# chengzhag/PanFusion

Hardware: AMD Instinct MI355X
Metric: DDIM denoise steps/sec, 512x1024 pano + 20x512^2 views (higher is better)
Workload: dtype fp16; 1 GPU; cfg2: 512x1024 pano + 20x512^2 views, CFG pair, SD-2-base UNet shapes; views=20, cfg_pair=True, hip_graphs=True, parallelism=single

## Files before the change

### include/panfusion_hip.h

```cpp
#ifndef PANFUSION_HIP_H
#define PANFUSION_HIP_H

#include <stddef.h>
#include <stdint.h>

#ifdef __cplusplus
extern "C" {
#endif

typedef enum { PF_OK = 0, PF_ERR_ARG = 1, PF_ERR_LAUNCH = 2, PF_ERR_UNSUPPORTED = 3 } pf_status;
typedef enum { PF_BF16 = 0, PF_F16 = 1, PF_F32 = 2, PF_U8 = 3 } pf_dtype;

int pf_version(void);
const char* pf_last_error_string(void);


pf_status pf_e2p_grid(const double* host_fov, const double* host_theta, const double* host_phi,
                      int ncam, int eh, int ew, int h, int w,
                      float* map_x, float* map_y, float* lonlat, void* stream);

pf_status pf_p2e_grid(const double* host_fov, const double* host_theta, const double* host_phi,
                      int ncam, int ph, int pw, int h, int w,
                      float* map_u, float* map_v, uint8_t* mask, void* stream);

// ... 63 lines not shown
pf_status pf_crop_width(const void* x, int dtype, int n, int h, int w, int C, int crop, void* y, void* stream);

pf_status pf_pad_width_rows(const void* x, int elem_bytes, long rows, int w, int pad, void* y, void* stream);
pf_status pf_roll_width_rows(const void* x, int elem_bytes, long rows, int w, int shift, void* y, void* stream);

pf_status pf_nchw_to_nhwc(const void* x, int src_dtype, int n, int C, int h, int w, int dst_dtype, void* y, void* stream);
pf_status pf_nhwc_to_nchw(const void* x, int src_dtype, int n, int C, int h, int w, int dst_dtype, void* y, void* stream);

pf_status pf_add(const void* a, int dtype_a, const void* b, int dtype_b, long n, void* y, void* stream);

pf_status pf_embed_tokens(const int64_t* ids, int B, int L, int Lp, int C, long vocab, const float* tok,
                          const float* pos, int out_dtype, void* out, void* stream);

pf_status pf_softmax_rows(const float* scores, long rows, int n, long scores_ld, float scale, int out_dtype,
                          void* probs, long probs_ld, void* stream);

pf_status pf_tensor_to_image(const float* x, int n, int C, int h, int w, uint8_t* y, void* stream);

pf_status pf_cfg_ddim_step(const float* x, const float* eps_uncond, const float* eps_cond,
                           float guidance, float sqrt_a_t, float sqrt_1m_a_t, float sqrt_a_prev,
                           float sqrt_1m_a_prev, long rows, int W, int roll, float* out, void* stream);

pf_status pf_cfg_ddim_step_pair(const float* x, const float* eps_uncond, const float* eps_cond,
                                float guidance, float sqrt_a_t, float sqrt_1m_a_t, float sqrt_a_prev,
                                float sqrt_1m_a_prev, long rows, int W, int roll, float* out, float* out2,
                                int64_t* tstep, int n_tstep, int64_t t_next, void* stream);

pf_status pf_cfg_dpmpp_step_pair(const float* x, const float* eps_uncond, const float* eps_cond,
                                 float guidance, float sqrt_a_t, float sqrt_1m_a_t, float sqrt_a_prev,
                                 float sqrt_1m_a_prev, long rows, int W, int roll, float* out, float* out2,
                                 int64_t* tstep, int n_tstep, int64_t t_next, const float* x0_prev, float k,
                                 float* x0_out, void* stream);

pf_status pf_cfg_inpaint_step_pair(const float* x, const float* eps_uncond, const float* eps_cond,
                                   float guidance, float sqrt_a_t, float sqrt_1m_a_t, float sqrt_a_prev,
                                   float sqrt_1m_a_prev, long rows, int W, int roll, float* out, float* out2,
                                   int64_t* tstep, int n_tstep, int64_t t_next, const float* x0_prev, float k,
                                   float* x0_out, const float* known, const float* noise, const float* mask,
                                   float ka, float kb, int known_roll, void* stream);

pf_status pf_noised_start_pair(const float* z, const float* noise, float ka, float kb, long rows, int W, int roll,
                               float* out, float* out2, int64_t* tstep, int n_tstep, int64_t t0, void* stream);

pf_status pf_upsampled_start_pair(const float* z, const float* noise, float ka, float kb, long planes, int h_src, int w_src,
                                  int H, int W, int mode, int wrap, int roll, float* out, float* out2, int64_t* tstep,
                                  int n_tstep, int64_t t0, void* stream);

typedef struct {
    const void* a0;
    const void* a1;
    int c0, c1;
    int a0_ld, a1_ld;
    int n_img, h_in, w_in;
    int h_out, w_out;
    int ksize;
    int stride;
    int pad;
    int upsample;
    const void* w;
    int n_out;
    const float* bias;
    const float* rowvec;
    int rowvec_ld;
    const void* residual;
    int res_ld;
    int res_dtype;
    void* out;
    int out_ld;
    int out_dtype;
    int dtype;
    int batch;
    long a_bstride, w_bstride, out_bstride, res_bstride;
    int epilogue;
    void* workspace;
    size_t workspace_bytes;
    float* gn_partial;
    int wrap_pad;
    int crop;
    int* tickets;
    int n_tickets;
    int split3;
    int subpixel;
    int gn_rows;
} pf_conv_desc;

enum { PF_EPILOGUE_NONE = 0, PF_EPILOGUE_GEGLU = 1, PF_EPILOGUE_SPLIT = 2 };

size_t pf_conv_gemm_workspace_size(const pf_conv_desc* desc);
int pf_conv_gemm_gn_rows(const pf_conv_desc* desc);
int pf_conv_gemm_kernel_id(const pf_conv_desc* desc);
typedef struct {
    int kernel;
    int mrep, nrep;
    int block_rows;
    int waves;
    int ring_slots;
    int splits;
    int kb_per_split;
    int m_split;
    int tail_splits, tail_kb;
    int gn_rows;
    int n_tickets;
    size_t workspace_bytes;
} pf_conv_plan;
pf_status pf_conv_gemm_plan(const pf_conv_desc* desc, int want_moments, pf_conv_plan* out);
pf_status pf_debug_gemm_profile(void* device_buffer, long capacity_blocks);
pf_status pf_conv_gemm(const pf_conv_desc* desc, void* stream);

typedef struct {
    const void* a; int a_ld;
    const void* w;
    const float* bias;
    const float* residual; int res_ld;
    void* out; int out_ld;
    void* out_vt; int vt_ld; int rows_per_batch; long vt_bs;
    const float* ln_gamma; const float* ln_beta; float ln_eps; void* ln_out; int ln_ld;
    int M, N, K;
    int dtype; int mode;
} pf_linear_ws_desc;
enum { PF_LWS_16 = 0, PF_LWS_F32 = 1, PF_LWS_GEGLU = 2, PF_LWS_QKV = 3, PF_LWS_F32_LN = 4, PF_LWS_VT = 5 };
int pf_linear_ws_supported(long M, int N, int K, int mode);
pf_status pf_linear_ws(const pf_linear_ws_desc* desc, void* stream);

pf_status pf_conv_in(const float* x, int n, int cin, int h, int w, const float* wgt, const float* bias,
                     int cout, int wrap, int out_dtype, void* y, void* stream);
pf_status pf_conv_out(const void* x, int dtype, int n, int cin, int h, int w, const float* wgt,
                      const float* bias, int cout, int wrap, float* y, void* stream);
pf_status pf_conv_out_gn(const float* x, int n, int cin, int h, int w, const float* scale, const float* shift, int act,
                         const float* wgt_t, const float* bias, int cout, int wrap, float* y, void* stream);

typedef struct {
    const void* q; const void* k; const void* vt; void* out;
    int dtype;
    int B, H, D;
    int nq, nk;
    int q_ld, k_ld, vt_ld, o_ld;
    long q_bs, k_bs, vt_bs, o_bs;
    float scale;
    const float* bias; long bias_ld;
    const uint8_t* flags; int flags_ld;
    float* lse;
    void* workspace; size_t workspace_bytes;
} pf_attn_desc;

pf_status pf_attention(const pf_attn_desc* desc, void* stream);
size_t pf_attention_workspace_size(const pf_attn_desc* desc);


pf_status pf_attention_delta(const void* out, const void* dout, int dtype, int B, int H, int D, long nq,
                             int ld, long bs, float* delta, void* stream);

typedef struct {
    const void* q; const void* k; const void* v; const void* dout;
    const void* qt; const void* kt; const void* dot;
    void* dq; void* dk; void* dv;
    int dtype;
    int B, H, D;
    int nq, nk;
    int q_ld, k_ld, v_ld, do_ld;
    int qt_ld, kt_ld, dot_ld;
    int dq_ld, dk_ld, dv_ld;
    long q_bs, k_bs, v_bs, do_bs, qt_bs, kt_bs, dot_bs, dq_bs, dk_bs, dv_bs;
    float scale;
    const float* bias; long bias_ld;
    const uint8_t* flags; int flags_ld;
    const float* lse; const float* delta;
// ... 58 lines not shown
```

### panfusion_amd/_lib.py

```python
import ctypes as C
import os

_HERE = os.path.dirname(os.path.abspath(__file__))
LIB_PATH = os.environ.get("PF_HIP_LIB") or os.path.join(_HERE, "libpanfusion_hip.so")

PF_OK = 0
PF_BF16, PF_F16, PF_F32, PF_U8 = 0, 1, 2, 3

c_void_p, c_int, c_long, c_float, c_size_t = C.c_void_p, C.c_int, C.c_long, C.c_float, C.c_size_t
c_dp = C.POINTER(C.c_double)


class ConvDesc(C.Structure):
    _fields_ = [
        ("a0", c_void_p), ("a1", c_void_p), ("c0", c_int), ("c1", c_int),
        ("a0_ld", c_int), ("a1_ld", c_int),
        ("n_img", c_int), ("h_in", c_int), ("w_in", c_int), ("h_out", c_int), ("w_out", c_int),
        ("ksize", c_int), ("stride", c_int), ("pad", c_int), ("upsample", c_int),
        ("w", c_void_p), ("n_out", c_int),
        ("bias", c_void_p), ("rowvec", c_void_p), ("rowvec_ld", c_int),
        ("residual", c_void_p), ("res_ld", c_int), ("res_dtype", c_int),
        ("out", c_void_p), ("out_ld", c_int), ("out_dtype", c_int), ("dtype", c_int),
        ("batch", c_int),
        ("a_bstride", c_long), ("w_bstride", c_long), ("out_bstride", c_long), ("res_bstride", c_long),
        ("epilogue", c_int), ("workspace", c_void_p), ("workspace_bytes", c_size_t),
        ("gn_partial", c_void_p), ("wrap_pad", c_int), ("crop", c_int),
        ("tickets", c_void_p), ("n_tickets", c_int), ("split3", c_int), ("subpixel", c_int), ("gn_rows", c_int),
    ]


class ConvPlan(C.Structure):
    _fields_ = [
        ("kernel", c_int), ("mrep", c_int), ("nrep", c_int), ("block_rows", c_int), ("waves", c_int), ("ring_slots", c_int),
        ("splits", c_int), ("kb_per_split", c_int), ("m_split", c_int), ("tail_splits", c_int), ("tail_kb", c_int),
        ("gn_rows", c_int), ("n_tickets", c_int), ("workspace_bytes", c_size_t),
    ]


class AttnDesc(C.Structure):
    _fields_ = [
        ("q", c_void_p), ("k", c_void_p), ("vt", c_void_p), ("out", c_void_p),
        ("dtype", c_int), ("B", c_int), ("H", c_int), ("D", c_int), ("nq", c_int), ("nk", c_int),
        ("q_ld", c_int), ("k_ld", c_int), ("vt_ld", c_int), ("o_ld", c_int),
        ("q_bs", c_long), ("k_bs", c_long), ("vt_bs", c_long), ("o_bs", c_long),
        ("scale", c_float),
        ("bias", c_void_p), ("bias_ld", c_long), ("flags", c_void_p), ("flags_ld", c_int),
        ("lse", c_void_p),
        ("workspace", c_void_p), ("workspace_bytes", c_size_t),
    ]


class LinearWsDesc(C.Structure):
    _fields_ = [
        ("a", c_void_p), ("a_ld", c_int), ("w", c_void_p), ("bias", c_void_p),
        ("residual", c_void_p), ("res_ld", c_int), ("out", c_void_p), ("out_ld", c_int),
        ("out_vt", c_void_p), ("vt_ld", c_int), ("rows_per_batch", c_int), ("vt_bs", c_long),
        ("ln_gamma", c_void_p), ("ln_beta", c_void_p), ("ln_eps", c_float), ("ln_out", c_void_p), ("ln_ld", c_int),
        ("M", c_int), ("N", c_int), ("K", c_int), ("dtype", c_int), ("mode", c_int),
    ]


class AttnBwdDesc(C.Structure):
    _fields_ = [
        ("q", c_void_p), ("k", c_void_p), ("v", c_void_p), ("dout", c_void_p),
        ("qt", c_void_p), ("kt", c_void_p), ("dot", c_void_p),
        ("dq", c_void_p), ("dk", c_void_p), ("dv", c_void_p),
        ("dtype", c_int), ("B", c_int), ("H", c_int), ("D", c_int), ("nq", c_int), ("nk", c_int),
        ("q_ld", c_int), ("k_ld", c_int), ("v_ld", c_int), ("do_ld", c_int),
        ("qt_ld", c_int), ("kt_ld", c_int), ("dot_ld", c_int),
        ("dq_ld", c_int), ("dk_ld", c_int), ("dv_ld", c_int),
        ("q_bs", c_long), ("k_bs", c_long), ("v_bs", c_long), ("do_bs", c_long), ("qt_bs", c_long), ("kt_bs", c_long),
        ("dot_bs", c_long), ("dq_bs", c_long), ("dk_bs", c_long), ("dv_bs", c_long),
        ("scale", c_float),
        ("bias", c_void_p), ("bias_ld", c_long), ("flags", c_void_p), ("flags_ld", c_int),
        ("lse", c_void_p), ("delta", c_void_p),
        ("workspace", c_void_p), ("workspace_bytes", c_size_t),
    ]


SIGNATURES = {
    "pf_version": (c_int, []),
    "pf_last_error_string": (C.c_char_p, []),
    "pf_e2p_grid": (c_int, [c_dp, c_dp, c_dp, c_int, c_int, c_int, c_int, c_int,
                            c_void_p, c_void_p, c_void_p, c_void_p]),
    "pf_p2e_grid": (c_int, [c_dp, c_dp, c_dp, c_int, c_int, c_int, c_int, c_int,
                            c_void_p, c_void_p, c_void_p, c_void_p]),
    "pf_py360_e2p": (c_int, [c_void_p, c_int, c_int, c_int, c_int, c_dp, c_dp, c_dp, c_dp, c_dp, c_int, c_int, c_int, c_int,
                             c_void_p, c_void_p]),
    "pf_nearest_indices": (c_int, [c_void_p, c_void_p, c_long, c_int, c_int, c_void_p, c_void_p]),
    "pf_remap": (c_int, [c_void_p, c_int, c_int, c_int, c_int, c_int, c_void_p, c_void_p, c_void_p,
                         c_int, c_int, c_int, c_int, c_void_p, c_void_p]),
    "pf_equi_coords": (c_int, [c_int, c_int, c_void_p, c_void_p]),
    "pf_spherical_pe": (c_int, [c_void_p, c_long, c_void_p, c_int, c_void_p, c_void_p]),
    "pf_epa_tables_workspace_size": (c_size_t, [c_int, c_int, c_int, c_int, c_int]),
    "pf_epa_tables_build": (c_int, [c_dp, c_dp, c_dp, c_int, c_int, c_int, c_int, c_int,
                                    c_void_p, c_void_p, c_void_p, c_void_p, c_void_p, c_size_t, c_void_p]),
    "pf_groupnorm_workspace_size": (c_size_t, [c_int, c_int, c_int]),
    "pf_groupnorm_stats": (c_int, [c_void_p, c_int, c_void_p, c_int, c_int, c_int, c_int, c_int, c_float,
                                   c_void_p, c_void_p, c_void_p, c_void_p, c_void_p, c_size_t, c_void_p]),
    "pf_groupnorm_stats_wrap": (c_int, [c_void_p, c_int, c_void_p, c_int, c_int, c_int, c_int, c_int, c_int, c_int, c_float,
                                        c_void_p, c_void_p, c_void_p, c_void_p, c_void_p, c_size_t, c_void_p]),
    "pf_scale_shift_act": (c_int, [c_void_p, c_int, c_void_p, c_int, c_int, c_int, c_int,
                                   c_void_p, c_void_p, c_int, c_int, c_int, c_void_p, c_void_p]),
    "pf_layernorm": (c_int, [c_void_p, c_void_p, c_long, c_int, c_long, c_int, c_void_p, c_void_p,
                             c_float, c_int, c_void_p, c_void_p]),
    "pf_axpby": (c_int, [c_void_p, c_void_p, c_float, c_float, c_long, c_void_p, c_void_p]),
    "pf_vae_sample": (c_int, [c_void_p, c_void_p, c_int, c_int, c_long, c_float, c_void_p, c_void_p]),
    "pf_geglu": (c_int, [c_void_p, c_int, c_long, c_int, c_void_p, c_void_p]),
    "pf_timestep_features": (c_int, [c_void_p, c_int, c_int, c_int, c_void_p, c_void_p]),
    "pf_timestep_features_strided": (c_int, [c_void_p, c_long, c_int, c_int, c_int, c_void_p, c_void_p]),
# ... 123 lines not shown
```

### panfusion_amd/csrc/pf_common.h

```cpp
#pragma once
#include <hip/hip_runtime.h>
#include <stdint.h>
#include <stdio.h>
#include <stdarg.h>
#include "../../include/panfusion_hip.h"

namespace pf {

void set_error(const char* fmt, ...);

#define PF_REQUIRE(cond, ...)                         \
    do {                                              \
        if (!(cond)) {                                \
            pf::set_error(__VA_ARGS__);               \
            return PF_ERR_ARG;                        \
        }                                             \
    } while (0)

#define PF_CHECK_LAUNCH(name)                                                        \
    do {                                                                             \
        hipError_t e__ = hipGetLastError();                                          \
        if (e__ != hipSuccess) {                                                     \
            pf::set_error("%s: launch failed: %s", name, hipGetErrorString(e__));    \
            return PF_ERR_LAUNCH;                                                    \
        }                                                                            \
    } while (0)

static inline bool aligned16(const void* p) { return (reinterpret_cast<uintptr_t>(p) & 15) == 0; }
static inline hipStream_t as_stream(void* s) { return reinterpret_cast<hipStream_t>(s); }
static inline long cdiv(long a, long b) { return (a + b - 1) / b; }

struct Bf16 { static constexpr int id = PF_BF16; };
struct F16  { static constexpr int id = PF_F16; };

typedef __attribute__((ext_vector_type(8))) unsigned short u16x8;
typedef __attribute__((ext_vector_type(4))) unsigned short u16x4;
typedef __attribute__((ext_vector_type(4))) float f32x4;
typedef __attribute__((ext_vector_type(16))) float f32x16;

template <typename T> __device__ __forceinline__ float to_f32(unsigned short v);
template <> __device__ __forceinline__ float to_f32<Bf16>(unsigned short v) {
    return __uint_as_float(static_cast<unsigned>(v) << 16);
}
template <> __device__ __forceinline__ float to_f32<F16>(unsigned short v) {
    _Float16 h;
    __builtin_memcpy(&h, &v, 2);
    return static_cast<float>(h);
}

template <typename T> __device__ __forceinline__ unsigned short from_f32(float f);
template <> __device__ __forceinline__ unsigned short from_f32<Bf16>(float f) {
    __bf16 b = static_cast<__bf16>(f);
    unsigned short v;
    __builtin_memcpy(&v, &b, 2);
    return v;
}
template <> __device__ __forceinline__ unsigned short from_f32<F16>(float f) {
    _Float16 h = static_cast<_Float16>(f);
    unsigned short v;
    __builtin_memcpy(&v, &h, 2);
    return v;
}

template <typename T> __device__ __forceinline__ void unpack8(const u16x8& v, float (&f)[8]) {
#pragma unroll
    for (int i = 0; i < 8; ++i) f[i] = to_f32<T>(v[i]);
}
template <typename T> __device__ __forceinline__ u16x8 pack8(const float (&f)[8]) {
    u16x8 v;
#pragma unroll
    for (int i = 0; i < 8; ++i) v[i] = from_f32<T>(f[i]);
    return v;
}

__host__ __device__ __forceinline__ int pair_off(int c) { return ((c >> 5) << 6) | (c & 31); }

__device__ __forceinline__ float silu_f(float x) { return x / (1.0f + __expf(-x)); }

template <typename S> __device__ __forceinline__ float ld_any(const void* p, long i);
struct AnyF32 {}; struct AnyBf16 {}; struct AnyF16 {};
template <> __device__ __forceinline__ float ld_any<AnyF32>(const void* p, long i) { return static_cast<const float*>(p)[i]; }
template <> __device__ __forceinline__ float ld_any<AnyBf16>(const void* p, long i) { return to_f32<Bf16>(static_cast<const unsigned short*>(p)[i]); }
template <> __device__ __forceinline__ float ld_any<AnyF16>(const void* p, long i) { return to_f32<F16>(static_cast<const unsigned short*>(p)[i]); }
template <typename S> __device__ __forceinline__ void st_any(void* p, long i, float v);
template <> __device__ __forceinline__ void st_any<AnyF32>(void* p, long i, float v) { static_cast<float*>(p)[i] = v; }
template <> __device__ __forceinline__ void st_any<AnyBf16>(void* p, long i, float v) { static_cast<unsigned short*>(p)[i] = from_f32<Bf16>(v); }
template <> __device__ __forceinline__ void st_any<AnyF16>(void* p, long i, float v) { static_cast<unsigned short*>(p)[i] = from_f32<F16>(v); }

template <typename T> struct Mfma32;
template <> struct Mfma32<Bf16> {
    typedef __attribute__((ext_vector_type(8))) __bf16 frag;
    static __device__ __forceinline__ f32x16 run(frag a, frag b, f32x16 c) {
        return __builtin_amdgcn_mfma_f32_32x32x16_bf16(a, b, c, 0, 0, 0);
    }
};
template <> struct Mfma32<F16> {
    typedef __attribute__((ext_vector_type(8))) _Float16 frag;
    static __device__ __forceinline__ f32x16 run(frag a, frag b, f32x16 c) {
        return __builtin_amdgcn_mfma_f32_32x32x16_f16(a, b, c, 0, 0, 0);
    }
};

__device__ __forceinline__ float geglu_value(float v, float g) {
    const float ax = fabsf(g);
    const float t = __builtin_amdgcn_rcpf(fmaf(ax, 0.23164189f, 1.0f));
    float y = fmaf(t, 0.5307027145f, -0.7265760135f);
    y = fmaf(y, t, 0.7107068705f);
    y = fmaf(y, t, -0.142248368f);
    y = fmaf(y, t, 0.127414796f);
    y *= t;
    const float h = y * __builtin_amdgcn_exp2f(-0.72134752044448170368f * (g * g));
    return v * fmaf(-ax, h, fmaxf(g, 0.0f));
}

#define PF_DISPATCH_16(dtype, name, ...)                                         \
    do {                                                                         \
        if ((dtype) == PF_BF16) { using T = pf::Bf16; __VA_ARGS__; }             \
        else if ((dtype) == PF_F16) { using T = pf::F16; __VA_ARGS__; }          \
        else { pf::set_error("%s: dtype must be PF_BF16 or PF_F16", name); return PF_ERR_ARG; } \
    } while (0)

}
```

### panfusion_amd/csrc/pf_elementwise.hip

```cpp
#include "pf_common.h"
#include <stdlib.h>
#include <math.h>
#include <algorithm>

namespace pf {

__device__ __forceinline__ float wave_sum(float v) {
#pragma unroll
    for (int o = 32; o > 0; o >>= 1) v += __shfl_xor(v, o);
    return v;
}

struct F32In {};
template <typename TI> struct In8 {
    typedef unsigned short elem;
    static __device__ __forceinline__ void load(const elem* ptr, float (&f)[8]) {
        unpack8<TI>(*reinterpret_cast<const u16x8*>(ptr), f);
    }
};
template <> struct In8<F32In> {
    typedef float elem;
    static __device__ __forceinline__ void load(const elem* ptr, float (&f)[8]) {
        const float4 a = reinterpret_cast<const float4*>(ptr)[0], b = reinterpret_cast<const float4*>(ptr)[1];
        f[0] = a.x; f[1] = a.y; f[2] = a.z; f[3] = a.w; f[4] = b.x; f[5] = b.y; f[6] = b.z; f[7] = b.w;
// ... 195 lines not shown
            const int pr = pbeg + pl;
            const bool first = pr < P0;
            const int pp = first ? pr : pr - P0, Ps = first ? P0 : P1, ppi = first ? ppi0 : ppi1;
            const float* base = (first ? part0 : part1) + static_cast<long>(img) * ppi * 2 * Ps + pp;
            int k = slice;
            for (; k + 3 * slices < ppi; k += 4 * slices) {
                float a[4], b[4];
#pragma unroll
                for (int u = 0; u < 4; ++u) {
                    a[u] = base[static_cast<long>(k + u * slices) * 2 * Ps];
                    b[u] = base[static_cast<long>(k + u * slices) * 2 * Ps + Ps];
                }
#pragma unroll
                for (int u = 0; u < 4; ++u) { s += a[u]; q += b[u]; }
            }
            for (; k < ppi; k += slices) {
                s += base[static_cast<long>(k) * 2 * Ps];
                q += base[static_cast<long>(k) * 2 * Ps + Ps];
            }
        }
        if (slices > 1) {
            red_s[t] = s;
            red_q[t] = q;
            __syncthreads();
            if (t < npairs) {
                double ss = 0.0, qq = 0.0;
                for (int sl = 0; sl < slices; ++sl) { ss += red_s[sl * npairs + t]; qq += red_q[sl * npairs + t]; }
                chs[t] = ss;
                chq[t] = qq;
            }
        } else if (pl < npairs) {
            chs[pl] = s;
            chq[pl] = q;
        }
    }
    __syncthreads();
    if (t < gpb && blockIdx.y * gpb + t < groups) {
        double s = 0.0, q = 0.0;
        for (int j = 0; j < ppg; ++j) { s += chs[t * ppg + j]; q += chq[t * ppg + j]; }
        const double cnt = static_cast<double>(hw) * cpg;
        const double mean = s / cnt;
        double var = q / cnt - mean * mean;
        if (var < 0.0) var = 0.0;
        g_mean[t] = static_cast<float>(mean);
        g_rstd[t] = static_cast<float>(1.0 / sqrt(var + static_cast<double>(eps)));
    }
    __syncthreads();
    const int cbeg = blockIdx.y * gpb * cpg, cend = min(C, cbeg + gpb * cpg);
    for (int c = cbeg + t; c < cend; c += 256) {
        const int gg = (c - cbeg) / cpg;
        const float sc = g_rstd[gg] * gamma[c];
        scale[static_cast<long>(img) * C + c] = sc;
        shift[static_cast<long>(img) * C + c] = beta[c] - g_mean[gg] * sc;
    }
}

template <typename TI, typename T, int OUT>
__global__ __launch_bounds__(256) void k_scale_shift_act(const typename In8<TI>::elem* __restrict__ x0, int c0,
                                  const typename In8<TI>::elem* __restrict__ x1, int c1, int hw,
                                  const float* __restrict__ scale, const float* __restrict__ shift,
                                  int act, void* __restrict__ yv, unsigned short* __restrict__ raw_pair) {
    typedef typename In8<TI>::elem elem;
    const unsigned C = c0 + c1, OCT = C / 8, per_img = static_cast<unsigned>(hw) * OCT;
    const unsigned img = blockIdx.y;
    const unsigned j0 = (blockIdx.x * 256u + threadIdx.x) * 2u;
    if (j0 >= per_img) return;
    float v[2][8];
    unsigned cc[2];
    long pix[2];
#pragma unroll
    for (int u = 0; u < 2; ++u) {
        const unsigned j = min(j0 + u, per_img - 1);
        const unsigned p = j / OCT, c = (j - p * OCT) * 8;
        cc[u] = c;
        pix[u] = static_cast<long>(img) * hw + p;
        const elem* src = (c < static_cast<unsigned>(c0)) ? x0 + pix[u] * c0 + c : x1 + pix[u] * c1 + (c - c0);
        In8<TI>::load(src, v[u]);
    }
#pragma unroll
    for (int u = 0; u < 2; ++u) {
        if (j0 + u >= per_img) break;
        if (raw_pair) {
            unsigned short* y = raw_pair + pix[u] * (2 * C) + pair_off(cc[u]);
            const u16x8 hi = pack8<T>(v[u]);
            float lo[8];
#pragma unroll
            for (int j = 0; j < 8; ++j) lo[j] = v[u][j] - to_f32<T>(hi[j]);
            *reinterpret_cast<u16x8*>(y) = hi;
            *reinterpret_cast<u16x8*>(y + 32) = pack8<T>(lo);
        }
        float f[8];
        if (scale) {
            const float4* sc = reinterpret_cast<const float4*>(scale + static_cast<long>(img) * C + cc[u]);
            const float4* sh = reinterpret_cast<const float4*>(shift + static_cast<long>(img) * C + cc[u]);
            float4 s0 = sc[0], s1 = sc[1], h0 = sh[0], h1 = sh[1];
            const float sv[8] = {s0.x, s0.y, s0.z, s0.w, s1.x, s1.y, s1.z, s1.w};
            const float hv[8] = {h0.x, h0.y, h0.z, h0.w, h1.x, h1.y, h1.z, h1.w};
#pragma unroll
            for (int j = 0; j < 8; ++j) f[j] = v[u][j] * sv[j] + hv[j];
        } else {
#pragma unroll
            for (int j = 0; j < 8; ++j) f[j] = v[u][j];
        }
        if (act) {
#pragma unroll
            for (int j = 0; j < 8; ++j) f[j] = f[j] * __builtin_amdgcn_rcpf(1.0f + __expf(-f[j]));
        }
        if (OUT == 0) {
            *reinterpret_cast<u16x8*>(static_cast<unsigned short*>(yv) + pix[u] * C + cc[u]) = pack8<T>(f);
        } else if (OUT == 1) {
            unsigned short* y = static_cast<unsigned short*>(yv) + pix[u] * (2 * C) + pair_off(cc[u]);
            const u16x8 hi = pack8<T>(f);
            float lo[8];
#pragma unroll
            for (int j = 0; j < 8; ++j) lo[j] = f[j] - to_f32<T>(hi[j]);
            *reinterpret_cast<u16x8*>(y) = hi;
            *reinterpret_cast<u16x8*>(y + 32) = pack8<T>(lo);
        } else {
            store8_f32(static_cast<float*>(yv) + pix[u] * C + cc[u], f);
        }
    }
}

template <typename TI, typename T, int ROWS>
__global__ __launch_bounds__(256) void k_layernorm(const typename In8<TI>::elem* __restrict__ x, const float* __restrict__ pe,
                            long pe_rows, long rows, int C, const float* __restrict__ gamma,
                            const float* __restrict__ beta, float eps, unsigned short* __restrict__ y) {
    const int lane = threadIdx.x & 63;
    const long row0 = (blockIdx.x * static_cast<long>(blockDim.x >> 6) + (threadIdx.x >> 6)) * ROWS;
    if (row0 >= rows) return;
    const int OCT = C / 8;
    constexpr int KMAX = ROWS == 1 ? 4 : 1;
    float raw[ROWS][KMAX][8];
#pragma unroll
    for (int r = 0; r < ROWS; ++r)
#pragma unroll
        for (int k = 0; k < KMAX; ++k) {
            const int oct = lane + 64 * k;
#pragma unroll
            for (int j = 0; j < 8; ++j) raw[r][k][j] = 0.f;
            if (oct < OCT && row0 + r < rows) In8<TI>::load(x + (row0 + r) * C + oct * 8, raw[r][k]);
        }
#pragma unroll
    for (int r = 0; r < ROWS; ++r) {
        const long row = row0 + r;
        if (row >= rows) break;
        float (&v)[KMAX][8] = raw[r];
        float s = 0.f;
#pragma unroll
        for (int k = 0; k < KMAX; ++k) {
            const int oct = lane + 64 * k;
            if (oct < OCT) {
                if (pe) {
                    const float4* pp = reinterpret_cast<const float4*>(pe + (row % pe_rows) * C + oct * 8);
                    float4 a = pp[0], b = pp[1];
                    v[k][0] += a.x; v[k][1] += a.y; v[k][2] += a.z; v[k][3] += a.w;
                    v[k][4] += b.x; v[k][5] += b.y; v[k][6] += b.z; v[k][7] += b.w;
                }
#pragma unroll
                for (int j = 0; j < 8; ++j) s += v[k][j];
            }
        }
        const float mean = wave_sum(s) / static_cast<float>(C);
        float q = 0.f;
#pragma unroll
        for (int k = 0; k < KMAX; ++k) {
            const int oct = lane + 64 * k;
            if (oct < OCT) {
#pragma unroll
                for (int j = 0; j < 8; ++j) { float d = v[k][j] - mean; q += d * d; }
            }
        }
        const float rstd = 1.0f / sqrtf(wave_sum(q) / static_cast<float>(C) + eps);
#pragma unroll
        for (int k = 0; k < KMAX; ++k) {
            const int oct = lane + 64 * k;
            if (oct < OCT) {
                const float4* gp = reinterpret_cast<const float4*>(gamma + oct * 8);
                const float4* bp = reinterpret_cast<const float4*>(beta + oct * 8);
                float4 g0 = gp[0], g1 = gp[1], b0 = bp[0], b1 = bp[1];
                const float gv[8] = {g0.x, g0.y, g0.z, g0.w, g1.x, g1.y, g1.z, g1.w};
                const float bv[8] = {b0.x, b0.y, b0.z, b0.w, b1.x, b1.y, b1.z, b1.w};
                float f[8];
#pragma unroll
                for (int j = 0; j < 8; ++j) f[j] = (v[k][j] - mean) * rstd * gv[j] + bv[j];
                *reinterpret_cast<u16x8*>(y + row * C + oct * 8) = pack8<T>(f);
            }
        }
    }
}

template <typename T>
__global__ void k_geglu(const unsigned short* __restrict__ in, long total_oct, int inner,
                        unsigned short* __restrict__ out) {
    long i = blockIdx.x * static_cast<long>(blockDim.x) + threadIdx.x;
    if (i >= total_oct) return;
    const int OCT = inner / 8;
    const long row = i / OCT;
    const int c = (i % OCT) * 8;
    u16x8 a = *reinterpret_cast<const u16x8*>(in + row * 2 * inner + c);
// ... 1203 lines not shown
```

### panfusion_amd/csrc/pf_gemm.hip

```cpp
#include "pf_common.h"
#include "pf_gemm_params.h"
#include <stdlib.h>
#include <algorithm>
#include <atomic>
#include <type_traits>

namespace pf {


template <typename T> struct Mfma;
template <> struct Mfma<Bf16> {
    typedef __attribute__((ext_vector_type(8))) __bf16 frag;
    static __device__ __forceinline__ f32x4 run(frag a, frag b, f32x4 c) {
        return __builtin_amdgcn_mfma_f32_16x16x32_bf16(a, b, c, 0, 0, 0);
    }
    static __device__ __forceinline__ void acc_agpr(frag a, frag b, f32x4& c) {
        asm volatile("v_mfma_f32_16x16x32_bf16 %0, %1, %2, %0" : "+a"(c) : "v"(a), "v"(b));
    }
};
template <> struct Mfma<F16> {
    typedef __attribute__((ext_vector_type(8))) _Float16 frag;
    static __device__ __forceinline__ f32x4 run(frag a, frag b, f32x4 c) {
        return __builtin_amdgcn_mfma_f32_16x16x32_f16(a, b, c, 0, 0, 0);
    }
// ... 336 lines not shown
template <typename T, int MREP, int NREP, int NT, int BM, int BN, int HALVES = 1, bool STATS = false, typename F = NoOp>
__device__ __forceinline__ void epilogue_tile(const GemmParams& p, long bz, f32x4 (&acc)[MREP][NREP],
                                              unsigned short* smem16, int m0, int n0, int row_base, int col_base,
                                              int lane, int t, F after_ring = F()) {
    if constexpr (STATS) {
        if (!(p.out_f32 && p.residual)) gn_moments_phase<T, MREP, NREP>(p, bz, acc, m0, n0, row_base, col_base, lane);
        __builtin_amdgcn_sched_barrier(0);
    }
    __syncthreads();
    stamp(p, 4);
    after_ring();
    stamp(p, 5);
    if constexpr (STATS) {
        if (p.out_f32 && p.residual) {
            epilogue_f32_stats<T, MREP, NREP, true>(p, bz, acc, m0, n0, row_base, col_base, lane);
            return;
        }
    }
    const int n_store = p.geglu ? p.N >> 1 : p.N;
    if (p.split_out && !p.rowvec && (p.N & 3) == 0 && (p.out_ld & 3) == 0 && p.N >= 4) {
        if (!p.residual) { epilogue_f32<T, MREP, NREP, false, true>(p, bz, acc, m0, n0, row_base, col_base, lane); return; }
        if (p.res_f32 && (p.res_ld & 3) == 0) { epilogue_f32<T, MREP, NREP, true, true>(p, bz, acc, m0, n0, row_base, col_base, lane); return; }
    }
    if (p.out_f32 && !p.geglu && !p.rowvec && (p.N & 3) == 0 && (p.out_ld & 3) == 0 && p.N >= 4) {
        if (!p.residual) { epilogue_f32<T, MREP, NREP, false>(p, bz, acc, m0, n0, row_base, col_base, lane); return; }
        if (p.res_f32 && (p.res_ld & 3) == 0) { epilogue_f32<T, MREP, NREP, true>(p, bz, acc, m0, n0, row_base, col_base, lane); return; }
    }
    const bool staged = !p.out_f32 && !p.res_f32 && !p.split_out && (p.out_ld & 7) == 0 && (n_store & 7) == 0 && (p.N & 3) == 0;
    if (staged && !(p.rowvec && p.residual) && !(p.geglu && (p.rowvec || p.residual))) {
        if (p.geglu) epilogue_fast<T, MREP, NREP, NT, BM, BN, 1, 3>(p, bz, acc, smem16, m0, n0, row_base, col_base, lane, t);
        else if (p.rowvec && p.rows_per_img < BM) goto generic;
        else if (p.rowvec) epilogue_fast<T, MREP, NREP, NT, BM, BN, HALVES, 1>(p, bz, acc, smem16, m0, n0, row_base, col_base, lane, t);
        else if (p.residual) epilogue_fast<T, MREP, NREP, NT, BM, BN, HALVES, 2>(p, bz, acc, smem16, m0, n0, row_base, col_base, lane, t);
        else epilogue_fast<T, MREP, NREP, NT, BM, BN, HALVES, 0>(p, bz, acc, smem16, m0, n0, row_base, col_base, lane, t);
        return;
    }
generic:
    const int cq = 4 * (lane >> 4), rl = lane & 15;
#pragma unroll
    for (int i = 0; i < MREP; ++i) {
        const int m = m0 + row_base + i * 16 + rl;
#pragma unroll
        for (int j = 0; j < NREP; ++j) {
            const int n4 = n0 + col_base + j * 16 + cq;
            float v[4] = {acc[i][j][0], acc[i][j][1], acc[i][j][2], acc[i][j][3]};
            if (m < p.M && n4 < p.N) epilogue_store<T>(p, bz, m, n4, v);
        }
    }
}


template <typename T, int BM, int BN, int NT>
__device__ __forceinline__ void splitk_finish(const GemmParams& p, long bz, int tile_lin, int m0, int n0, int* flag, int t) {
    asm volatile("s_waitcnt vmcnt(0)" ::: "memory");
    __syncthreads();
    int* ticket = p.tickets + (bz * p.mtiles * p.ntiles + tile_lin);
    if (t == 0) {
        const int drawn = __hip_atomic_fetch_add(ticket, 1, __ATOMIC_RELAXED, __HIP_MEMORY_SCOPE_AGENT);
        *flag = drawn == p.splits - 1 ? 1 : 0;
    }
    __syncthreads();
    const bool last = *flag != 0;
    __syncthreads();
    if (!last) return;
    if (t == 0) __builtin_amdgcn_fence(__ATOMIC_ACQUIRE, "agent");
    __syncthreads();
    constexpr int QPR = BN / 4;
    const int Ms = p.M - p.m_begin;
    const long slab = static_cast<long>(p.batch) * Ms * p.N;
    for (int q = t; q < BM * QPR; q += NT) {
        const int r = q / QPR, m = m0 + r, n4 = n0 + (q - r * QPR) * 4;
        if (m >= p.M || n4 >= p.N) continue;
        const float* src = p.partial + (bz * Ms + (m - p.m_begin)) * p.N + n4;
        float v[4] = {0.f, 0.f, 0.f, 0.f};
        for (int s = 0; s < p.splits; ++s) {
            const float4 x = *reinterpret_cast<const float4*>(src + s * slab);
            v[0] += x.x; v[1] += x.y; v[2] += x.z; v[3] += x.w;
        }
        epilogue_store<T>(p, bz, m, n4, v);
    }
    if (t == 0) __hip_atomic_store(ticket, 0, __ATOMIC_RELAXED, __HIP_MEMORY_SCOPE_AGENT);
}

template <typename T, int MREP, int NREP, bool STATS = false, bool S3 = false, int STAGES = 2>
__global__ __launch_bounds__(256, STAGES > 2 ? 1 : 2) void k_conv_gemm(const GemmParams p) {
    constexpr int BM = 32 * MREP, BN = 32 * NREP;
    extern __shared__ __attribute__((aligned(16))) unsigned short smem[];
    unsigned short* As = smem;
    unsigned short* Bs = smem + STAGES * BM * 64;

    const int ntile_total = p.mtiles * p.ntiles;
    int tid_lin = blockIdx.x;
    {
        const int q = ntile_total / 8, r = ntile_total % 8;
        const int xcd = tid_lin % 8, idx = tid_lin / 8;
        tid_lin = (xcd < r ? xcd * (q + 1) : r * (q + 1) + (xcd - r) * q) + idx;
    }
    const int tile_n = tid_lin % p.ntiles, tile_m = tid_lin / p.ntiles;
    const int m0 = p.m_begin + tile_m * BM, n0 = tile_n * BN;
    const long bz = blockIdx.z;
    const unsigned short* a0 = p.a0 + bz * p.a_bs;
    const unsigned short* a1 = p.a1 ? p.a1 + bz * p.a_bs : nullptr;
    const unsigned short* wg = p.w + bz * p.w_bs;

    const int t = threadIdx.x, lane = t & 63;
    const int wave = __builtin_amdgcn_readfirstlane(t >> 6);
    const int wm = wave >> 1, wn = wave & 1;
    const int chunk = t & 7, lrow = t >> 3;
    const int lchunk8 = (chunk ^ ((lrow >> 1) & 7)) * 8;

    const int pad_y = p.subpix ? 1 - (static_cast<int>(bz) >> 1) : p.pad, pad_x = p.subpix ? 1 - (static_cast<int>(bz) & 1) : p.pad;
    int a_img[MREP], a_y[MREP], a_x[MREP];
#pragma unroll
    for (int i = 0; i < MREP; ++i) {
        const int m = m0 + i * 32 + lrow;
        if (m < p.M) {
            const int img = m / p.rows_per_img, rem = m - img * p.rows_per_img;
            const int yo = rem / p.w_out;
            a_img[i] = img;
            a_y[i] = yo * p.stride - pad_y;
            a_x[i] = (rem - yo * p.w_out + p.crop) * p.stride - pad_x;
        } else {
            a_img[i] = 0; a_y[i] = -(1 << 20); a_x[i] = 0;
        }
        if (p.fastseg) seg_pack(a_img[i], a_y[i], a_x[i], p.h_in, p.w_in);
    }
    constexpr unsigned OOB = 0x80000000u;
    auto uniform_ptr = [](const unsigned short* ptr) {
        const unsigned long long v = reinterpret_cast<unsigned long long>(ptr);
        const unsigned lo = __builtin_amdgcn_readfirstlane(static_cast<unsigned>(v));
        const unsigned hi = __builtin_amdgcn_readfirstlane(static_cast<unsigned>(v >> 32));
        return reinterpret_cast<unsigned short*>(static_cast<unsigned long long>(lo) | (static_cast<unsigned long long>(hi) << 32));
    };
    const __amdgpu_buffer_rsrc_t rs_w = __builtin_amdgcn_make_buffer_rsrc(uniform_ptr(wg), 0, __builtin_amdgcn_readfirstlane(p.w_bytes), 0x00020000);
    unsigned w_off[NREP];
#pragma unroll
    for (int j = 0; j < NREP; ++j) {
        const int n = n0 + j * 32 + lrow;
        w_off[j] = n < p.N ? static_cast<unsigned>(n * p.K + lchunk8) * 2u : OOB;
    }
    const int Ctot = p.c0 + p.c1;
    const int Hl = p.h_in << p.up, Wl = (p.w_in + 2 * p.wrap) << p.up;

    const int nkb = p.K / 64;
    const int kb0 = blockIdx.y * p.kb_per_split;
    const int kb1 = min(nkb, kb0 + p.kb_per_split);
    int kg = kb0 * 64;
    int tap = kg / Ctot, cc = kg - tap * Ctot;
    unsigned a_off[MREP];
    bool seg1 = false;
    auto set_segment = [&]() {
        const int ky = p.ksize == 3 ? tap / 3 : p.ksize == 2 ? tap >> 1 : 0, kx = p.ksize == 3 ? tap - 3 * ky : p.ksize == 2 ? tap & 1 : 0;
        seg1 = __builtin_amdgcn_readfirstlane(cc >= p.c0 ? 1 : 0) != 0;
        const int ld = seg1 ? p.a1_ld : p.a0_ld;
        if (p.fastseg) {
            const unsigned sel = (1u << ky) | (16u << kx);
            const int tap_pix = ky * p.w_in + kx;
#pragma unroll
            for (int i = 0; i < MREP; ++i) {
                const unsigned off = ((static_cast<unsigned>(a_img[i]) + static_cast<unsigned>(tap_pix)) * static_cast<unsigned>(ld) + static_cast<unsigned>(lchunk8)) * 2u;
                a_off[i] = (static_cast<unsigned>(a_y[i]) & sel) == sel ? off : OOB;
            }
            return;
        }
#pragma unroll
        for (int i = 0; i < MREP; ++i) {
            const int yi = a_y[i] + ky, xi = a_x[i] + kx;
            const bool ok = yi >= 0 && yi < Hl && xi >= 0 && xi < Wl;
            int sx = (xi >> p.up) - p.wrap;
            sx += sx < 0 ? p.w_in : 0;
            sx -= sx >= p.w_in ? p.w_in : 0;
            const int pix = (a_img[i] * p.h_in + (yi >> p.up)) * p.w_in + sx;
            a_off[i] = ok ? static_cast<unsigned>(pix * ld + lchunk8) * 2u : OOB;
        }
    };
    set_segment();

    auto lds_dma = [&](const __amdgpu_buffer_rsrc_t& r, unsigned short* dst, unsigned voff, int soff) {
        __builtin_amdgcn_raw_ptr_buffer_load_lds(r, (__attribute__((address_space(3))) void*)dst, 16, voff, soff, 0, 0);
    };
    auto dma_stage = [&](int buf) {
        const int soff_a = __builtin_amdgcn_readfirstlane((seg1 ? cc - p.c0 : cc) * 2);
        const int soff_w = __builtin_amdgcn_readfirstlane(kg * 2);
        const __amdgpu_buffer_rsrc_t rs_a = __builtin_amdgcn_make_buffer_rsrc(
            uniform_ptr(seg1 ? a1 : a0), 0, __builtin_amdgcn_readfirstlane(seg1 ? p.a1_bytes : p.a0_bytes), 0x00020000);
#pragma unroll
        for (int i = 0; i < MREP; ++i) {
            unsigned short* dst = As + buf * BM * 64 + (i * 32 + wave * 8) * 64;
            lds_dma(rs_a, dst, a_off[i], soff_a);
        }
#pragma unroll
        for (int j = 0; j < NREP; ++j) {
            unsigned short* dst = Bs + buf * BN * 64 + (j * 32 + wave * 8) * 64;
            lds_dma(rs_w, dst, w_off[j], soff_w);
        }
        kg += 64;
        cc += 64;
        if (cc == Ctot) { cc = 0; ++tap; set_segment(); }
        else if (cc == p.c0) set_segment();
    };

    f32x4 acc[MREP][NREP];
#pragma unroll
    for (int i = 0; i < MREP; ++i)
#pragma unroll
        for (int j = 0; j < NREP; ++j) acc[i][j] = f32x4{0.f, 0.f, 0.f, 0.f};

    typedef typename Mfma<T>::frag frag;
    const int frow = lane & 15, fchunk = lane >> 4;
    auto compute = [&](int buf) {
        if constexpr (S3) {
            frag af[2][MREP], bf[2][NREP];
#pragma unroll
            for (int slab = 0; slab < 2; ++slab) {
#pragma unroll
                for (int i = 0; i < MREP; ++i)
                    af[slab][i] = __builtin_bit_cast(frag, *reinterpret_cast<const u16x8*>(As + buf * BM * 64 + lds_off(wm * 16 * MREP + i * 16 + frow, slab * 4 + fchunk)));
#pragma unroll
                for (int j = 0; j < NREP; ++j)
                    bf[slab][j] = __builtin_bit_cast(frag, *reinterpret_cast<const u16x8*>(Bs + buf * BN * 64 + lds_off(wn * 16 * NREP + j * 16 + frow, slab * 4 + fchunk)));
            }
#pragma unroll
            for (int i = 0; i < MREP; ++i)
#pragma unroll
                for (int j = 0; j < NREP; ++j) {
                    acc[i][j] = Mfma<T>::run(bf[0][j], af[0][i], acc[i][j]);
                    acc[i][j] = Mfma<T>::run(bf[0][j], af[1][i], acc[i][j]);
                    acc[i][j] = Mfma<T>::run(bf[1][j], af[0][i], acc[i][j]);
                }
            return;
        }
#pragma unroll
        for (int slab = 0; slab < 2; ++slab) {
            frag af[MREP], bf[NREP];
#pragma unroll
            for (int i = 0; i < MREP; ++i) {
                const int brow = wm * 16 * MREP + i * 16 + frow;
                u16x8 v = *reinterpret_cast<const u16x8*>(As + buf * BM * 64 + lds_off(brow, slab * 4 + fchunk));
                af[i] = __builtin_bit_cast(frag, v);
            }
#pragma unroll
            for (int j = 0; j < NREP; ++j) {
                const int brow = wn * 16 * NREP + j * 16 + frow;
                u16x8 v = *reinterpret_cast<const u16x8*>(Bs + buf * BN * 64 + lds_off(brow, slab * 4 + fchunk));
                bf[j] = __builtin_bit_cast(frag, v);
            }
#pragma unroll
            for (int i = 0; i < MREP; ++i)
#pragma unroll
                for (int j = 0; j < NREP; ++j) acc[i][j] = Mfma<T>::run(bf[j], af[i], acc[i][j]);
        }
    };

    stamp(p, 0);
    if constexpr (STAGES == 2) {
        dma_stage(0);
        asm volatile("s_waitcnt vmcnt(0)" ::: "memory");
        __syncthreads();
        stamp(p, 1);
        for (int kb = kb0, it = 0; kb < kb1; ++kb, ++it) {
            if (kb + 1 < kb1) dma_stage((it + 1) & 1);
            compute(it & 1);
            asm volatile("s_waitcnt vmcnt(0)" ::: "memory");
            __syncthreads();
        }
    } else {
        constexpr int L = MREP + NREP, KEEP = (STAGES - 2) * L;
        const int n_it = kb1 - kb0;
#pragma unroll
        for (int s = 0; s < STAGES - 1; ++s)
            if (s < n_it) dma_stage(s);
        if (n_it >= STAGES - 1) asm volatile("s_waitcnt vmcnt(%0)" :: "n"(KEEP) : "memory");
        else asm volatile("s_waitcnt vmcnt(0)" ::: "memory");
        __syncthreads();
        stamp(p, 1);
        int slot = 0, fill = STAGES - 1;
        for (int it = 0; it < n_it; ++it) {
            const bool more = it + STAGES - 1 < n_it;
            if (more) dma_stage(fill);
            compute(slot);
            if (more) asm volatile("s_waitcnt vmcnt(%0)" :: "n"(KEEP) : "memory");
            else asm volatile("s_waitcnt vmcnt(0)" ::: "memory");
            __syncthreads();
            slot = slot == STAGES - 1 ? 0 : slot + 1;
            fill = fill == STAGES - 1 ? 0 : fill + 1;
        }
    }
    stamp(p, 2);

    if (p.splits > 1) {
#pragma unroll
        for (int i = 0; i < MREP; ++i) {
            const int m = m0 + wm * 16 * MREP + i * 16 + (lane & 15);
            if (m >= p.M) continue;
#pragma unroll
            for (int j = 0; j < NREP; ++j) {
                const int n4 = n0 + wn * 16 * NREP + j * 16 + 4 * (lane >> 4);
                if (n4 >= p.N) continue;
                slab_store(p, ((static_cast<long>(blockIdx.y) * p.batch + bz) * (p.M - p.m_begin) + (m - p.m_begin)) * p.N + n4, acc[i][j]);
            }
        }
        if (p.tickets) splitk_finish<T, BM, BN, 256>(p, bz, tid_lin, m0, n0, reinterpret_cast<int*>(smem), t);
        return;
    }
    epilogue_tile<T, MREP, NREP, 256, BM, BN, 1, STATS>(p, bz, acc, smem, m0, n0, wm * 16 * MREP, wn * 16 * NREP, lane, t);
    stamp(p, 3);
}

template <typename T, int NREP, int NW, bool STATS = false, bool S3 = false, int BM_ = 256>
__global__ __launch_bounds__(64 * NW, BM_ == 128 ? 2 : 1) void k_conv_gemm8(const GemmParams p) {
    constexpr int NT = 64 * NW, WMG = NW / 2, BM = BM_, BN = 32 * NREP, MREP = BM / (16 * WMG), STAGES = BM_ == 128 ? 2 : 3;
    constexpr bool ONEWAVE = NW == 4 && BM_ == 256;
    static_assert(BM_ == 256 || (BM_ == 128 && NW == 4), "tile shapes: 256 rows (8 or 4 waves) or 128 rows (4 waves, two blocks per CU)");
    constexpr int RPP = NT / 8;
    constexpr int STAGE = (BM + BN) * 64;
    constexpr int BFULL = BN / RPP;
    constexpr bool BHALF = (BN % RPP) != 0;
    extern __shared__ __attribute__((aligned(16))) unsigned short smem[];

    const int ntile_total = p.mtiles * p.ntiles;
    const long bz = blockIdx.z;
    const unsigned short* a0 = p.a0 + bz * p.a_bs;
    const unsigned short* a1 = p.a1 ? p.a1 + bz * p.a_bs : nullptr;
    const unsigned short* wg = p.w + bz * p.w_bs;
    int m0 = 0, n0 = 0;
    const int pad_y = p.subpix ? 1 - (static_cast<int>(bz) >> 1) : p.pad, pad_x = p.subpix ? 1 - (static_cast<int>(bz) & 1) : p.pad;

    const int t = threadIdx.x, lane = t & 63;
    const int wave = __builtin_amdgcn_readfirstlane(t >> 6);
    const int wm = wave >> 1, wn = wave & 1;
    const int chunk = t & 7, lrow = t >> 3;
    const int lchunk8 = (chunk ^ ((lrow >> 1) & 7)) * 8;
    const int hrow = wave * 4 + (lane >> 3);
    const int hchunk8 = (chunk ^ ((hrow >> 1) & 7)) * 8;

    constexpr int APASS = BM / RPP;
    int a_img[APASS], a_y[APASS], a_x[APASS];
    constexpr unsigned OOB = 0x80000000u;
    auto uniform_ptr = [](const unsigned short* ptr) __attribute__((always_inline)) {
        const unsigned long long v = reinterpret_cast<unsigned long long>(ptr);
        const unsigned lo = __builtin_amdgcn_readfirstlane(static_cast<unsigned>(v));
        const unsigned hi = __builtin_amdgcn_readfirstlane(static_cast<unsigned>(v >> 32));
        return reinterpret_cast<unsigned short*>(static_cast<unsigned long long>(lo) | (static_cast<unsigned long long>(hi) << 32));
    };
    const __amdgpu_buffer_rsrc_t rs_w = __builtin_amdgcn_make_buffer_rsrc(uniform_ptr(wg), 0, __builtin_amdgcn_readfirstlane(p.w_bytes), 0x00020000);
    unsigned w_off[BFULL + 1];
#ifdef PF_GEMM_BDIRECT
    unsigned wb_off[NREP];
    int kw = 0;
#endif
    const int Ctot = p.c0 + p.c1;
    const int Hl = p.h_in << p.up, Wl = (p.w_in + 2 * p.wrap) << p.up;

    const int nkb = p.K / 64;
    const int kb0 = blockIdx.y * p.kb_per_split;
    const int kb1 = min(nkb, kb0 + p.kb_per_split);
    const int n_it = kb1 - kb0;
    int kg = 0, tap = 0, cc = 0;
    unsigned a_off[APASS];
    bool seg1 = false;
    auto set_segment = [&]() __attribute__((always_inline)) {
        const int ky = p.ksize == 3 ? tap / 3 : p.ksize == 2 ? tap >> 1 : 0, kx = p.ksize == 3 ? tap - 3 * ky : p.ksize == 2 ? tap & 1 : 0;
        seg1 = __builtin_amdgcn_readfirstlane(cc >= p.c0 ? 1 : 0) != 0;
        const int ld = seg1 ? p.a1_ld : p.a0_ld;
        if (p.fastseg) {
            const unsigned sel = (1u << ky) | (16u << kx);
            const int tap_pix = ky * p.w_in + kx;
#pragma unroll
            for (int i = 0; i < APASS; ++i) {
                const unsigned off = ((static_cast<unsigned>(a_img[i]) + static_cast<unsigned>(tap_pix)) * static_cast<unsigned>(ld) + static_cast<unsigned>(lchunk8)) * 2u;
                a_off[i] = (static_cast<unsigned>(a_y[i]) & sel) == sel ? off : OOB;
            }
            return;
        }
#pragma unroll
        for (int i = 0; i < APASS; ++i) {
            const int yi = a_y[i] + ky, xi = a_x[i] + kx;
            const bool ok = yi >= 0 && yi < Hl && xi >= 0 && xi < Wl;
            int sx = (xi >> p.up) - p.wrap;
            sx += sx < 0 ? p.w_in : 0;
            sx -= sx >= p.w_in ? p.w_in : 0;
            const int pix = (a_img[i] * p.h_in + (yi >> p.up)) * p.w_in + sx;
            a_off[i] = ok ? static_cast<unsigned>(pix * ld + lchunk8) * 2u : OOB;
        }
    };
    auto set_tile = [&](int tile) __attribute__((always_inline)) {
        int tid_lin = tile;
        {
            const int q = ntile_total >> 3, r = ntile_total & 7;
            const int xcd = tid_lin & 7, idx = tid_lin >> 3;
            tid_lin = (xcd < r ? xcd * (q + 1) : r * (q + 1) + (xcd - r) * q) + idx;
        }
        const int tile_m = static_cast<unsigned>(tid_lin) / static_cast<unsigned>(p.ntiles), tile_n = tid_lin - tile_m * p.ntiles;
        m0 = p.m_begin + tile_m * BM;
        n0 = tile_n * BN;
        {
            const unsigned m = static_cast<unsigned>(m0 + lrow);
            int img = static_cast<int>(m / static_cast<unsigned>(p.rows_per_img));
            const unsigned rem = m - static_cast<unsigned>(img) * static_cast<unsigned>(p.rows_per_img);
            int yo = static_cast<int>(rem / static_cast<unsigned>(p.w_out));
            int xo = static_cast<int>(rem) - yo * p.w_out;
#pragma unroll
            for (int i = 0; i < APASS; ++i) {
                const bool ok = m0 + i * RPP + lrow < p.M;
                a_img[i] = ok ? img : 0;
                a_y[i] = ok ? yo * p.stride - pad_y : -(1 << 20);
                a_x[i] = (xo + p.crop) * p.stride - pad_x;
                if (p.fastseg) seg_pack(a_img[i], a_y[i], a_x[i], p.h_in, p.w_in);
                xo += p.adv_x;
                if (xo >= p.w_out) { xo -= p.w_out; ++yo; }
                yo += p.adv_y;
                if (yo >= p.h_out) { yo -= p.h_out; ++img; }
                img += p.adv_img;
            }
        }
#pragma unroll
        for (int j = 0; j < BFULL; ++j) {
            const int n = n0 + j * RPP + lrow;
            w_off[j] = n < p.N ? static_cast<unsigned>(n * p.K + lchunk8) * 2u : OOB;
        }
        {
            const int n = n0 + BFULL * RPP + hrow;
            w_off[BFULL] = (BHALF && n < p.N) ? static_cast<unsigned>(n * p.K + hchunk8) * 2u : OOB;
        }
        kg = kb0 * 64;
        tap = kg / Ctot;
        cc = kg - tap * Ctot;
        set_segment();
#ifdef PF_GEMM_BDIRECT
        kw = kb0 * 64;
#pragma unroll
        for (int j = 0; j < NREP; ++j) {
            const int n = n0 + (wave & 1) * 16 * NREP + j * 16 + (lane & 15);
            wb_off[j] = n < p.N ? static_cast<unsigned>(n * p.K + (lane >> 4) * 8) * 2u : OOB;
        }
#endif
    };

    constexpr int NPIECE = APASS + BFULL + (BHALF ? 1 : 0);
    int st_soff_a = 0, st_soff_w = 0;
    auto stage_begin = [&]() __attribute__((always_inline)) {
        st_soff_a = __builtin_amdgcn_readfirstlane((seg1 ? cc - p.c0 : cc) * 2);
        st_soff_w = __builtin_amdgcn_readfirstlane(kg * 2);
        return __builtin_amdgcn_make_buffer_rsrc(uniform_ptr(seg1 ? a1 : a0), 0,
                                                 __builtin_amdgcn_readfirstlane(seg1 ? p.a1_bytes : p.a0_bytes), 0x00020000);
    };
    auto stage_end = [&]() __attribute__((always_inline)) {
        kg += 64;
        cc += 64;
        if (cc == Ctot) { cc = 0; ++tap; set_segment(); }
        else if (cc == p.c0) set_segment();
    };
    auto lds_dma = [&](const __amdgpu_buffer_rsrc_t& r, unsigned short* dst, unsigned voff, int soff) __attribute__((always_inline)) {
        __builtin_amdgcn_raw_ptr_buffer_load_lds(r, (__attribute__((address_space(3))) void*)dst, 16, voff, soff, 0, 0);
    };
    auto dma_piece = [&](const __amdgpu_buffer_rsrc_t& rs_a, int slot, int k) __attribute__((always_inline)) {
        unsigned short* As = smem + slot * STAGE;
        unsigned short* Bs = As + BM * 64;
        if (k < APASS) {
            unsigned short* dst = As + (k * RPP + wave * 8) * 64;
            lds_dma(rs_a, dst, a_off[k], st_soff_a);
#ifdef PF_GEMM_BDIRECT
        } else if (true) {
#endif
        } else if (k < APASS + BFULL) {
            const int j = k - APASS;
            lds_dma(rs_w, Bs + (j * RPP + wave * 8) * 64, w_off[j], st_soff_w);
        } else if (BHALF) {
            if (lane < 32) lds_dma(rs_w, Bs + (BFULL * RPP + wave * 4) * 64, w_off[BFULL], st_soff_w);
        }
    };
    auto dma_stage = [&](int slot) __attribute__((always_inline)) {
        const __amdgpu_buffer_rsrc_t rs_a = stage_begin();
#pragma unroll
        for (int k = 0; k < NPIECE; ++k) dma_piece(rs_a, slot, k);
        stage_end();
    };

    f32x4 acc[MREP][NREP];

    typedef typename Mfma<T>::frag frag;
    const int frow = lane & 15, fchunk = lane >> 4;
    frag fa0[MREP], fb0[NREP], fa1[MREP], fb1[NREP];
#ifdef PF_ABL_DUMMY_B
#pragma unroll
    for (int j = 0; j < NREP; ++j) {
        u16x8 z = {1, 2, 3, 4, 5, 6, 7, static_cast<unsigned short>(lane)};
        asm volatile("" : "+v"(z));
        fb0[j] = __builtin_bit_cast(frag, z);
        fb1[j] = __builtin_bit_cast(frag, z);
    }
#endif
    auto load_frags_a = [&](int slot, int slab, frag (&fa)[MREP]) __attribute__((always_inline)) {
        const unsigned short* As = smem + slot * STAGE;
#pragma unroll
        for (int i = 0; i < MREP; ++i)
            fa[i] = __builtin_bit_cast(frag, *reinterpret_cast<const u16x8*>(As + lds_off(wm * 16 * MREP + i * 16 + frow, slab * 4 + fchunk)));
    };
    auto load_frags_b = [&](int slot, int slab, frag (&fb)[NREP], int kadd) __attribute__((always_inline)) {
#ifdef PF_GEMM_BDIRECT
        typedef __attribute__((ext_vector_type(4))) unsigned int u32x4;
        const int soff = __builtin_amdgcn_readfirstlane((kw + kadd + slab * 32) * 2);
#pragma unroll
        for (int j = 0; j < NREP; ++j) {
            const u32x4 v = __builtin_amdgcn_raw_buffer_load_b128(rs_w, wb_off[j], soff, 0);
            fb[j] = __builtin_bit_cast(frag, v);
        }
        return;
#endif
        const unsigned short* Bs = smem + slot * STAGE + BM * 64;
#ifdef PF_ABL_DUMMY_B
#pragma unroll
        for (int j = 0; j < NREP; ++j) {
            u16x8 v = *reinterpret_cast<const u16x8*>(Bs + lds_off(wn * 16 * NREP + j * 16 + frow, slab * 4 + fchunk));
            asm volatile("" :: "v"(v));
        }
        (void)fb;
#else
#pragma unroll
        for (int j = 0; j < NREP; ++j)
            fb[j] = __builtin_bit_cast(frag, *reinterpret_cast<const u16x8*>(Bs + lds_off(wn * 16 * NREP + j * 16 + frow, slab * 4 + fchunk)));
#endif
    };
    auto load_frags = [&](int slot, int slab, frag (&fa)[MREP], frag (&fb)[NREP], int kadd) __attribute__((always_inline)) {
        load_frags_a(slot, slab, fa);
#ifndef PF_ABL_NOLDS_B
        load_frags_b(slot, slab, fb, kadd);
#endif
    };

    auto issue_prologue = [&]() __attribute__((always_inline)) {
        dma_stage(0);
        if (n_it > 1) dma_stage(1);
    };
    const std::true_type YES;
    const std::false_type NO;
    int cur = 0, nx1 = 1, nx2 = 2;
#ifdef PF_GEMM_TIMELINE
    int tl_tile = 0, tl_step = 0;
#endif
    auto step_l = [&](auto more_tag, auto dma_tag, auto wait_tag, auto flead_tag) __attribute__((always_inline)) {
        constexpr bool MORE = decltype(more_tag)::value, DMA = decltype(dma_tag)::value;
        constexpr int WAIT = decltype(wait_tag)::value;
        constexpr int NM = MREP * NREP, LEAD0 = NM - 1 - 2 * (NPIECE - 1), LEAD = LEAD0 < 4 ? LEAD0 : 4, FLEAD = decltype(flead_tag)::value;
#pragma unroll
        for (int idx = 0; idx < NM; ++idx) {
            const int fi = S3 ? idx % MREP : idx / NREP, fj = S3 ? idx / MREP : idx % NREP;
            if constexpr (ONEWAVE) Mfma<T>::acc_agpr(fb0[fj], fa0[fi], acc[fi][fj]);
            else acc[fi][fj] = Mfma<T>::run(fb0[fj], fa0[fi], acc[fi][fj]);
#ifdef PF_GEMM_FLEAD2
            if (idx == FLEAD - 1) { __builtin_amdgcn_sched_barrier(0); load_frags_a(cur, 1, fa1); __builtin_amdgcn_sched_barrier(0); }
            if (idx == PF_GEMM_FLEAD2 - 1) { __builtin_amdgcn_sched_barrier(0); load_frags_b(cur, 1, fb1, 0); __builtin_amdgcn_sched_barrier(0); }
#else
            if (idx == FLEAD - 1) {
                __builtin_amdgcn_sched_barrier(0);
#ifndef PF_ABL_NOLDS
                load_frags(cur, 1, fa1, fb1, 0);
#endif
                __builtin_amdgcn_sched_barrier(0);
            }
#endif
        }
        if constexpr (S3) __builtin_amdgcn_sched_barrier(0);
        if constexpr (MORE) {
#ifdef PF_GEMM_BDIRECT
            if constexpr (true) asm volatile("s_waitcnt vmcnt(0) lgkmcnt(0)" ::: "memory");
#else
            if constexpr (WAIT == 0) asm volatile("s_waitcnt vmcnt(0) lgkmcnt(0)" ::: "memory");
#endif
            else if constexpr (WAIT == 6) asm volatile("s_waitcnt vmcnt(6) lgkmcnt(0)" ::: "memory");
            else if constexpr (WAIT == 7) asm volatile("s_waitcnt vmcnt(7) lgkmcnt(0)" ::: "memory");
            else if constexpr (WAIT == 8) asm volatile("s_waitcnt vmcnt(8) lgkmcnt(0)" ::: "memory");
            else if constexpr (WAIT == 9) asm volatile("s_waitcnt vmcnt(9) lgkmcnt(0)" ::: "memory");
            else if constexpr (WAIT == 12) asm volatile("s_waitcnt vmcnt(12) lgkmcnt(0)" ::: "memory");
            else if constexpr (WAIT == 13) asm volatile("s_waitcnt vmcnt(13) lgkmcnt(0)" ::: "memory");
            else static_assert(WAIT == 0, "add the immediate");
#ifndef PF_ABL_NOBARRIER
            __builtin_amdgcn_s_barrier();
#endif
            asm volatile("" ::: "memory");
        }
        __amdgpu_buffer_rsrc_t rs_a = rs_w;
        if constexpr (DMA) rs_a = stage_begin();
        if constexpr (S3) {
#pragma unroll
            for (int idx = 0; idx < NM; ++idx) {
                acc[idx / NREP][idx % NREP] = Mfma<T>::run(fb1[idx % NREP], fa0[idx / NREP], acc[idx / NREP][idx % NREP]);
                if constexpr (DMA) {
                    const int k = idx - LEAD;
                    if (k >= 0 && (k & 1) == 0 && (k >> 1) < NPIECE) {
                        __builtin_amdgcn_sched_barrier(0);
                        dma_piece(rs_a, cur, k >> 1);
                        __builtin_amdgcn_sched_barrier(0);
                    }
                }
            }
            if (MORE) { __builtin_amdgcn_sched_barrier(0); load_frags_a(nx1, 0, fa0); __builtin_amdgcn_sched_barrier(0); }
#pragma unroll
            for (int j = 0; j < NREP; ++j) {
#pragma unroll
                for (int i = 0; i < MREP; ++i) acc[i][j] = Mfma<T>::run(fb0[j], fa1[i], acc[i][j]);
                if (MORE) {
                    __builtin_amdgcn_sched_barrier(0);
                    const unsigned short* Bn = smem + nx1 * STAGE + BM * 64;
                    fb0[j] = __builtin_bit_cast(frag, *reinterpret_cast<const u16x8*>(Bn + lds_off(wn * 16 * NREP + j * 16 + frow, fchunk)));
                    __builtin_amdgcn_sched_barrier(0);
                }
            }
        } else {
#pragma unroll
        for (int idx = 0; idx < NM; ++idx) {
            if constexpr (ONEWAVE) Mfma<T>::acc_agpr(fb1[idx % NREP], fa1[idx / NREP], acc[idx / NREP][idx % NREP]);
            else acc[idx / NREP][idx % NREP] = Mfma<T>::run(fb1[idx % NREP], fa1[idx / NREP], acc[idx / NREP][idx % NREP]);
#ifdef PF_GEMM_FLEAD2
            if (MORE && idx == FLEAD - 1) { __builtin_amdgcn_sched_barrier(0); load_frags_a(nx1, 0, fa0); __builtin_amdgcn_sched_barrier(0); }
            if (MORE && idx == PF_GEMM_FLEAD2 - 1) { __builtin_amdgcn_sched_barrier(0); load_frags_b(nx1, 0, fb0, 64); __builtin_amdgcn_sched_barrier(0); }
#else
            if (MORE && idx == FLEAD - 1) {
                __builtin_amdgcn_sched_barrier(0);
#ifndef PF_ABL_NOLDS
                load_frags(nx1, 0, fa0, fb0, 64);
#endif
                __builtin_amdgcn_sched_barrier(0);
            }
#endif
            if constexpr (DMA) {
                const int k = idx - LEAD;
                if (k >= 0 && (k & 1) == 0 && (k >> 1) < NPIECE) {
                    __builtin_amdgcn_sched_barrier(0);
#ifndef PF_ABL_NODMA
#ifdef PF_ABL_NODMA_B
                    if ((k >> 1) < APASS)
#endif
                    dma_piece(rs_a, cur, k >> 1);
#endif
                    __builtin_amdgcn_sched_barrier(0);
                }
            }
        }
        }
        static_assert(LEAD >= 0 && LEAD + 2 * (NPIECE - 1) < NM, "DMA pieces must fit behind the MFMAs of the second half");
        if constexpr (DMA) stage_end();
        cur = cur == STAGES - 1 ? 0 : cur + 1;
        nx1 = nx1 == STAGES - 1 ? 0 : nx1 + 1;
        nx2 = nx2 == STAGES - 1 ? 0 : nx2 + 1;
#ifdef PF_GEMM_BDIRECT
        kw += 64;
#endif
#ifdef PF_GEMM_TIMELINE
        PF_TL(p, tl_tile == 1 && tl_step < 8, 15 + tl_step);
        ++tl_step;
#endif
    };
#ifndef PF_GEMM_FLEAD
#define PF_GEMM_FLEAD 4
#endif
    auto step = [&](auto more_tag, auto dma_tag, auto wait_tag) __attribute__((always_inline)) { step_l(more_tag, dma_tag, wait_tag, std::integral_constant<int, PF_GEMM_FLEAD>()); };

    stamp(p, 0);
#ifdef PF_GEMM_SETPRIO
    if (NW == 8 && wave >= 4) __builtin_amdgcn_s_setprio(PF_GEMM_SETPRIO);
#endif
    int tile = blockIdx.x;
    set_tile(tile);
    issue_prologue();
    bool first = true;
    for (;;) {
        PF_TL(p, tl_tile == 1, 12);
#pragma unroll
        for (int i = 0; i < MREP; ++i)
#pragma unroll
            for (int j = 0; j < NREP; ++j) acc[i][j] = f32x4{0.f, 0.f, 0.f, 0.f};
        if (first && n_it > 1) {
#ifdef PF_GEMM_BDIRECT
            if constexpr (true) asm volatile("s_waitcnt vmcnt(0)" ::: "memory");
#else
            if constexpr (NPIECE == 7) asm volatile("s_waitcnt vmcnt(7)" ::: "memory");
#endif
            else if constexpr (NPIECE == 6) asm volatile("s_waitcnt vmcnt(6)" ::: "memory");
            else if constexpr (NPIECE == 8) asm volatile("s_waitcnt vmcnt(8)" ::: "memory");
            else if constexpr (NPIECE == 9) asm volatile("s_waitcnt vmcnt(9)" ::: "memory");
            else if constexpr (NPIECE == 13) asm volatile("s_waitcnt vmcnt(13)" ::: "memory");
            else if constexpr (NPIECE == 12) asm volatile("s_waitcnt vmcnt(12)" ::: "memory");
            else asm volatile("s_waitcnt vmcnt(0)" ::: "memory");
        } else {
            asm volatile("s_waitcnt vmcnt(0)" ::: "memory");
        }
        __builtin_amdgcn_s_barrier();
        asm volatile("" ::: "memory");
        if (first) stamp(p, 1);
        first = false;
        PF_TL(p, tl_tile == 1, 13);
        if constexpr (STAGES == 3) { if (n_it > 2) dma_stage(2); }
        load_frags(0, 0, fa0, fb0, 0);
        cur = 0; nx1 = 1; nx2 = 2 % STAGES;
        PF_TL(p, tl_tile == 1, 14);
        const std::integral_constant<int, NPIECE> W1;
        const std::integral_constant<int, 0> W0;
        if constexpr (STAGES == 3) {
            for (int it = 0; it + 3 < n_it; ++it) step(YES, YES, W1);
            if (n_it >= 3) step(YES, NO, W1);
            if (n_it >= 2) step(YES, NO, W0);
            step(NO, NO, W0);
        } else {
            for (int it = 0; it + 2 < n_it; ++it) step(YES, YES, W0);
            if (n_it >= 2) step(YES, NO, W0);
            step(NO, NO, W0);
        }
        if constexpr (ONEWAVE) asm volatile("s_nop 15\n\ts_nop 15" ::: "memory");
        stamp(p, 2);

        const int em0 = m0, en0 = n0;
        const int next = tile + static_cast<int>(gridDim.x);
        const bool has_next = next < ntile_total;
        if (p.splits > 1) {
#pragma unroll
            for (int i = 0; i < MREP; ++i) {
                const int m = em0 + wm * 16 * MREP + i * 16 + (lane & 15);
                if (m >= p.M) continue;
#pragma unroll
                for (int j = 0; j < NREP; ++j) {
                    const int n4 = en0 + wn * 16 * NREP + j * 16 + 4 * (lane >> 4);
                    if (n4 >= p.N) continue;
                    slab_store(p, ((static_cast<long>(blockIdx.y) * p.batch + bz) * (p.M - p.m_begin) + (m - p.m_begin)) * p.N + n4, acc[i][j]);
                }
            }
            if (p.tickets) splitk_finish<T, BM, BN, NT>(p, bz, tile, em0, en0, reinterpret_cast<int*>(smem + (STAGES - 1) * STAGE), t);
            if (!has_next) break;
            __syncthreads();
            set_tile(next);
            issue_prologue();
        } else {
            int e_lane = lane, e_t = t;
            asm volatile("" : "+v"(e_lane), "+v"(e_t));
            if constexpr (STAGES == 3) {
                epilogue_tile<T, MREP, NREP, NT, BM, BN, 2, STATS>(p, bz, acc, smem + 2 * STAGE, em0, en0, wm * 16 * MREP, wn * 16 * NREP,
                                                            e_lane, e_t, [&]() __attribute__((always_inline)) { if (has_next) { set_tile(next); issue_prologue(); } });
            } else {
                epilogue_tile<T, MREP, NREP, NT, BM, BN, 1, STATS>(p, bz, acc, smem, em0, en0, wm * 16 * MREP, wn * 16 * NREP, e_lane, e_t);
                if (has_next) {
                    __syncthreads();
                    set_tile(next);
                    issue_prologue();
                }
            }
            PF_TL(p, tl_tile == 1, 23);
            if (!has_next) break;
        }
        tile = next;
#ifdef PF_GEMM_TIMELINE
        ++tl_tile; tl_step = 0;
#endif
    }
    stamp(p, 3);
}

template <typename T>
__global__ __launch_bounds__(256) void k_splitk_reduce(const GemmParams p) {
    const long quads = static_cast<long>(p.N / 4);
    const int Ms = p.M - p.m_begin;
    const long total = static_cast<long>(p.batch) * Ms * quads;
    const long i = blockIdx.x * 256L + threadIdx.x;
    if (i >= total) return;
    const int n4 = static_cast<int>(i % quads) * 4;
    const long bm = i / quads;
    const int ml = static_cast<int>(bm % Ms), m = p.m_begin + ml;
    const long bz = bm / Ms;
    const long slab = static_cast<long>(p.batch) * Ms * p.N;
    const float* src = p.partial + (bz * Ms + ml) * p.N + n4;
    float v[4] = {0.f, 0.f, 0.f, 0.f};
    for (int s = 0; s < p.splits; ++s) {
        const float4 x = *reinterpret_cast<const float4*>(src + s * slab);
        v[0] += x.x; v[1] += x.y; v[2] += x.z; v[3] += x.w;
    }
    epilogue_store<T>(p, bz, m, n4, v);
}

struct ProfState { unsigned long long* buf; long blocks; };
static std::atomic<const ProfState*> g_prof_state{nullptr};
static inline ProfState prof_snapshot() {
    const ProfState* s = g_prof_state.load(std::memory_order_acquire);
    return s ? *s : ProfState{nullptr, 0};
}

pf_status allow_dynamic_lds(const void* kernel, size_t bytes, std::atomic<unsigned long long>& done, const char* what) {
    int dev = 0;
    hipError_t e = hipGetDevice(&dev);
    const unsigned long long bit = dev >= 0 && dev < 64 ? 1ULL << dev : 0;
    if (e == hipSuccess && (done.load(std::memory_order_relaxed) & bit)) return PF_OK;
    if (e == hipSuccess) e = hipFuncSetAttribute(kernel, hipFuncAttributeMaxDynamicSharedMemorySize, static_cast<int>(bytes));
    if (e != hipSuccess) { set_error("%s: hipFuncSetAttribute failed: %s", what, hipGetErrorString(e)); return PF_ERR_LAUNCH; }
    done.fetch_or(bit, std::memory_order_relaxed);
    return PF_OK;
}


template <typename T, int MREP, int NREP, bool STATS, bool S3, int STAGES>
static pf_status launch_ring(const GemmParams& p, int batch, hipStream_t st) {
    constexpr int BM = 32 * MREP, BN = 32 * NREP;
    const size_t smem = static_cast<size_t>(STAGES) * (BM + BN) * 64 * sizeof(unsigned short);
    static std::atomic<unsigned long long> lds_set{0};
    const pf_status s = allow_dynamic_lds(reinterpret_cast<const void*>(k_conv_gemm<T, MREP, NREP, STATS, S3, STAGES>), smem, lds_set, "pf_conv_gemm");
    if (s != PF_OK) return s;
    hipLaunchKernelGGL((k_conv_gemm<T, MREP, NREP, STATS, S3, STAGES>), dim3(p.mtiles * p.ntiles, p.splits, batch), dim3(256), smem, st, p);
    PF_CHECK_LAUNCH("pf_conv_gemm");
    return PF_OK;
}

template <typename T, int MREP, int NREP, bool STATS = false, bool S3 = false>
static pf_status launch_s(const pf_conv_plan& g, const GemmParams& gp, int batch, hipStream_t st) {
    constexpr int BM = 32 * MREP, BN = 32 * NREP;
    GemmParams p = gp;
    p.mtiles = static_cast<int>(cdiv(p.M - p.m_begin, BM));
    p.ntiles = static_cast<int>(cdiv(p.N, BN));
    const ProfState ps = prof_snapshot();
    p.prof = (ps.buf && static_cast<long>(p.mtiles) * p.ntiles * p.splits * batch <= ps.blocks) ? ps.buf : nullptr;
    if constexpr (!STATS && !S3) {
        if (g.ring_slots == 4) return launch_ring<T, MREP, NREP, false, false, 4>(p, batch, st);
    }
    return launch_ring<T, MREP, NREP, STATS, S3, 2>(p, batch, st);
}

template <typename T, int MREP, int NREP>
static pf_status launch(const pf_conv_plan& g, const GemmParams& gp, int batch, hipStream_t st) {
    if (gp.s3) return gp.gn_partial ? launch_s<T, MREP, NREP, true, true>(g, gp, batch, st) : launch_s<T, MREP, NREP, false, true>(g, gp, batch, st);
    return gp.gn_partial ? launch_s<T, MREP, NREP, true>(g, gp, batch, st) : launch_s<T, MREP, NREP, false>(g, gp, batch, st);
}

template <typename T, int NREP, int NW, bool STATS = false, bool S3 = false, int BM = 256>
static pf_status launch8w_s(const GemmParams& gp, int batch, hipStream_t st) {
    constexpr int BN = 32 * NREP, STAGES = BM == 128 ? 2 : 3;
    GemmParams p = gp;
    p.mtiles = static_cast<int>(cdiv(p.M - p.m_begin, BM));
    p.ntiles = static_cast<int>(cdiv(p.N, BN));
    {
        const int rpp = 8 * NW, rem = rpp % p.rows_per_img;
        p.adv_img = rpp / p.rows_per_img;
        p.adv_y = rem / p.w_out;
        p.adv_x = rem % p.w_out;
    }
    const ProfState ps = prof_snapshot();
    p.prof = (ps.buf && static_cast<long>(p.mtiles) * p.ntiles * p.splits * batch <= ps.blocks) ? ps.buf : nullptr;
    const size_t smem = static_cast<size_t>(STAGES) * (BM + BN) * 64 * sizeof(unsigned short);
    static std::atomic<unsigned long long> lds_set{0};
    const pf_status s = allow_dynamic_lds(reinterpret_cast<const void*>(k_conv_gemm8<T, NREP, NW, STATS, S3, BM>), smem, lds_set, "pf_conv_gemm (8-wave)");
    if (s != PF_OK) return s;
    const int cap1 = gemm_tuning().big_persist;
    const int cap = BM == 128 ? 2 * cap1 : cap1;
    int grid = p.mtiles * p.ntiles;
    if (cap > 0) {
        int gx = std::max(1, cap / (p.splits * batch));
        if (gx >= 8) gx = gx / 8 * 8;
        grid = std::min(grid, gx);
    }
    hipLaunchKernelGGL((k_conv_gemm8<T, NREP, NW, STATS, S3, BM>), dim3(grid, p.splits, batch), dim3(64 * NW), smem, st, p);
    PF_CHECK_LAUNCH("pf_conv_gemm (8-wave)");
    return PF_OK;
}

template <typename T, int NREP, int NW, int BM = 256>
static pf_status launch8w(const GemmParams& gp, int batch, hipStream_t st) {
    if constexpr (NW == 8 || BM == 128) {
        if (gp.s3) return gp.gn_partial ? launch8w_s<T, NREP, NW, true, true, BM>(gp, batch, st) : launch8w_s<T, NREP, NW, false, true, BM>(gp, batch, st);
        if (gp.gn_partial) return launch8w_s<T, NREP, NW, true, false, BM>(gp, batch, st);
    }
    return launch8w_s<T, NREP, NW, false, false, BM>(gp, batch, st);
}

template <typename T, int NREP>
static pf_status launch8(const pf_conv_plan& g, const GemmParams& gp, int batch, hipStream_t st) {
    if (g.block_rows == 128) return launch8w<T, NREP, 4, 128>(gp, batch, st);
    if (g.waves == 4) return launch8w<T, NREP, 4>(gp, batch, st);
    return launch8w<T, NREP, 8>(gp, batch, st);
}

static pf_status launch_pass(const pf_conv_plan& g, GemmParams p, int dtype, int batch, hipStream_t st) {
    pf_status s = PF_OK;
    if (g.kernel == 2) {
        const ProfState ps = prof_snapshot();
        p.prof = (ps.buf && ps.blocks >= 256) ? ps.buf : nullptr;
        s = launch_gemm32(p, dtype, batch, st);
    } else if (g.kernel == 1) {
        PF_DISPATCH_16(dtype, "pf_conv_gemm", s = g.nrep == 5 ? launch8<T, 5>(g, p, batch, st) : launch8<T, 4>(g, p, batch, st));
    } else {
        PF_DISPATCH_16(dtype, "pf_conv_gemm",
            if (g.nrep == 5) s = g.mrep == 2 ? launch<T, 2, 5>(g, p, batch, st) : launch<T, 4, 5>(g, p, batch, st);
            else s = g.mrep == 2 ? launch<T, 2, 4>(g, p, batch, st) : launch<T, 4, 4>(g, p, batch, st));
    }
    if (s != PF_OK || p.splits == 1 || p.tickets) return s;
    const long total = static_cast<long>(batch) * (p.M - p.m_begin) * (p.N / 4);
    PF_DISPATCH_16(dtype, "pf_conv_gemm", hipLaunchKernelGGL((k_splitk_reduce<T>), dim3(cdiv(total, 256)), dim3(256), 0, st, p));
    PF_CHECK_LAUNCH("pf_conv_gemm (split-K reduce)");
    return PF_OK;
}

}

using namespace pf;

extern "C" pf_status pf_conv_gemm(const pf_conv_desc* d, void* stream) {
    PF_REQUIRE(d, "pf_conv_gemm: null descriptor");
    PF_REQUIRE(d->a0 && d->w && d->out, "pf_conv_gemm: null pointer");
    PF_REQUIRE(d->dtype == PF_BF16 || d->dtype == PF_F16, "pf_conv_gemm: dtype must be PF_BF16 or PF_F16");
    PF_REQUIRE(d->out_dtype == d->dtype || d->out_dtype == PF_F32, "pf_conv_gemm: out_dtype must equal dtype or be PF_F32");
    PF_REQUIRE(!d->residual || d->res_dtype == d->dtype || d->res_dtype == PF_F32, "pf_conv_gemm: res_dtype must equal dtype or be PF_F32");
    const int c1 = d->a1 ? d->c1 : 0;
    PF_REQUIRE(d->c0 > 0 && d->c0 % 64 == 0 && c1 % 64 == 0, "pf_conv_gemm: channel counts (%d,%d) must be multiples of 64", d->c0, c1);
    PF_REQUIRE(d->ksize == 1 || d->ksize == 3, "pf_conv_gemm: ksize must be 1 or 3");
    PF_REQUIRE(d->stride == 1 || d->stride == 2, "pf_conv_gemm: stride must be 1 or 2");
    PF_REQUIRE(d->pad == 0 || d->pad == 1, "pf_conv_gemm: pad must be 0 or 1");
    PF_REQUIRE(d->upsample == 0 || d->upsample == 1, "pf_conv_gemm: upsample must be 0 or 1");
    PF_REQUIRE(d->n_img > 0 && d->h_in > 0 && d->w_in > 0 && d->h_out > 0 && d->w_out > 0, "pf_conv_gemm: bad spatial sizes");
    PF_REQUIRE(d->n_out > 0 && (d->n_out % 4 == 0 || (!d->bias && !d->rowvec && !d->residual && d->out_ld >= (d->n_out + 3) / 4 * 4)),
               "pf_conv_gemm: n_out=%d must be a multiple of 4 (or no epilogue operands and a padded out_ld)", d->n_out);
    PF_REQUIRE(d->a0_ld >= d->c0 && d->a0_ld % 8 == 0, "pf_conv_gemm: a0_ld must be >= c0 and a multiple of 8");
    PF_REQUIRE(!d->a1 || (d->a1_ld >= c1 && d->a1_ld % 8 == 0), "pf_conv_gemm: a1_ld must be >= c1 and a multiple of 8");
    PF_REQUIRE(d->epilogue == PF_EPILOGUE_GEGLU || (d->out_ld >= d->n_out && d->out_ld % 4 == 0), "pf_conv_gemm: out_ld must be >= n_out and a multiple of 4");
    PF_REQUIRE(!d->residual || (d->res_ld >= d->n_out && d->res_ld % 4 == 0), "pf_conv_gemm: res_ld must be >= n_out and a multiple of 4");
    PF_REQUIRE(!d->rowvec || (d->rowvec_ld >= d->n_out && d->rowvec_ld % 4 == 0), "pf_conv_gemm: rowvec_ld must be >= n_out and a multiple of 4");
    PF_REQUIRE(aligned16(d->a0) && aligned16(d->w) && aligned16(d->out) && (!d->a1 || aligned16(d->a1)) &&
               (!d->bias || aligned16(d->bias)) && (!d->rowvec || aligned16(d->rowvec)) &&
               (!d->residual || aligned16(d->residual)), "pf_conv_gemm: pointers must be 16-byte aligned");
    PF_REQUIRE(d->batch >= 1, "pf_conv_gemm: batch must be >= 1");
    PF_REQUIRE(d->epilogue == PF_EPILOGUE_NONE || d->epilogue == PF_EPILOGUE_GEGLU || d->epilogue == PF_EPILOGUE_SPLIT,
               "pf_conv_gemm: unknown epilogue %d", d->epilogue);
    if (d->epilogue == PF_EPILOGUE_SPLIT)
        PF_REQUIRE(d->n_out % 32 == 0 && d->out_dtype == d->dtype && d->out_ld >= 2 * d->n_out && !d->rowvec,
                   "pf_conv_gemm: SPLIT epilogue needs n_out %% 32 == 0 (hi / lo interleave per 32 columns), a 16-bit output with out_ld >= 2 n_out, no row vector");
    if (d->split3)
        PF_REQUIRE(!d->a1 && d->c0 % 64 == 0, "pf_conv_gemm: a split-precision walk (split3) takes ONE source of 2 x channels = c0 (hi / lo interleaved per 32)");
    if (d->epilogue == PF_EPILOGUE_GEGLU)
        PF_REQUIRE(d->n_out % 4 == 0 && d->out_dtype == d->dtype && !d->residual && d->out_ld >= d->n_out / 2 && d->out_ld % 2 == 0,
                   "pf_conv_gemm: GEGLU epilogue needs n_out %% 4 == 0, 16-bit output, no residual, out_ld >= n_out/2");
    PF_REQUIRE(d->wrap_pad >= 0 && d->wrap_pad <= 2 && d->crop >= 0 && d->crop <= 2 && d->wrap_pad <= d->w_in,
               "pf_conv_gemm: wrap_pad and crop must be in 0..2");
    {
        const int hl = d->h_in << d->upsample, wl = (d->w_in + 2 * d->wrap_pad) << d->upsample;
        const int ho = (hl + 2 * d->pad - d->ksize) / d->stride + 1, wo = (wl + 2 * d->pad - d->ksize) / d->stride + 1 - 2 * d->crop;
        const int ho1 = (hl + 2 * d->pad + 1 - d->ksize) / d->stride + 1, wo1 = (wl + 2 * d->pad + 1 - d->ksize) / d->stride + 1 - 2 * d->crop;
        PF_REQUIRE((d->h_out == ho && d->w_out == wo) || (d->h_out == ho1 && d->w_out == wo1),
                   "pf_conv_gemm: output size (%d,%d) does not match (%d,%d) [or (%d,%d) with a trailing zero row / column]",
                   d->h_out, d->w_out, ho, wo, ho1, wo1);
    }
    if (d->subpixel)
        PF_REQUIRE(d->ksize == 3 && d->upsample == 1 && d->stride == 1 && d->pad == 1 && d->batch == 1 && !d->residual && !d->rowvec &&
                   d->epilogue == PF_EPILOGUE_NONE && d->h_out % 2 == 0 && d->w_out % 2 == 0 && d->crop % 2 == 0 && d->wrap_pad <= 1,
                   "pf_conv_gemm: subpixel serves nearest x2 + 3x3 stride-1 pad-1 convolutions (bias only; weights packed [4][n_out][2][2][c0 + c1])");
    const int batch = d->subpixel ? 4 : d->batch;
    GemmParams p;
    params_from_desc(d, p);
    const pf_conv_plan g = plan_conv_gemm(p, batch, d->workspace != nullptr, d->gn_partial != nullptr);
    if (d->gn_partial) {
        PF_REQUIRE(g.gn_rows > 0, "pf_conv_gemm: gn_partial given but this problem cannot emit GroupNorm moments (ask pf_conv_gemm_gn_rows first)");
        PF_REQUIRE(aligned16(d->gn_partial), "pf_conv_gemm: gn_partial must be 16-byte aligned");
        PF_REQUIRE(d->gn_rows == g.gn_rows, "pf_conv_gemm: gn_partial is sized for runs of gn_rows = %d rows, but this launch's plan writes runs of %d rows (ask pf_conv_gemm_plan again)",
                   d->gn_rows, g.gn_rows);
        p.gn_partial = d->gn_partial;
        p.gn_rows = g.gn_rows;
    }
    {
        const long npix = static_cast<long>(d->n_img) * d->h_in * d->w_in;
        const long a0b = ((npix - 1) * p.a0_ld + p.c0) * 2, a1b = p.a1 ? ((npix - 1) * p.a1_ld + p.c1) * 2 : 0;
        const long wb = static_cast<long>(p.N) * p.K * 2;
        PF_REQUIRE(a0b < (1L << 31) && a1b < (1L << 31) && wb < (1L << 31),
                   "pf_conv_gemm: each operand must be smaller than 2 GiB (32-bit buffer offsets)");
        p.a0_bytes = static_cast<unsigned>(a0b); p.a1_bytes = static_cast<unsigned>(a1b); p.w_bytes = static_cast<unsigned>(wb);
    }
    p.partial = static_cast<float*>(d->workspace);
    if (d->tickets && g.kernel != 2 && gemm_tuning().splitk_inkernel && d->workspace_bytes < (1ULL << 32)) {
        PF_REQUIRE(d->n_tickets >= g.n_tickets && (reinterpret_cast<uintptr_t>(d->tickets) & 3) == 0,
                   "pf_conv_gemm: %d arrival counters needed, %d given", g.n_tickets, d->n_tickets);
        p.tickets = d->tickets;
    }
    PF_REQUIRE(g.workspace_bytes == 0 || (d->workspace_bytes >= g.workspace_bytes && aligned16(d->workspace)),
               "pf_conv_gemm: workspace of %zu bytes (16-byte aligned) needed, got %zu", g.workspace_bytes, d->workspace_bytes);
    hipStream_t st = as_stream(stream);
    p.splits = g.splits; p.kb_per_split = g.kb_per_split;
    if (g.m_split == 0) return launch_pass(g, p, d->dtype, batch, st);
    GemmParams p2 = p;
    p.M = g.m_split;
    p2.m_begin = g.m_split; p2.splits = g.tail_splits; p2.kb_per_split = g.tail_kb;
    const pf_status s1 = launch_pass(g, p, d->dtype, batch, st);
    return s1 != PF_OK ? s1 : launch_pass(g, p2, d->dtype, batch, st);
}

extern "C" pf_status pf_debug_gemm_profile(void* device_buffer, long capacity_blocks) {
    const ProfState* s = device_buffer ? new ProfState{static_cast<unsigned long long*>(device_buffer), capacity_blocks} : nullptr;
    g_prof_state.store(s, std::memory_order_release);
    return PF_OK;
}
```

### panfusion_amd/csrc/pf_gemm_params.h

```cpp
#pragma once
#include <atomic>
#include <cstdlib>

#include "pf_common.h"

namespace pf {

struct GemmParams {
    const unsigned short* a0; const unsigned short* a1;
    int c0, c1, a0_ld, a1_ld;
    int h_in, w_in, h_out, w_out;
    int ksize, stride, pad, up;
    int wrap, crop;
    const unsigned short* w;
    int M, N, K;
    int m_begin;
    int rows_per_img;
    const float* bias; const float* rowvec; int rowvec_ld;
    const void* residual; int res_ld; int res_f32;
    void* out; int out_ld; int out_f32; int geglu;
    int split_out;
    long a_bs, w_bs, out_bs, res_bs;
    int mtiles, ntiles;
    int splits, kb_per_split;
    float* partial;
    int* tickets;
    int batch;
    unsigned a0_bytes, a1_bytes, w_bytes;
    int adv_img, adv_y, adv_x;
    unsigned long long* prof;
    int s3;
    float* gn_partial;
    int gn_rows;
    int fastseg;
    int subpix;
};

__device__ __forceinline__ void seg_pack(int& img_pix, int& y_msk, int x, int h_in, int w_in) {
    const int img = img_pix, y = y_msk;
    unsigned m = 0;
#pragma unroll
    for (int k = 0; k < 3; ++k) {
        m |= (static_cast<unsigned>(y + k) < static_cast<unsigned>(h_in) ? 1u : 0u) << k;
        m |= (static_cast<unsigned>(x + k) < static_cast<unsigned>(w_in) ? 16u : 0u) << k;
    }
    img_pix = static_cast<int>((static_cast<unsigned>(img) * static_cast<unsigned>(h_in) + static_cast<unsigned>(y)) * static_cast<unsigned>(w_in) + static_cast<unsigned>(x));
    y_msk = static_cast<int>(m);
}

__device__ __forceinline__ long out_row(const GemmParams& p, long bz, int m) {
    if (!p.subpix) return m;
    const int q = m / p.w_out, x = m - q * p.w_out;
    return (2L * q + (bz >> 1)) * (2 * p.w_out) + 2 * x + (bz & 1);
}
__device__ __forceinline__ long gn_part(const GemmParams& p, long bz, int m) {
    if (!p.subpix) return m / p.gn_rows;
    const int img = m / p.rows_per_img, rem = m - img * p.rows_per_img, ppi = p.rows_per_img / p.gn_rows;
    return (static_cast<long>(img) * 4 + bz) * ppi + rem / p.gn_rows;
}

#ifdef PF_GEMM_TIMELINE
#define PF_TL(p, cond, slot) do { if ((cond) && (p).prof && threadIdx.x == 0) { const long b_ = blockIdx.x + static_cast<long>(gridDim.x) * (blockIdx.y + static_cast<long>(gridDim.y) * blockIdx.z); (p).prof[b_ * 32 + (slot)] = __builtin_amdgcn_s_memtime(); } } while (0)
#else
#define PF_TL(p, cond, slot) do { } while (0)
#endif
__device__ __forceinline__ void stamp(const GemmParams& p, int slot) {
    if (p.prof && threadIdx.x == 0) {
        const long b = blockIdx.x + static_cast<long>(gridDim.x) * (blockIdx.y + static_cast<long>(gridDim.y) * blockIdx.z);
        p.prof[b * 32 + slot] = __builtin_amdgcn_s_memtime();
    }
}

template <typename T>
__device__ __forceinline__ void epilogue_store(const GemmParams& p, long bz, int m, int n4, float (&v)[4]) {
    if (p.bias) {
        const float4 b = *reinterpret_cast<const float4*>(p.bias + n4);
        v[0] += b.x; v[1] += b.y; v[2] += b.z; v[3] += b.w;
    }
    if (p.rowvec) {
        const int img = m / p.rows_per_img;
        const float4 b = *reinterpret_cast<const float4*>(p.rowvec + static_cast<long>(img) * p.rowvec_ld + n4);
        v[0] += b.x; v[1] += b.y; v[2] += b.z; v[3] += b.w;
    }
    if (p.residual && p.res_f32) {
        const float4 r = *reinterpret_cast<const float4*>(static_cast<const float*>(p.residual) + bz * p.res_bs + static_cast<long>(m) * p.res_ld + n4);
        v[0] += r.x; v[1] += r.y; v[2] += r.z; v[3] += r.w;
    } else if (p.residual) {
        const u16x4 r = *reinterpret_cast<const u16x4*>(static_cast<const unsigned short*>(p.residual) + bz * p.res_bs + static_cast<long>(m) * p.res_ld + n4);
#pragma unroll
        for (int e = 0; e < 4; ++e) v[e] += to_f32<T>(r[e]);
    }
    if (p.geglu) {
        unsigned short* o = static_cast<unsigned short*>(p.out) + bz * p.out_bs + out_row(p, bz, m) * p.out_ld + (n4 >> 1);
        typedef __attribute__((ext_vector_type(2))) unsigned short u16x2;
        u16x2 w2;
#pragma unroll
        for (int e = 0; e < 2; ++e) {
            const float g = v[2 * e + 1];
            w2[e] = from_f32<T>(geglu_value(v[2 * e], g));
        }
        *reinterpret_cast<u16x2*>(o) = w2;
    } else if (p.split_out) {
        unsigned short* o = static_cast<unsigned short*>(p.out) + bz * p.out_bs + out_row(p, bz, m) * p.out_ld + n4;
        u16x4 hi, lo;
#pragma unroll
        for (int e = 0; e < 4; ++e) {
            hi[e] = from_f32<T>(v[e]);
            lo[e] = from_f32<T>(v[e] - to_f32<T>(hi[e]));
        }
        *reinterpret_cast<u16x4*>(o + (pair_off(n4) - n4)) = hi;
        *reinterpret_cast<u16x4*>(o + (pair_off(n4) - n4) + 32) = lo;
    } else if (p.out_f32) {
        float* o = static_cast<float*>(p.out) + bz * p.out_bs + out_row(p, bz, m) * p.out_ld + n4;
        *reinterpret_cast<float4*>(o) = float4{v[0], v[1], v[2], v[3]};
    } else {
        unsigned short* o = static_cast<unsigned short*>(p.out) + bz * p.out_bs + out_row(p, bz, m) * p.out_ld + n4;
        u16x4 w4;
// ... 57 lines not shown
```

### panfusion_amd/csrc/pf_gemm_plan.hip

```cpp
#include "pf_gemm_params.h"

namespace pf {

const GemmTuning& gemm_tuning() {
    static const GemmTuning t;
    return t;
}

void params_from_desc(const pf_conv_desc* d, GemmParams& p) {
    const int c1 = d->a1 ? d->c1 : 0;
    const int Ctot = d->c0 + c1;
    p.a0 = static_cast<const unsigned short*>(d->a0);
    p.a1 = static_cast<const unsigned short*>(d->a1);
    p.c0 = d->c0; p.c1 = c1; p.a0_ld = d->a0_ld; p.a1_ld = d->a1 ? d->a1_ld : 0;
    p.h_in = d->h_in; p.w_in = d->w_in; p.h_out = d->h_out; p.w_out = d->w_out;
    p.ksize = d->ksize; p.stride = d->stride; p.pad = d->pad; p.up = d->upsample;
    p.wrap = d->wrap_pad; p.crop = d->crop;
    p.w = static_cast<const unsigned short*>(d->w);
    p.rows_per_img = d->h_out * d->w_out;
    p.M = d->n_img * p.rows_per_img; p.N = d->n_out; p.K = d->ksize * d->ksize * Ctot;
    p.bias = d->bias; p.rowvec = d->rowvec; p.rowvec_ld = d->rowvec_ld;
    p.residual = d->residual; p.res_ld = d->res_ld;
    p.res_f32 = d->residual != nullptr && d->res_dtype == PF_F32;
    p.out = d->out; p.out_ld = d->out_ld; p.out_f32 = d->out_dtype == PF_F32;
    p.geglu = d->epilogue == PF_EPILOGUE_GEGLU;
    p.split_out = d->epilogue == PF_EPILOGUE_SPLIT;
    p.a_bs = d->a_bstride; p.w_bs = d->w_bstride; p.out_bs = d->out_bstride; p.res_bs = d->res_bstride;
    p.mtiles = p.ntiles = 0;
    p.prof = nullptr;
    p.s3 = d->split3 != 0;
    p.batch = d->batch;
    p.gn_partial = nullptr; p.gn_rows = 0;
    p.m_begin = 0; p.splits = 1; p.kb_per_split = 0; p.partial = nullptr; p.tickets = nullptr;
    p.a0_bytes = p.a1_bytes = p.w_bytes = 0; p.adv_img = p.adv_y = p.adv_x = 0;
    p.subpix = 0;
    p.fastseg = (d->upsample == 0 || d->subpixel) && d->wrap_pad == 0 && GemmTuning::conv_fastseg() ? 1 : 0;
    if (d->subpixel) {
        p.subpix = 1; p.ksize = 2; p.up = 0; p.pad = 0;
        p.h_out = d->h_out / 2; p.w_out = d->w_out / 2;
        p.rows_per_img = p.h_out * p.w_out;
        p.M = d->n_img * p.rows_per_img; p.K = 4 * Ctot;
        p.crop = d->crop / 2;
        p.batch = 4; p.a_bs = 0; p.out_bs = 0; p.res_bs = 0; p.w_bs = static_cast<long>(p.N) * p.K;
    }
}


static pf_conv_plan plan_small(long M, int N, int K, int batch, bool allow_split, bool s3) {
    const GemmTuning& t = gemm_tuning();
    pf_conv_plan g{};
    g.kernel = 0;
    g.nrep = (N % 160 == 0) ? 5 : 4;
    const long ntiles = cdiv(N, 32 * g.nrep);
    const long tiles128 = cdiv(M, 128) * ntiles * batch;
    g.mrep = tiles128 < 512 ? 2 : 4;
    g.block_rows = 32 * g.mrep;
    const long tiles = cdiv(M, 32 * g.mrep) * ntiles * batch;
    const int nkb = K / 64;
    g.splits = 1;
    g.kb_per_split = nkb;
    if (t.deep_ring && !s3 && tiles <= 256) {
        long s = allow_split && N % 4 == 0 && nkb >= t.split_min_kb ? 256 / tiles : 1;
        if (s > nkb / 4) s = nkb / 4;
        if (s > 32) s = 32;
        if (s > 1) {
            g.kb_per_split = static_cast<int>(cdiv(nkb, s));
            g.splits = static_cast<int>(cdiv(nkb, g.kb_per_split));
        }
        return g;
    }
    if (allow_split && N % 4 == 0 && tiles <= 320 && nkb >= t.split_min_kb) {
        long s = (640 + tiles - 1) / tiles;
        if (s > nkb / 6) s = nkb / 6;
        if (s > 32) s = 32;
        if (s > 1) {
            g.kb_per_split = static_cast<int>(cdiv(nkb, s));
            g.splits = static_cast<int>(cdiv(nkb, g.kb_per_split));
        }
    }
    return g;
}

static pf_conv_plan plan_big(int nrep, int K) {
    pf_conv_plan g{};
    g.kernel = 1; g.mrep = 8; g.nrep = nrep; g.block_rows = 256; g.splits = 1; g.kb_per_split = K / 64;
    return g;
}

static pf_conv_plan plan_tiles(long M, int N, int K, int batch, bool allow_split, bool s3) {
    const GemmTuning& t = gemm_tuning();
    const int nrep = (N % 160 == 0) ? 5 : 4;
    const long tiles256 = cdiv(M, 256) * cdiv(N, 32 * nrep) * batch;
    const long rounds = cdiv(tiles256, 256);
    const bool filled = tiles256 * 100 >= rounds * 256 * t.big_fill_pct;
    pf_conv_plan tail = plan_big(nrep, K);
    bool tail_ok = false;
    if (t.big_min_tiles > 0 && t.tail_split && allow_split && batch == 1 && N % 4 == 0 && tiles256 > 256 && K >= t.big_min_k &&
        K / 64 >= t.tail_min_kb) {
        const long ntl = cdiv(N, 32 * nrep), mt = cdiv(M, 256);
        const long rows1 = (tiles256 / 256) * 256 / ntl;
        const long tiles2 = (mt - rows1) * ntl;
        long sp = tiles2 > 0 ? (256 + tiles2 / 2) / tiles2 : 1;
        if (sp > (K / 64) / 8) sp = (K / 64) / 8;
        if (rows1 > 0 && tiles2 > 0 && sp >= 2 && rows1 * ntl * 100 >= (tiles256 / 256) * 256 * 90) {
            tail.m_split = static_cast<int>(rows1 * 256);
            tail.tail_kb = static_cast<int>(cdiv(K / 64, sp));
            tail.tail_splits = static_cast<int>(cdiv(K / 64, tail.tail_kb));
            tail_ok = true;
        }
    }
    if (tail_ok && tiles256 * 100 < rounds * 256 * t.tail_first_pct) return tail;
    if (t.big_min_tiles > 0 && tiles256 >= t.big_min_tiles && filled && K >= t.big_min_k) return plan_big(nrep, K);
    if (tail_ok) return tail;
    const int nkb_all = K / 64;
    if (t.big_min_tiles > 0 && allow_split && N % 4 == 0 && tiles256 >= 32 && tiles256 <= 128 && nkb_all >= 32) {
        long sp = 256 / tiles256;
        if (sp > nkb_all / 16) sp = nkb_all / 16;
        if (sp >= 2) {
            pf_conv_plan g = plan_big(nrep, K);
            g.kb_per_split = static_cast<int>(cdiv(nkb_all, sp));
            g.splits = static_cast<int>(cdiv(nkb_all, g.kb_per_split));
            return g;
        }
    }
    return plan_small(M, N, K, batch, allow_split, s3);
}

static bool takes_128_row_blocks(const pf_conv_plan& g, long M, int N, int K, int batch) {
    const GemmTuning& t = gemm_tuning();
    if (g.kernel != 1 || g.m_split > 0 || t.bm128 == 0) return false;
    if (t.bm128 == 1) return true;
    const long tiles256 = cdiv(M, 256) * cdiv(N, 32 * g.nrep) * batch * g.splits;
    return t.bm128 == 2 && (K <= t.bm128_max_k || (t.bm128_one_round && tiles256 <= 256));
}

static int gn_rows16(const GemmParams& p, const pf_conv_plan& g, int batch) {
    if ((batch != 1 && !p.subpix) || g.splits > 1 || g.m_split > 0 || p.geglu || p.split_out) return 0;
    if (p.residual && GemmTuning::gn_epilogue_res() == 0) return 0;
    if (g.kernel == 1 && gemm_tuning().big_waves == 4) return 0;
    const int rows = g.kernel == 1 ? 64 : 16 * g.mrep;
    const int BM = g.kernel == 1 ? 256 : 32 * g.mrep;
    if (p.rows_per_img % rows != 0 || p.N % (32 * g.nrep) != 0) return 0;
    if (p.out_f32) {
        const bool ok = !p.rowvec && (p.out_ld & 3) == 0 && (!p.residual || (p.res_f32 && (p.res_ld & 3) == 0));
        return ok ? rows : 0;
    }
    const bool staged = !p.res_f32 && (p.out_ld & 7) == 0 && (p.N & 7) == 0 && !(p.rowvec && p.residual) &&
                        !(p.rowvec && p.rows_per_img < BM);
    return staged ? rows : 0;
}


static bool plan32(const GemmParams& p, int batch, bool allow_split, pf_conv_plan& g) {
    const GemmTuning& t = gemm_tuning();
    if (!GemmTuning::gemm32() || p.s3 || p.subpix || batch != 1 || p.N % 320 != 0 || p.K < t.gemm32_min_k || p.K % 64 != 0 || p.geglu)
        return false;
    if (p.ksize != 3 && !t.gemm32_k1) return false;
    const int nkb = p.K / 64;
    g = pf_conv_plan{};
    g.kernel = 2; g.mrep = 8; g.nrep = 10; g.block_rows = 256; g.splits = 1; g.kb_per_split = nkb;
    const long ntl = p.N / 320, mt = cdiv(p.M, 256), tiles = mt * ntl;
    const long full = tiles / 256 * 256, rest = tiles - full;
    if (rest == 0) return true;
    if (full == 0 || !allow_split || p.N % 4 != 0) return false;
    const long rows1 = full / ntl;
    long sp = (256 + rest / 2) / rest;
    if (sp > nkb / 8) sp = nkb / 8;
    if (sp < 2 || rest * sp > 256) return false;
    g.m_split = static_cast<int>(rows1 * 256);
    g.tail_kb = static_cast<int>(cdiv(nkb, sp));
    g.tail_splits = static_cast<int>(cdiv(nkb, g.tail_kb));
    return true;
}
static int gn_rows32(const GemmParams& p, const pf_conv_plan& g) {
    if (g.m_split > 0 || p.residual || p.split_out || p.geglu) return 0;
    if (p.rows_per_img % 64 != 0) return 0;
    const bool ok = p.out_f32 ? (p.out_ld & 3) == 0 : (p.out_ld & 7) == 0;
    return ok ? 64 : 0;
}


pf_conv_plan plan_conv_gemm(const GemmParams& p, int batch, bool allow_split, bool want_moments) {
    const GemmTuning& t = gemm_tuning();
    pf_conv_plan g{};
    if (plan32(p, batch, allow_split, g) && (!want_moments || gn_rows32(p, g) > 0)) {
        g.gn_rows = want_moments ? 64 : 0;
        g.waves = 8; g.ring_slots = 4;
    } else {
        g = plan_tiles(p.M, p.N, p.K, batch, allow_split, p.s3 != 0);
        g.gn_rows = want_moments ? gn_rows16(p, g, batch) : 0;
        if (g.kernel == 1) {
            if (takes_128_row_blocks(g, p.M, p.N, p.K, batch)) { g.block_rows = 128; g.waves = 4; g.ring_slots = 2; }
            else { g.waves = t.big_waves == 4 && !p.s3 ? 4 : 8; g.ring_slots = 3; }
        } else {
            const long blocks = cdiv(p.M, g.block_rows) * cdiv(p.N, 32 * g.nrep) * g.splits * batch;
            const int deep_max = t.deep_ring ? t.deep_ring_max_blocks : 0;
            g.waves = 4;
            g.ring_slots = g.gn_rows == 0 && !p.s3 && blocks <= deep_max && p.K / 64 / g.splits >= 3 ? 4 : 2;
        }
    }
    const long rows2 = p.M - g.m_split;
    if (g.m_split > 0) g.workspace_bytes = static_cast<size_t>(g.tail_splits) * rows2 * p.N * sizeof(float);
    else if (g.splits > 1) g.workspace_bytes = static_cast<size_t>(g.splits) * batch * p.M * p.N * sizeof(float);
    if (g.workspace_bytes && g.kernel != 2) g.n_tickets = static_cast<int>(cdiv(rows2, g.block_rows) * cdiv(p.N, 32 * g.nrep) * batch);
    return g;
}

}

using namespace pf;

extern "C" pf_status pf_conv_gemm_plan(const pf_conv_desc* d, int want_moments, pf_conv_plan* out) {
    PF_REQUIRE(d && out, "pf_conv_gemm_plan: null pointer");
    PF_REQUIRE(d->batch >= 1 && d->n_out >= 1 && d->n_img >= 1, "pf_conv_gemm_plan: batch, n_out and n_img must be >= 1");
    GemmParams p;
    params_from_desc(d, p);
    *out = plan_conv_gemm(p, d->subpixel ? 4 : d->batch, true, want_moments != 0);
    return PF_OK;
}

extern "C" int pf_conv_gemm_gn_rows(const pf_conv_desc* d) {
    pf_conv_plan g;
    return pf_conv_gemm_plan(d, 1, &g) == PF_OK ? g.gn_rows : 0;
}

extern "C" int pf_conv_gemm_kernel_id(const pf_conv_desc* d) {
    pf_conv_plan g;
    return pf_conv_gemm_plan(d, 0, &g) == PF_OK ? g.kernel : -1;
}

extern "C" size_t pf_conv_gemm_workspace_size(const pf_conv_desc* d) {
    pf_conv_plan g0, g1;
    if (pf_conv_gemm_plan(d, 0, &g0) != PF_OK || pf_conv_gemm_plan(d, 1, &g1) != PF_OK) return 0;
    if (d->residual && g1.gn_rows == 0) return g0.workspace_bytes;
    return g0.workspace_bytes > g1.workspace_bytes ? g0.workspace_bytes : g1.workspace_bytes;
}
```

### panfusion_amd/engine.py

```python
import os
from types import SimpleNamespace as NS

import torch

from . import ops


def default_precision(dtype):
    env = os.environ.get("PF_PRECISION")
    if env in ("mixed", "fast"):
        return env
    return "mixed" if dtype == torch.float16 else "fast"


RAW_PAIR_FUSED = os.environ.get("PF_RAW_PAIR", "1") != "0"
VIRTUAL_PAD = os.environ.get("PF_VIRTUAL_PAD", "1") != "0"
EXACT_UP0 = os.environ.get("PF_EXACT_UP0", "1") != "0"
SUBPIXEL_UP = os.environ.get("PF_SUBPIXEL_UP", "1") != "0"
FUSED_HEAD = os.environ.get("PF_FUSED_HEAD", "1") != "0"


def stream_dtype(dtype, precision):
    return torch.float32 if precision == "mixed" else dtype


def _f32(t, dev):
    return t.detach().to(device=dev, dtype=torch.float32).contiguous()


def _w16(t, dev, dtype):
    return t.detach().to(device=dev, dtype=torch.float32).to(dtype).contiguous()


def _processor_lora(attn, name):
    proc = getattr(attn, "processor", None)
    lora = getattr(proc, name, None) if proc is not None else None
    if lora is not None and not (hasattr(lora, "down") and hasattr(lora, "up")):
        raise TypeError("%s.%s has no down / up matrices" % (type(proc).__name__, name))
    return lora


def _conv3_weight(conv, dev, dtype):
    return _w16(conv.weight.detach().float().permute(0, 2, 3, 1).reshape(conv.weight.shape[0], -1), dev, dtype)


def _subpixel_weight(conv, dev, dtype):
    w = conv.weight.detach().float()
    groups = (((0,), (1, 2)), ((0, 1), (2,)))
    phases = []
    for a in range(2):
        for b in range(2):
            taps = [[sum(w[:, :, ky, kx] for ky in groups[a][r] for kx in groups[b][c]) for c in range(2)] for r in range(2)]
            phases.append(torch.stack([torch.stack(row, 1) for row in taps], 1))
    return _w16(torch.stack(phases).reshape(4 * w.shape[0], -1), dev, dtype)


def _split_weight(w, taps, dev, dtype):
    w = w.detach().to(device=dev, dtype=torch.float32).reshape(w.shape[0], taps, -1, 32)
    hi = w.to(dtype)
    lo = (w - hi.float()).to(dtype)
    return torch.stack([hi, lo], 3).reshape(w.shape[0], -1).contiguous()


def split_operand(x0, x1=None, scale=None, shift=None, act=0, dtype=None):
    c = x0.shape[-1]
    n_img = scale.shape[0] if scale is not None else 1
    hw = x0.numel() // (c * n_img)
    return ops.scale_shift_act(x0, x1, n_img, hw, scale, shift, act, out_dtype=dtype, split=True)


def exact_gemm(a_split, w3, n_out, **kw):
    C2 = a_split.shape[-1]
    k = kw.get("ksize", 1)
    return ops.conv_gemm(a_split, w3, n_out, c0=C2, a0_ld=C2, algo_k=k * k * (C2 // 2), split3=True, **kw)


def to16(x, dtype):
    if x.dtype == dtype:
        return x
    c = x.shape[-1]
    return ops.scale_shift_act(x, None, 1, x.numel() // c, None, None, 0, out_dtype=dtype).view(x.shape)


def _norm(n, dev):
    return NS(g=_f32(n.weight, dev), b=_f32(n.bias, dev), eps=float(n.eps),
              groups=getattr(n, "num_groups", None))


def _bias(m, dev):
    return None if m.bias is None else _f32(m.bias, dev)


def pack_resnet(res, dev, dtype, mixed=False):
    r = NS()
    r.dtype, r.stream = dtype, (torch.float32 if mixed else dtype)
    r.cin, r.cout = res.conv1.weight.shape[1], res.conv1.weight.shape[0]
    r.norm1, r.norm2 = _norm(res.norm1, dev), _norm(res.norm2, dev)
    r.w1, r.b1 = _conv3_weight(res.conv1, dev, dtype), _bias(res.conv1, dev)
    r.w2, r.b2 = _conv3_weight(res.conv2, dev, dtype), _bias(res.conv2, dev)
    sc = getattr(res, "conv_shortcut", None)
    r.ws3 = None
    if sc is not None:
        r.ws = _w16(sc.weight.detach().float().reshape(r.cout, r.cin), dev, dtype)
        r.bs = _bias(sc, dev)
        if mixed:
            r.ws3 = _split_weight(sc.weight.detach().float().reshape(r.cout, r.cin), 1, dev, dtype)
    else:
        r.ws = r.bs = None
    r.temb = getattr(res, "time_emb_proj", None)
    r.src = res
    return r


def pack_resnet_plain(res, dev, dtype, mixed=False):
    r = pack_resnet(res, dev, dtype, mixed)
    del r.temb
    return r


def run_resnet_plain(r, x):
    return run_resnet(r, x, None, None)


def _current_lora(attn, name, lin):
    own = getattr(lin, "lora_layer", None)
    proc = _processor_lora(attn, name + "_lora")
    if own is not None and proc is not None:
        raise ValueError("LoRA weights found both in <linear>.lora_layer and in the attention processor")
    return own if own is not None else proc


def _dev32(t, dev):
    t = t.detach()
    if t.dtype == torch.float32 and t.device == torch.device(dev) and t.is_contiguous():
        return t
    return t.to(device=dev, dtype=torch.float32).contiguous()


def pack_attention(attn, dev, dtype, self_attn):
    a = NS()
    a.heads, a.src, a.dtype, a.self_attn = attn.heads, attn, dtype, self_attn
    Cc, Dk = attn.to_q.weight.shape[0], attn.to_k.weight.shape[1]
    a.dim = Cc
    buf = lambda rows, cols: torch.empty(rows, cols, device=dev, dtype=dtype)
    if self_attn:
        a.wqkv = buf(3 * Cc, Cc)
        a.wqk, a.wv = a.wqkv[:2 * Cc], a.wqkv[2 * Cc:]
        dst = {"to_q": a.wqkv[:Cc], "to_k": a.wqkv[Cc:2 * Cc], "to_v": a.wv}
    else:
        a.wq, a.wkv = buf(Cc, Cc), buf(2 * Cc, Dk)
        a.wk, a.wv = a.wkv[:Cc], a.wkv[Cc:]
# ... 140 lines not shown
                      c=m.weight.shape[0])
    c.zero_down = [zc(m) for m in cn.controlnet_down_blocks]
    c.zero_mid = zc(cn.controlnet_mid_block)
    return c


def run_cond_embedding(c, cond):
    n, _, H, W = cond.shape
    dev = cond.device
    key = (n, H, W, str(dev))
    bufs = c.ce_bufs.get(key)
    if bufs is None:
        bufs = [torch.zeros(n, H, W, c.ce_c0, device=dev, dtype=c.dtype)]
        h, w = H, W
        for L in c.ce_layers:
            h, w = (h - 1) // L.stride + 1, (w - 1) // L.stride + 1
            bufs.append(torch.zeros(n, h, w, _pad64(L.cout), device=dev, dtype=c.dtype))
        c.ce_bufs[key] = bufs
    x = ops.conv_in(cond.float(), c.ce_w0, c.ce_b0, c.ce_c0, c.dtype, wrap=False, out=bufs[0])
    x = ops.silu(x, out=x)
    h, w = H, W
    for i, L in enumerate(c.ce_layers):
        out = bufs[i + 1]
        ops.conv_gemm(x, L.w, L.cout, n_img=n, h_in=h, w_in=w, ksize=3, stride=L.stride, pad=1, bias=L.b,
                      c0=L.cin_pad, out=out.view(-1, out.shape[-1]))
        if i + 1 < len(c.ce_layers):
            out = ops.silu(out, out=out)
        x, h, w = out, out.shape[1], out.shape[2]
    return x


def run_controlnet(c, latent, timestep, text, cond, make_branch=None, embed=None, rec=None):
    br = (make_branch or Branch)(c, latent, timestep, text, pano=False, pad=False)
    br.h = ops.add(br.h, (embed or run_cond_embedding)(c, cond))
    br.skips = [br.h]
    for blk in c.down:
        for j, r in enumerate(blk.resnets):
            br.resnet(r)
            if blk.attns is not None:
                br.attention(blk.attns[j])
            br.push()
        if blk.down is not None:
            br.downsample(blk.down)
            br.push()
    br.resnet(c.mid.resnets[0])
    for a, r in zip(c.mid.attns, c.mid.resnets[1:]):
        br.attention(a)
        br.resnet(r)

    def zero_conv(z, x):
        n, h, w, Cc = x.shape
        return ops.conv_gemm(to16(x, c.dtype), z.w, z.c, n_img=n, h_in=h, w_in=w, ksize=1, bias=z.b).view(n, h, w, z.c)

    if rec is not None:
        rec.br, rec.skips, rec.h_mid = br, list(br.skips), br.h
    return [zero_conv(z, s) for z, s in zip(c.zero_down, br.skips)], zero_conv(c.zero_mid, br.h)


def pack_epa(block, dev, dtype, mixed=False):
    tr = block.transformer
    e = NS()
    e.cdtype, e.stream = dtype, (torch.float32 if mixed else dtype)
    e.dim = tr.norm1.weight.shape[0]
    e.heads = e.dim // 32
    e.ln1, e.ln2 = _norm(tr.norm1, dev), _norm(tr.norm2, dev)
    a = tr.attn1
    e.wqkv = _w16(torch.cat([a.to_q.weight.detach().float(), a.to_k.weight.detach().float(), a.to_v.weight.detach().float()], 0), dev, dtype)
    e.wqk, e.wv = e.wqkv[:2 * e.dim], e.wqkv[2 * e.dim:]
    e.wo, e.bo = _w16(a.to_out.weight, dev, dtype), _bias(a.to_out, dev)
    e.w_ff1, e.b_ff1 = ops.interleave_geglu(_w16(tr.ff.net[0].proj.weight, dev, dtype), _bias(tr.ff.net[0].proj, dev))
    e.w_ff2, e.b_ff2 = _w16(tr.ff.net[2].weight, dev, dtype), _bias(tr.ff.net[2], dev)
    e.freq = _f32(block.pe.freq_bands, dev)
    return e


def run_resnet(r, x, skip, temb_all, groups_eps=None, wrap=0, save=None):
    n, h, w, _ = x.shape
    hw = h * w
    sc, sh = ops.groupnorm_scale_shift(x, skip, n, hw, r.norm1.groups, r.norm1.eps, r.norm1.g, r.norm1.b,
                                       wrap=(w, wrap) if wrap else None)
    if save is not None:
        save.sc1, save.sh1 = sc, sh
    pair = None
    if r.ws3 is not None and x.dtype == torch.float32 and RAW_PAIR_FUSED:
        y, pair = ops.scale_shift_act(x, skip, n, hw, sc, sh, 1, out_dtype=r.dtype, raw_pair=True)
    else:
        y = ops.scale_shift_act(x, skip, n, hw, sc, sh, 1, out_dtype=r.dtype)
    rowvec = temb_all[:, r.temb_off:] if temb_all is not None else None
    wp = w + 2 * wrap
    h1 = ops.conv_gemm(y, r.w1, r.cout, n_img=n, h_in=h, w_in=w, ksize=3, pad=1, bias=r.b1, rowvec=rowvec, gn_stats=True,
                       wrap_pad=wrap, out_dtype=torch.float32 if save is not None else None)
    h1 = ops.carry(h1.view(n, h * wp, r.cout), h1)
    sc, sh = ops.groupnorm_scale_shift(h1, None, n, h * wp, r.norm2.groups, r.norm2.eps, r.norm2.g, r.norm2.b)
    if save is not None:
        save.h1, save.sc2, save.sh2 = h1, sc, sh
    y2 = ops.scale_shift_act(h1, None, n, h * wp, sc, sh, 1, out_dtype=r.dtype)
    if r.ws3 is not None:
        if pair is None:
            pair = split_operand(x, skip, dtype=r.dtype)
        short = exact_gemm(pair, r.ws3, r.cout, w_in=n * hw, bias=r.bs, out_dtype=r.stream)
    elif r.ws is not None:
        short = ops.conv_gemm(x, r.ws, r.cout, a1=skip, n_img=n, h_in=h, w_in=w, ksize=1, bias=r.bs)
    else:
        short = x.view(n * hw, r.cout)
    out = ops.conv_gemm(y2, r.w2, r.cout, n_img=n, h_in=h, w_in=wp, ksize=3, pad=1, bias=r.b2, residual=short, gn_stats=True,
                        crop=wrap)
    return ops.carry(out.view(n, h, w, r.cout), out)


def text_kv(a, text):
    n, L = text.shape[:2]
    return ops.linear(text.reshape(n * L, -1), a.wk), ops.linear_t(text, a.wv)


def all_transformers(u):
    for blk in [*u.down, u.mid, *u.up]:
        for t in (blk.attns or []):
            yield t


def self_qkv(a, tokens, n, nk):
    fused = ops.linear_qkv(tokens, a.wqkv, n)
    if fused is not None:
        return fused
    qk = ops.linear(tokens, a.wqk)
    vt = ops.linear_vt(tokens, a.wv, n)
    if vt is None:
        vt = ops.linear_t(tokens.view(n, nk, -1), a.wv)
    return qk, vt


def _attend(a, q_src, kv_tokens, n, nq, nk, head_dim, *, self_attn, residual, kv=None, next_ln=None, split=None):
    Cq = a.dim
    vt = None
    if split is not None and self_attn and n == 1:
        from . import sharding
        o = sharding.split_pano_attention(split, a, q_src, nq)
        if next_ln is not None:
            return ops.linear_ln(o.view(n * nq, Cq), a.wo, a.bo, residual, next_ln.g, next_ln.b, next_ln.eps)
        return ops.linear(o.view(n * nq, Cq), a.wo, bias=a.bo, residual=residual)
    if self_attn:
        qk, vt = self_qkv(a, q_src, n, nk)
        q, k, ld = qk, qk[:, Cq:], 2 * Cq
    else:
        q, ld = ops.linear(q_src, a.wq), Cq
        k = kv[0] if kv is not None else ops.linear(kv_tokens, a.wk)
    if kv is not None:
        vt = kv[1]
    elif vt is None:
        vt = ops.linear_t(kv_tokens.view(n, nk, -1), a.wv)
    o = ops.attention(q, k, vt, n, a.heads, head_dim, nq, nk,
                      q_ld=ld, k_ld=(ld if self_attn else Cq), vt_ld=vt.shape[-1],
                      q_bs=nq * ld, k_bs=nk * (ld if self_attn else Cq), vt_bs=vt.shape[1] * vt.shape[2])
    if next_ln is not None:
        return ops.linear_ln(o.view(n * nq, Cq), a.wo, a.bo, residual, next_ln.g, next_ln.b, next_ln.eps)
    return ops.linear(o.view(n * nq, Cq), a.wo, bias=a.bo, residual=residual)


def run_transformer(t, x, text, kv=None, split=None):
    n, h, w, Cc = x.shape
    hw = h * w
    sc, sh = ops.groupnorm_scale_shift(x, None, n, hw, t.norm.groups, t.norm.eps, t.norm.g, t.norm.b)
    if t.w_in3 is not None:
        tok = exact_gemm(split_operand(x, None, sc, sh, 0, dtype=t.dtype), t.w_in3, Cc, w_in=n * hw, bias=t.b_in,
                         out_dtype=t.stream)
    else:
        y = ops.scale_shift_act(x, None, n, hw, sc, sh, 0)
        tok = ops.linear(y.view(n * hw, Cc), t.w_in, bias=t.b_in)
    dh = t.attn1.dim // t.attn1.heads
    ln = ops.layernorm(tok, t.ln1.g, t.ln1.b, t.ln1.eps, out_dtype=t.dtype)
    tok, ln = _attend(t.attn1, ln, ln, n, hw, hw, dh, self_attn=True, residual=tok, next_ln=t.ln2, split=split)
    if ln is None:
        ln = ops.layernorm(tok, t.ln2.g, t.ln2.b, t.ln2.eps, out_dtype=t.dtype)
    L = text.shape[1]
    tok, ln = _attend(t.attn2, ln, text.reshape(n * L, -1), n, hw, L, dh, self_attn=False, residual=tok, kv=kv, next_ln=t.ln3)
    if ln is None:
        ln = ops.layernorm(tok, t.ln3.g, t.ln3.b, t.ln3.eps, out_dtype=t.dtype)
    g = ops.linear(ln, t.w_ff1, bias=t.b_ff1, geglu=True)
    if t.w_out3 is not None and os.environ.get("PF_FF2_PAIR", "1") != "0":
        pair = ops.linear(g, t.w_ff2, bias=t.b_ff2, residual=tok, split_out=True)
        out = exact_gemm(pair, t.w_out3, Cc, w_in=n * hw, bias=t.b_out, residual=x.view(n * hw, Cc), gn_stats=True)
    elif t.w_out3 is not None:
        tok = ops.linear(g, t.w_ff2, bias=t.b_ff2, residual=tok)
        out = exact_gemm(split_operand(tok, dtype=t.dtype), t.w_out3, Cc, w_in=n * hw, bias=t.b_out, residual=x.view(n * hw, Cc),
                         gn_stats=True)
    else:
        tok = ops.linear(g, t.w_ff2, bias=t.b_ff2, residual=tok)
        out = ops.linear(tok, t.w_out, bias=t.b_out, residual=x.view(n * hw, Cc), gn_stats=True)
    return ops.carry(out.view(n, h, w, Cc), out)


class Branch:

    def __init__(self, u, latent, timestep, text, pano, pad):
        self.u, self.text, self.pad = u, text, (pano and pad)
        n = latent.shape[0]
        feats = ops.timestep_features(timestep, u.t_dim, u.dtype)
        e = ops.linear(feats, u.w_t1, bias=u.b_t1)
        e = ops.linear(ops.silu(e), u.w_t2, bias=u.b_t2)
        self.temb = ops.linear(ops.silu(e), u.w_temb, bias=u.b_temb, out_dtype=torch.float32)
        self.h = ops.conv_in(latent.float(), u.w_conv_in, u.b_conv_in, u.c0, u.stream, wrap=self.pad)
        self.skips = [self.h]
        self.text_kv = {}
        self.text_ready = None
        self.attn_split = None
        self.attn_help = None
        self.split_streams = None
        self.keep = None

    def precompute_text_kv(self):
        key = (self.text.data_ptr(), self.text._version, tuple(self.text.shape), self.text.dtype, str(self.text.device))
        cache = self.u.__dict__.setdefault("text_kv_cache", {})
        hit = cache.get(key)
        if hit is None:
            if len(cache) >= 4:
                victim = next((ck for ck, h in cache.items() if not h.get("pins")), None)
                if victim is not None:
                    cache.pop(victim)
            hit = {id(t): text_kv(t.attn2, self.text) for t in all_transformers(self.u)}
            hit["text"] = self.text
            cache[key] = hit
        self.text_kv = hit

    def _padded(self, t, p):
        return ops.pad_width(t, p) if (self.pad and t is not None) else t

    def resnet(self, r, skip=False, save=None):
        s = self.skips.pop() if skip else None
        if self.pad and VIRTUAL_PAD:
            self.h = run_resnet(r, self.h, s, self.temb, wrap=2, save=save)
        elif self.pad:
            out = run_resnet(r, self._padded(self.h, 2), self._padded(s, 2), self.temb, save=save)
            self.h = ops.crop_width(out, 2)
        else:
            self.h = run_resnet(r, self.h, s, self.temb, save=save)

    def attention(self, t):
        if self.text_ready is not None:
            torch.cuda.current_stream(self.h.device).wait_event(self.text_ready)
            self.text_ready = None
        split = None
        if self.attn_split is not None:
            from . import sharding
            if sharding.splits_pano_attention(self.attn_split, self.h.shape[1] * self.h.shape[2]) and self.h.shape[0] == 1:
                split = self.attn_split
        if split is not None and self.split_streams is not None:
            main, side = self.split_streams
            main.wait_stream(side)
# ... 255 lines not shown
```

### panfusion_amd/ops.py

```python
import ctypes as C
import os

import numpy as np
import torch

from . import _lib
from ._lib import PF_BF16, PF_F16, PF_F32, AttnBwdDesc, AttnDesc, ConvDesc, ConvPlan, LinearWsDesc, check

_DT = {torch.bfloat16: PF_BF16, torch.float16: PF_F16, torch.float32: PF_F32}

TRACE = None


class _PlanCache(__import__("threading").local):
    LIMIT = 4096

    def __init__(self):
        self.plans = {}


_PLANS = _PlanCache()
SPLITK_INKERNEL = os.environ.get("PF_SPLITK_INKERNEL") == "1"


# ... 381 lines not shown
    if x0_out is None:
        x0_out = torch.empty_like(x)
    assert x.is_contiguous() and out.is_contiguous() and x0_out.is_contiguous() and (out2 is None or out2.is_contiguous())
    assert x0_prev is None or (x0_prev.is_contiguous() and x0_prev.dtype == torch.float32 and x0_prev.numel() == x.numel())
    assert x0_out.dtype == torch.float32 and x0_out.numel() == x.numel()
    assert tstep is None or (tstep.dtype == torch.int64 and tstep.is_contiguous())
    sa, sb, sap, sbp = (float(c) for c in coef)
    check(_lib.lib().pf_cfg_dpmpp_step_pair(_p(x), _p(eps_uncond), _p(eps_cond), float(guidance), sa, sb, sap, sbp,
                                            rows, W, int(roll), _p(out), _p(out2) if out2 is not None else None,
                                            _p(tstep) if tstep is not None else None, tstep.numel() if tstep is not None else 0,
                                            int(t_next), _p(x0_prev) if x0_prev is not None else None, float(k), _p(x0_out),
                                            _stream()), "pf_cfg_dpmpp_step_pair")
    return out, x0_out


def cfg_inpaint_step_pair(x, eps_uncond, eps_cond, guidance, coef, roll=0, out=None, out2=None, tstep=None, t_next=0,
                          x0_prev=None, k=0.0, x0_out=None, *, known, noise, mask, ka, kb, known_roll=0):
    W = x.shape[-1]
    rows = x.numel() // W
    if out is None:
        out = torch.empty_like(x)
    assert x.is_contiguous() and out.is_contiguous() and (out2 is None or out2.is_contiguous())
    assert x0_out is None or (x0_out.is_contiguous() and x0_out.dtype == torch.float32 and x0_out.numel() == x.numel())
    assert x0_prev is None or (x0_prev.is_contiguous() and x0_prev.dtype == torch.float32 and x0_prev.numel() == x.numel())
    for t in (known, noise, mask):
        assert t is None or (t.is_contiguous() and t.dtype == torch.float32 and t.numel() == x.numel())
    assert tstep is None or (tstep.dtype == torch.int64 and tstep.is_contiguous())
    sa, sb, sap, sbp = (float(c) for c in coef)
    opt = lambda t: _p(t) if t is not None else None
    check(_lib.lib().pf_cfg_inpaint_step_pair(_p(x), _p(eps_uncond), _p(eps_cond), float(guidance), sa, sb, sap, sbp,
                                              rows, W, int(roll), _p(out), opt(out2), opt(tstep),
                                              tstep.numel() if tstep is not None else 0, int(t_next), opt(x0_prev), float(k),
                                              opt(x0_out), opt(known), opt(noise), opt(mask), float(ka), float(kb),
                                              int(known_roll), _stream()), "pf_cfg_inpaint_step_pair")
    return out, x0_out


def noised_start_pair(z, noise, ka, kb, roll=0, *, out, out2=None, tstep=None, t0=0):
    W = noise.shape[-1]
    rows = noise.numel() // W
    for t in (z, noise, out, out2):
        assert t is None or (t.is_contiguous() and t.dtype == torch.float32 and t.numel() == noise.numel())
    assert tstep is None or (tstep.dtype == torch.int64 and tstep.is_contiguous())
    opt = lambda t: _p(t) if t is not None else None
    check(_lib.lib().pf_noised_start_pair(opt(z), _p(noise), float(ka), float(kb), rows, W, int(roll), _p(out), opt(out2),
                                          opt(tstep), tstep.numel() if tstep is not None else 0, int(t0), _stream()),
          "pf_noised_start_pair")
    return out


RESIZE_MODES = {"nearest": 0, "bilinear": 1, "bicubic": 2}


def upsampled_start_pair(z, noise, ka, kb, roll=0, *, mode, wrap, out, out2=None, tstep=None, t0=0):
    if mode not in RESIZE_MODES:
        raise ValueError("resample mode must be one of %s, got %r" % (sorted(RESIZE_MODES), mode))
    (h, w), (H, W) = z.shape[-2:], out.shape[-2:]
    planes = z.numel() // (h * w)
    assert tuple(z.shape[:-2]) == tuple(out.shape[:-2]), (z.shape, out.shape)
    for t in (z, noise, out, out2):
        assert t is None or (t.is_contiguous() and t.dtype == torch.float32)
    for t in (noise, out2):
        assert t is None or t.numel() == out.numel()
    assert tstep is None or (tstep.dtype == torch.int64 and tstep.is_contiguous())
    opt = lambda t: _p(t) if t is not None else None
    check(_lib.lib().pf_upsampled_start_pair(_p(z), opt(noise), float(ka), float(kb), planes, h, w, H, W, RESIZE_MODES[mode],
                                             int(bool(wrap)), int(roll), _p(out), opt(out2), opt(tstep),
                                             tstep.numel() if tstep is not None else 0, int(t0), _stream()),
          "pf_upsampled_start_pair")
    return out


def resize_latent(x, size, mode="bicubic", wrap=False, out=None):
    if out is None:
        out = torch.empty(tuple(x.shape[:-2]) + tuple(size), device=x.device, dtype=torch.float32)
    assert tuple(out.shape[-2:]) == tuple(size)
    return upsampled_start_pair(x, None, 0.0, 0.0, 0, mode=mode, wrap=wrap, out=out)


def conv_gemm(a0, w, n_out, *, a1=None, n_img=1, h_in=1, w_in=None, ksize=1, stride=1, pad=0, upsample=0,
              bias=None, rowvec=None, residual=None, out=None, out_dtype=None, batch=1,
              a_bstride=0, w_bstride=0, out_bstride=0, res_bstride=0, a0_ld=None, a1_ld=None, c0=None, c1=None,
              out_ld=None, res_ld=None, geglu=False, algo_k=None, split_out=False, pad_hi=0, gn_stats=False,
              wrap_pad=0, crop=0, split3=False, plan_only=False, subpixel=False):
    c0 = c0 if c0 is not None else a0.shape[-1]
    c1 = (c1 if c1 is not None else a1.shape[-1]) if a1 is not None else 0
    if w_in is None:
        w_in = a0.numel() // (a0.shape[-1] * max(batch, 1)) if ksize == 1 else None
    hl, wl = h_in << upsample, (w_in + 2 * wrap_pad) << upsample
    h_out = (hl + 2 * pad + pad_hi - ksize) // stride + 1
    w_out = (wl + 2 * pad + pad_hi - ksize) // stride + 1 - 2 * crop
    M = n_img * h_out * w_out
    if out is not None:
        out_dtype = out.dtype
    if split_out:
        out_dtype = a0.dtype
    out_dtype = out_dtype or (residual.dtype if residual is not None else a0.dtype)
    n_store = n_out // 2 if geglu else (2 * n_out if split_out else n_out)
    if out is None:
        out = torch.empty((batch, M, n_store) if batch > 1 else (M, n_store), device=a0.device, dtype=out_dtype)
    a0_ld = a0_ld if a0_ld is not None else _ld(a0)
    a1_ld = (a1_ld if a1_ld is not None else _ld(a1)) if a1 is not None else 0
    rowvec_ld = _ld(rowvec) if rowvec is not None else 0
    res_ld = (res_ld if res_ld is not None else _ld(residual)) if residual is not None else 0
    res_dtype = dt(residual) if residual is not None else dt(a0)
    out_ld = out_ld if out_ld is not None else _ld(out)
    epilogue = 1 if geglu else (2 if split_out else 0)
    pkey = (c0, c1, a0_ld, a1_ld, n_img, h_in, w_in, h_out, w_out, ksize, stride, pad, upsample, n_out, batch, epilogue, wrap_pad,
            crop, dt(a0), dt(out_dtype), residual is not None, res_dtype, res_ld, rowvec is not None, rowvec_ld, bias is not None,
            out_ld, a_bstride, w_bstride, out_bstride, res_bstride, bool(split3), bool(subpixel))
    plans = _PLANS.plans
    plan = plans.get(pkey)
    if plan is None:
        d = _conv_desc(pkey)
        d.a0, d.a1, d.w, d.bias, d.rowvec, d.residual, d.out = _p(a0), _p(a1), _p(w), _p(bias), _p(rowvec), _p(residual), _p(out)
        if len(plans) >= _PLANS.LIMIT:
            plans.pop(next(iter(plans)))
        plan = plans[pkey] = [d, _conv_plan(d, 0), None]
    d = plan[0]
    if plan_only:
        return plan[1].kernel
    d.a0, d.a1, d.w, d.bias, d.rowvec, d.residual, d.out = _p(a0), _p(a1), _p(w), _p(bias), _p(rowvec), _p(residual), _p(out)
    d.gn_partial, d.gn_rows, d.tickets, d.n_tickets = None, 0, None, 0
    g, gn = plan[1], None
    if gn_stats and GN_FROM_EPILOGUE and batch == 1:
        if plan[2] is None:
            plan[2] = _conv_plan(d, 1)
        if plan[2].gn_rows > 0:
            g = plan[2]
            gn = (torch.empty(M // g.gn_rows, 2, n_out // 2, device=a0.device, dtype=torch.float32), g.gn_rows)
            d.gn_partial, d.gn_rows = _p(gn[0]), g.gn_rows
    nbytes = g.workspace_bytes
    ws = torch.empty(nbytes, device=a0.device, dtype=torch.uint8) if nbytes else None
    d.workspace, d.workspace_bytes = _p(ws), nbytes
    if nbytes and SPLITK_INKERNEL:
        d.tickets, d.n_tickets = _ticket_slice(a0.device), _TICKET_SLICE
    if TRACE is None:
        check(_lib.lib().pf_conv_gemm(C.byref(d), _stream()), "pf_conv_gemm")
    else:
        _traced("k_conv_gemm", 2.0 * M * n_out * (algo_k or ksize * ksize * (c0 + c1)) * batch,
                lambda: check(_lib.lib().pf_conv_gemm(C.byref(d), _stream()), "pf_conv_gemm"),
                "M%d N%d K%d k%d s%d u%d b%d%s" % (M, n_out, ksize * ksize * (c0 + c1), ksize, stride, upsample, batch, " g32" if plan[1].kernel == 2 else " subpixel" if subpixel else ""))
    if gn is not None:
        out._pf_gn = gn
    elif hasattr(out, "_pf_gn"):
        del out._pf_gn
    return out


def _conv_desc(pkey):
    d = ConvDesc()
    (d.c0, d.c1, d.a0_ld, d.a1_ld, d.n_img, d.h_in, d.w_in, d.h_out, d.w_out, d.ksize, d.stride, d.pad, d.upsample, d.n_out, d.batch,
     d.epilogue, d.wrap_pad, d.crop, d.dtype, d.out_dtype, _, d.res_dtype, d.res_ld, _, d.rowvec_ld, _, d.out_ld,
     d.a_bstride, d.w_bstride, d.out_bstride, d.res_bstride, d.split3, d.subpixel) = pkey
    return d


def _conv_plan(d, want_moments):
    g = ConvPlan()
    check(_lib.lib().pf_conv_gemm_plan(C.byref(d), want_moments, C.byref(g)), "pf_conv_gemm_plan")
    return g


def gemm_workspace_bytes(a0, w, n_out, *, a1=None, n_img=1, h_in=1, w_in=None, ksize=1, stride=1, pad=0,
                         upsample=0, batch=1, wrap_pad=0, crop=0, subpixel=False, **_):
    c0, c1 = a0.shape[-1], (a1.shape[-1] if a1 is not None else 0)
    if w_in is None:
        w_in = a0.numel() // (a0.shape[-1] * max(batch, 1))
    h_out = ((h_in << upsample) + 2 * pad - ksize) // stride + 1
    w_out = (((w_in + 2 * wrap_pad) << upsample) + 2 * pad - ksize) // stride + 1 - 2 * crop
    d = _conv_desc((c0, c1, c0, c1, n_img, h_in, w_in, h_out, w_out, ksize, stride, pad, upsample, n_out, batch, 0, wrap_pad, crop,
                    dt(a0), dt(a0), False, dt(a0), 0, False, 0, False, n_out, 0, 0, 0, 0, False, bool(subpixel)))
    d.a1 = _p(a1)
    return max(_conv_plan(d, 0).workspace_bytes, _conv_plan(d, 1).workspace_bytes)


LWS_16, LWS_F32, LWS_GEGLU, LWS_QKV, LWS_F32_LN, LWS_VT = 0, 1, 2, 3, 4, 5
LINEAR_WS = os.environ.get("PF_LINEAR_WS", "1") != "0"
LINEAR_WS_K640 = os.environ.get("PF_LINEAR_WS_K640", "1") != "0"
LINEAR_WS_K1280 = os.environ.get("PF_LINEAR_WS_K1280", "1") != "0"
LINEAR_VT = os.environ.get("PF_LINEAR_VT", "1") != "0"
LINEAR_WS_MIN_ROWS = int(os.environ.get("PF_LINEAR_WS_MIN_ROWS", "8192"))


def linear_ws_ok(rows, N, K, mode, x=None):
    if not LINEAR_WS or rows < LINEAR_WS_MIN_ROWS:
        return False
    if K == 640:
        if not LINEAR_WS_K640 or not ((N % 256 == 0 and mode in (LWS_16, LWS_GEGLU)) or (N % 128 == 0 and mode in (LWS_16, LWS_VT))):
            return False
    elif K == 1280:
        if not LINEAR_WS_K1280 or N % 128 or mode not in (LWS_16, LWS_GEGLU, LWS_VT):
            return False
    elif K != 320 or N % 320:
        return False
    elif N == 320 and rows < 4 * LINEAR_WS_MIN_ROWS:
        return False
    if x is not None and (x.dtype not in (torch.float16, torch.bfloat16) or x.stride(-1) != 1 or x.stride(-2) % 8):
        return False
    return bool(_lib.lib().pf_linear_ws_supported(rows, N, K, mode))


def linear_ws(x, w, mode, bias=None, residual=None, out=None, out_vt=None, rows_per_batch=0, ln=None):
    rows, K = x.shape
    N = w.shape[0]
    d = LinearWsDesc()
    ln_out = None
    if mode == LWS_F32_LN:
        ln_out = torch.empty(rows, N, device=x.device, dtype=x.dtype)
        d.ln_gamma, d.ln_beta, d.ln_eps, d.ln_out, d.ln_ld = _p(ln[0]), _p(ln[1]), float(ln[2]), _p(ln_out), N
    if mode == LWS_QKV:
        nb = rows // rows_per_batch
        if out is None:
            out = torch.empty(rows, 640, device=x.device, dtype=x.dtype)
        if out_vt is None:
            out_vt = torch.empty(nb, 320, rows_per_batch, device=x.device, dtype=x.dtype)
        d.out_vt, d.vt_ld, d.rows_per_batch, d.vt_bs = _p(out_vt), out_vt.stride(1), rows_per_batch, out_vt.stride(0)
    elif mode == LWS_VT:
        nb = rows // rows_per_batch
        if out_vt is None:
            out_vt = torch.empty(nb, N, rows_per_batch, device=x.device, dtype=x.dtype)
        d.out_vt, d.vt_ld, d.rows_per_batch, d.vt_bs = _p(out_vt), out_vt.stride(1), rows_per_batch, out_vt.stride(0)
    elif out is None:
        out = torch.empty(rows, N // 2 if mode == LWS_GEGLU else N, device=x.device,
                          dtype=torch.float32 if mode in (LWS_F32, LWS_F32_LN) else x.dtype)
    d.a, d.a_ld, d.w, d.bias = _p(x), _ld(x), _p(w), _p(bias)
    d.residual, d.res_ld = _p(residual), (_ld(residual) if residual is not None else 0)
    for buf in (out, out_vt):
        if buf is not None:
            _written(buf)
    d.out, d.out_ld = _p(out), (_ld(out) if out is not None else 0)
    d.M, d.N, d.K, d.dtype, d.mode = rows, N, K, dt(x), mode
    if TRACE is None:
        check(_lib.lib().pf_linear_ws(C.byref(d), _stream()), "pf_linear_ws")
    else:
        _traced("k_linear_ws", 2.0 * rows * N * K, lambda: check(_lib.lib().pf_linear_ws(C.byref(d), _stream()), "pf_linear_ws"),
                "M%d N%d K%d mode%d" % (rows, N, K, mode))
    return (out, out_vt) if mode == LWS_QKV else (out, ln_out) if mode == LWS_F32_LN else out_vt if mode == LWS_VT else out


def linear_vt(x, w, n_batch):
    rows, K = x.shape
    nk = rows // n_batch
    if not LINEAR_VT:
        return None
    if nk * n_batch != rows or nk % (16 if K == 1280 else 32 if K == 640 else 64) or not w.is_contiguous() or not linear_ws_ok(rows, w.shape[0], K, LWS_VT, x):
        return None
    return linear_ws(x, w, LWS_VT, rows_per_batch=nk)


def linear_ln(x, w, bias, residual, gamma, beta, eps):
    rows, K = x.shape
    if (w.shape[0] == 320 and x.dim() == 2 and w.is_contiguous() and residual is not None and residual.dtype == torch.float32
            and linear_ws_ok(rows, 320, K, LWS_F32_LN, x) and os.environ.get("PF_LINEAR_LN", "1") != "0"):
        return linear_ws(x, w, LWS_F32_LN, bias=bias, residual=residual, ln=(gamma, beta, eps))
# ... 299 lines not shown
```

### panfusion_amd/train_engine.py

```python
import torch

from . import engine, ops, training

import os

NS = engine.NS
F32 = torch.float32
EXACT = os.environ.get("PF_TRAIN_EXACT", "1") != "0"
KEEP = os.environ.get("PF_TRAIN_KEEP", "1") != "0"
TWO_STREAMS = os.environ.get("PF_TRAIN_STREAMS", "1") != "0"


def flip_conv3_weight(w, dtype):
    w = w.detach().float()
    return w.flip(2, 3).permute(1, 2, 3, 0).reshape(w.shape[1], -1).to(dtype).contiguous()


def conv_out_dgrad_weight(w):
    return w.detach().float().flip(2, 3).permute(2, 3, 0, 1).contiguous()


def _t16(w, dev, dtype):
    return w.detach().to(device=dev, dtype=F32).t().to(dtype).contiguous()

# ... 450 lines not shown
        g_n, b_n = gn_param_grads(t.norm, x, None, n, hw, sc, sh, 0, dy.view(n, hw, Cc))
        put(src.norm.weight, g_n)
        put(src.norm.bias, b_n)
    dx, _ = ops.groupnorm_bwd(x, None, n, hw, t.norm.groups, t.norm.eps, t.norm.g, sc, sh, 0, dy.view(n, hw, Cc), dres=d.view(n, hw, Cc))
    return _unscale(dx, state).view(n, h, w, Cc)


class ScaledSink:

    def __init__(self, sink, state):
        self.sink, self.state = sink, state


def downsample_backward(d, dout, pano_pad, dev_dtype, wsink=None, x=None):
    tw = getattr(d, "train", None)
    cin = d.src.weight.shape[1]
    if tw is None:
        wflip = d.src.weight.detach().float().flip(2, 3).permute(1, 2, 3, 0).reshape(cin, -1)
        tw = d.train = NS(w=wflip.to(device=dout.device, dtype=dev_dtype).contiguous(), w3=None)
        if EXACT:
            tw.w3 = engine._split_weight(wflip, 9, dout.device, dev_dtype)
    g, state = _normalise(dout)
    if pano_pad:
        g = ops.crop_width_bwd(g, 1)
    if wsink is not None:
        assert not pano_pad and x is not None
        put = _scaled(wsink, state)
        put(d.src.weight, conv3_wgrad(engine.to16(g, dev_dtype), engine.to16(x, dev_dtype), stride=2))
        put(d.src.bias, ops.colsum(g.view(-1, g.shape[-1])))
    if tw.w3 is not None:
        n, ho, wo, cout = g.shape
        z = ops.zero_insert2(engine.split_operand(g, dtype=dev_dtype).view(n, ho, wo, 2 * cout))
        dx = engine.exact_gemm(z, tw.w3, cin, n_img=n, h_in=2 * ho, w_in=2 * wo, ksize=3, pad=1, out_dtype=F32).view(n, 2 * ho, 2 * wo, cin)
    else:
        dx = conv3_dgrad(g, tw.w, cin, "s2", dev_dtype)
    if pano_pad:
        dx = ops.pad_width_bwd(dx, 2)
    return _unscale(dx, state)


def upsample_backward(up, dout, pano_pad, dev_dtype):
    tw = getattr(up, "train", None)
    if tw is None:
        tw = up.train = NS(w=flip_conv3_weight(up.src.weight, dev_dtype))
    g, state = _normalise(dout)
    if pano_pad:
        g = ops.crop_width_bwd(g, 2)
    dx = conv3_dgrad(g, tw.w.to(dout.device), up.src.weight.shape[1], "up", dev_dtype)
    if pano_pad:
        dx = ops.pad_width_bwd(dx, 1)
    return _unscale(dx, state)


def head_backward(u, hin, d_eps, pano_pad):
    n, h, w, Cc = hin.shape
    tw = getattr(u, "train_head", None)
    if tw is None:
        tw = u.train_head = NS(w=conv_out_dgrad_weight(u.src_conv_out.weight).to(hin.device))
    g, state = _normalise(d_eps.float().contiguous())
    sc, sh = ops.groupnorm_scale_shift(hin, None, n, h * w, u.norm_out.groups, u.norm_out.eps, u.norm_out.g, u.norm_out.b)
    dy = conv_out_dgrad(g, tw.w, Cc, bool(pano_pad))
    dx, _ = ops.groupnorm_bwd(hin, None, n, h * w, u.norm_out.groups, u.norm_out.eps, u.norm_out.g, sc, sh, 1, dy.view(n, h * w, Cc))
    return _unscale(dx, state).view(n, h, w, Cc)


class TrainBranch(engine.Branch):

    def __init__(self, tape, *args, **kw):
        super().__init__(*args, **kw)
        self.tape = tape

    def resnet(self, r, skip=False):
        x, s = self.h, (self.skips[-1] if skip else None)
        saved = NS() if KEEP else None
        super().resnet(r, skip, save=saved)
        self.tape.append(("resnet", self, r, x, s, saved))

    def attention(self, t):
        x = self.h
        rec = None
        if KEEP:
            self.h, rec = transformer_forward_keep(t, x, self.text)
        else:
            super().attention(t)
        self.tape.append(("attention", self, t, x, rec))

    def push(self):
        super().push()
        self.tape.append(("push", self))

    def downsample(self, d):
        x = self.h
        super().downsample(d)
        self.tape.append(("down", self, d, x))

    def upsample(self, up):
        super().upsample(up)
        self.tape.append(("up", self, up))

    def head(self):
        x = self.h
        out = super().head()
        self.tape.append(("head", self, x))
        return out


class ParamGrads:

    def __init__(self):
        self.grads = {}

    def __call__(self, param, grad, scale=1.0):
        g = grad.reshape(param.shape).to(F32)
        if scale != 1.0:
            g = g * scale
        key = id(param)
        if key in self.grads:
            self.grads[key] = (param, ops.add(self.grads[key][1].contiguous(), g.contiguous()))
        else:
            self.grads[key] = (param, g)

    def get(self, param):
        hit = self.grads.get(id(param))
        return None if hit is None else hit[1].to(device=param.device, dtype=param.dtype)


def _trains(refs):
    return any(r is not None and (r.up.requires_grad or r.down.requires_grad) for r in refs)


def _first_trainable_entry(tape):
    for i, entry in enumerate(tape):
        kind = entry[0]
        if kind in ("cn_skips", "cn_mid"):
            return i
        if kind == "fuse" and any(p_.requires_grad for p_ in training.train_params(entry[3])):
            return i
        if kind == "attention":
            tw = transformer_train(entry[2], entry[3].device)
            groups = (tw.attn1.lora_qkv, tw.attn1.lora_out, tw.attn2.lora_q, tw.attn2.lora_kv, tw.attn2.lora_out)
            if any(_trains(g.refs) for g in groups):
                return i
    return None


def backward(tape, d_eps, sink, dh=None, dskips=None, wsink=None, dtemb=None, side=None):
    import contextlib
    dh = {} if dh is None else dh
    dskips = {} if dskips is None else dskips
    main = torch.cuda.current_stream() if side is not None else None
    crossing = []
    if side is not None:
        side.wait_stream(main)

    def stream_of(br):
        return torch.cuda.stream(side) if (side is not None and getattr(br, "on_side", False)) else contextlib.nullcontext()
    first = 0 if wsink is not None else _first_trainable_entry(tape)
    if first is None:
        return dh, dskips
    for index in range(len(tape) - 1, first - 1, -1):
        entry = tape[index]
        kind, br = entry[0], entry[1]
        if kind == "cn_mid":
            entry[2].d_mid = dh[br]
            continue
        if kind == "cn_skips":
            with stream_of(br):
# ... 218 lines not shown
```

Measured before the change: 16.74 steps/s.

## Fuse fp32 source split and GroupNorm affine into conv GEMM A staging

Adds an fp32-source mode (A32) to the conv GEMM kernels. In this mode the kernel loads fp32 activations directly, optionally applies the per-image GroupNorm scale/shift, and splits each value into hi/lo half-precision parts while writing to LDS. This replaces the separate split_operand pass that materialized the hi/lo pair buffer before the exact (split3) GEMMs in resnet shortcuts and transformer proj_in. It saves a full read/write of the activation but moves register-staged loads and conversion math into the GEMM pipeline, which can cost occupancy or pipelining, and some plan shapes are excluded.

New measurement: 16.97 steps/s (median of 6 runs). +1.4%, better.

```diff
diff --git a/include/panfusion_hip.h b/include/panfusion_hip.h
--- a/include/panfusion_hip.h
+++ b/include/panfusion_hip.h
@@ -169,6 +169,9 @@
     int split3;
     int subpixel;
     int gn_rows;
+    int a_src_dtype;
+    const float* a_scale;
+    const float* a_shift;
 } pf_conv_desc;
 
 enum { PF_EPILOGUE_NONE = 0, PF_EPILOGUE_GEGLU = 1, PF_EPILOGUE_SPLIT = 2 };
diff --git a/panfusion_amd/_lib.py b/panfusion_amd/_lib.py
--- a/panfusion_amd/_lib.py
+++ b/panfusion_amd/_lib.py
@@ -26,6 +26,7 @@
         ("epilogue", c_int), ("workspace", c_void_p), ("workspace_bytes", c_size_t),
         ("gn_partial", c_void_p), ("wrap_pad", c_int), ("crop", c_int),
         ("tickets", c_void_p), ("n_tickets", c_int), ("split3", c_int), ("subpixel", c_int), ("gn_rows", c_int),
+        ("a_src_dtype", c_int), ("a_scale", c_void_p), ("a_shift", c_void_p),
     ]
 
 
diff --git a/panfusion_amd/csrc/pf_common.h b/panfusion_amd/csrc/pf_common.h
--- a/panfusion_amd/csrc/pf_common.h
+++ b/panfusion_amd/csrc/pf_common.h
@@ -75,6 +75,19 @@
 
 __host__ __device__ __forceinline__ int pair_off(int c) { return ((c >> 5) << 6) | (c & 31); }
 
+__device__ __forceinline__ float affine_f(float v, float scale, float shift) {
+    float r = __builtin_fmaf(v, scale, shift);
+    asm("" : "+v"(r));
+    return r;
+}
+template <typename T> __device__ __forceinline__ void split8(const float (&f)[8], u16x8& hi, u16x8& lo) {
+    hi = pack8<T>(f);
+    float r[8];
+#pragma unroll
+    for (int j = 0; j < 8; ++j) r[j] = f[j] - to_f32<T>(hi[j]);
+    lo = pack8<T>(r);
+}
+
 __device__ __forceinline__ float silu_f(float x) { return x / (1.0f + __expf(-x)); }
 
 template <typename S> __device__ __forceinline__ float ld_any(const void* p, long i);
diff --git a/panfusion_amd/csrc/pf_elementwise.hip b/panfusion_amd/csrc/pf_elementwise.hip
--- a/panfusion_amd/csrc/pf_elementwise.hip
+++ b/panfusion_amd/csrc/pf_elementwise.hip
@@ -301,12 +301,10 @@
         if (j0 + u >= per_img) break;
         if (raw_pair) {
             unsigned short* y = raw_pair + pix[u] * (2 * C) + pair_off(cc[u]);
-            const u16x8 hi = pack8<T>(v[u]);
-            float lo[8];
-#pragma unroll
-            for (int j = 0; j < 8; ++j) lo[j] = v[u][j] - to_f32<T>(hi[j]);
+            u16x8 hi, lo;
+            split8<T>(v[u], hi, lo);
             *reinterpret_cast<u16x8*>(y) = hi;
-            *reinterpret_cast<u16x8*>(y + 32) = pack8<T>(lo);
+            *reinterpret_cast<u16x8*>(y + 32) = lo;
         }
         float f[8];
         if (scale) {
@@ -316,7 +314,7 @@
             const float sv[8] = {s0.x, s0.y, s0.z, s0.w, s1.x, s1.y, s1.z, s1.w};
             const float hv[8] = {h0.x, h0.y, h0.z, h0.w, h1.x, h1.y, h1.z, h1.w};
 #pragma unroll
-            for (int j = 0; j < 8; ++j) f[j] = v[u][j] * sv[j] + hv[j];
+            for (int j = 0; j < 8; ++j) f[j] = affine_f(v[u][j], sv[j], hv[j]);
         } else {
 #pragma unroll
             for (int j = 0; j < 8; ++j) f[j] = v[u][j];
@@ -329,12 +327,10 @@
             *reinterpret_cast<u16x8*>(static_cast<unsigned short*>(yv) + pix[u] * C + cc[u]) = pack8<T>(f);
         } else if (OUT == 1) {
             unsigned short* y = static_cast<unsigned short*>(yv) + pix[u] * (2 * C) + pair_off(cc[u]);
-            const u16x8 hi = pack8<T>(f);
-            float lo[8];
-#pragma unroll
-            for (int j = 0; j < 8; ++j) lo[j] = f[j] - to_f32<T>(hi[j]);
+            u16x8 hi, lo;
+            split8<T>(f, hi, lo);
             *reinterpret_cast<u16x8*>(y) = hi;
-            *reinterpret_cast<u16x8*>(y + 32) = pack8<T>(lo);
+            *reinterpret_cast<u16x8*>(y + 32) = lo;
         } else {
             store8_f32(static_cast<float*>(yv) + pix[u] * C + cc[u], f);
         }
diff --git a/panfusion_amd/csrc/pf_gemm.hip b/panfusion_amd/csrc/pf_gemm.hip
--- a/panfusion_amd/csrc/pf_gemm.hip
+++ b/panfusion_amd/csrc/pf_gemm.hip
@@ -442,9 +442,10 @@
     if (t == 0) __hip_atomic_store(ticket, 0, __ATOMIC_RELAXED, __HIP_MEMORY_SCOPE_AGENT);
 }
 
-template <typename T, int MREP, int NREP, bool STATS = false, bool S3 = false, int STAGES = 2>
+template <typename T, int MREP, int NREP, bool STATS = false, bool S3 = false, int STAGES = 2, bool A32 = false>
 __global__ __launch_bounds__(256, STAGES > 2 ? 1 : 2) void k_conv_gemm(const GemmParams p) {
     constexpr int BM = 32 * MREP, BN = 32 * NREP;
+    static_assert(!A32 || (S3 && STAGES == 2 && MREP % 2 == 0), "fp32-source staging: split-precision walk, two slots");
     extern __shared__ __attribute__((aligned(16))) unsigned short smem[];
     unsigned short* As = smem;
     unsigned short* Bs = smem + STAGES * BM * 64;
@@ -513,6 +514,7 @@
         const int ky = p.ksize == 3 ? tap / 3 : p.ksize == 2 ? tap >> 1 : 0, kx = p.ksize == 3 ? tap - 3 * ky : p.ksize == 2 ? tap & 1 : 0;
         seg1 = __builtin_amdgcn_readfirstlane(cc >= p.c0 ? 1 : 0) != 0;
         const int ld = seg1 ? p.a1_ld : p.a0_ld;
+        if constexpr (A32) return;
         if (p.fastseg) {
             const unsigned sel = (1u << ky) | (16u << kx);
             const int tap_pix = ky * p.w_in + kx;
@@ -539,13 +541,49 @@
     auto lds_dma = [&](const __amdgpu_buffer_rsrc_t& r, unsigned short* dst, unsigned voff, int soff) {
         __builtin_amdgcn_raw_ptr_buffer_load_lds(r, (__attribute__((address_space(3))) void*)dst, 16, voff, soff, 0, 0);
     };
+    constexpr int NP32 = A32 ? MREP / 2 : 1;
+    const int c4 = t & 3, r32 = t >> 2;
+    f32x4 xr[NP32][2], sr[NP32][2], hr[NP32][2];
+    auto a32_load = [&](const __amdgpu_buffer_rsrc_t& rs_a, int soff_a) {
+        const int ld = seg1 ? p.a1_ld : p.a0_ld;
+#pragma unroll
+        for (int u = 0; u < NP32; ++u) {
+            const int m = m0 + 64 * u + r32;
+            const unsigned voff = m < p.M ? (static_cast<unsigned>(m) * static_cast<unsigned>(ld) + 8u * c4) * 4u : OOB;
+            xr[u][0] = __builtin_bit_cast(f32x4, __builtin_amdgcn_raw_buffer_load_b128(rs_a, voff, soff_a, 0));
+            xr[u][1] = __builtin_bit_cast(f32x4, __builtin_amdgcn_raw_buffer_load_b128(rs_a, voff + 16u, soff_a, 0));
+            if (p.a_scale) {
+                const long so = static_cast<long>(min(m, p.M - 1) / p.rows_per_img) * (Ctot >> 1) + (cc >> 1) + 8 * c4;
+                sr[u][0] = *reinterpret_cast<const f32x4*>(p.a_scale + so); sr[u][1] = *reinterpret_cast<const f32x4*>(p.a_scale + so + 4);
+                hr[u][0] = *reinterpret_cast<const f32x4*>(p.a_shift + so); hr[u][1] = *reinterpret_cast<const f32x4*>(p.a_shift + so + 4);
+            }
+        }
+    };
+    auto a32_write = [&](int buf) {
+#pragma unroll
+        for (int u = 0; u < NP32; ++u) {
+            float f[8];
+#pragma unroll
+            for (int j = 0; j < 8; ++j) f[j] = xr[u][j >> 2][j & 3];
+            if (p.a_scale) {
+#pragma unroll
+                for (int j = 0; j < 8; ++j) f[j] = affine_f(f[j], sr[u][j >> 2][j & 3], hr[u][j >> 2][j & 3]);
+            }
+            u16x8 hi, lo;
+            split8<T>(f, hi, lo);
+            unsigned short* dst = As + buf * BM * 64;
+            *reinterpret_cast<u16x8*>(dst + lds_off(64 * u + r32, c4)) = hi;
+            *reinterpret_cast<u16x8*>(dst + lds_off(64 * u + r32, c4 + 4)) = lo;
+        }
+    };
     auto dma_stage = [&](int buf) {
         const int soff_a = __builtin_amdgcn_readfirstlane((seg1 ? cc - p.c0 : cc) * 2);
         const int soff_w = __builtin_amdgcn_readfirstlane(kg * 2);
         const __amdgpu_buffer_rsrc_t rs_a = __builtin_amdgcn_make_buffer_rsrc(
             uniform_ptr(seg1 ? a1 : a0), 0, __builtin_amdgcn_readfirstlane(seg1 ? p.a1_bytes : p.a0_bytes), 0x00020000);
-#pragma unroll
-        for (int i = 0; i < MREP; ++i) {
+        if constexpr (A32) a32_load(rs_a, soff_a);
+#pragma unroll
+        for (int i = 0; i < (A32 ? 0 : MREP); ++i) {
             unsigned short* dst = As + buf * BM * 64 + (i * 32 + wave * 8) * 64;
             lds_dma(rs_a, dst, a_off[i], soff_a);
         }
@@ -616,12 +654,14 @@
     if constexpr (STAGES == 2) {
         dma_stage(0);
         asm volatile("s_waitcnt vmcnt(0)" ::: "memory");
+        if constexpr (A32) a32_write(0);
         __syncthreads();
         stamp(p, 1);
         for (int kb = kb0, it = 0; kb < kb1; ++kb, ++it) {
             if (kb + 1 < kb1) dma_stage((it + 1) & 1);
             compute(it & 1);
             asm volatile("s_waitcnt vmcnt(0)" ::: "memory");
+            if constexpr (A32) { if (kb + 1 < kb1) a32_write((it + 1) & 1); }
             __syncthreads();
         }
     } else {
@@ -667,7 +707,7 @@
     stamp(p, 3);
 }
 
-template <typename T, int NREP, int NW, bool STATS = false, bool S3 = false, int BM_ = 256>
+template <typename T, int NREP, int NW, bool STATS = false, bool S3 = false, int BM_ = 256, bool A32 = false, bool AFF = false>
 __global__ __launch_bounds__(64 * NW, BM_ == 128 ? 2 : 1) void k_conv_gemm8(const GemmParams p) {
     constexpr int NT = 64 * NW, WMG = NW / 2, BM = BM_, BN = 32 * NREP, MREP = BM / (16 * WMG), STAGES = BM_ == 128 ? 2 : 3;
     constexpr bool ONEWAVE = NW == 4 && BM_ == 256;
@@ -695,6 +735,12 @@
     const int hchunk8 = (chunk ^ ((hrow >> 1) & 7)) * 8;
 
     constexpr int APASS = BM / RPP;
+    static_assert(!A32 || (S3 && APASS == 4 && BM * 4 == NT * 2), "fp32-source staging: two octets = four 16-byte loads per thread and stage");
+    struct XR { f32x4 x[2][2], s[2], h[2]; int cc; };
+    XR xq;
+    const int c4 = t & 3, r32 = 2 * (t >> 2);
+    unsigned x_off[2];
+    int x_sidx = 0;
     int a_img[APASS], a_y[APASS], a_x[APASS];
     constexpr unsigned OOB = 0x80000000u;
     auto uniform_ptr = [](const unsigned short* ptr) __attribute__((always_inline)) {
@@ -723,6 +769,14 @@
         const int ky = p.ksize == 3 ? tap / 3 : p.ksize == 2 ? tap >> 1 : 0, kx = p.ksize == 3 ? tap - 3 * ky : p.ksize == 2 ? tap & 1 : 0;
         seg1 = __builtin_amdgcn_readfirstlane(cc >= p.c0 ? 1 : 0) != 0;
         const int ld = seg1 ? p.a1_ld : p.a0_ld;
+        if constexpr (A32) {
+#pragma unroll
+            for (int u = 0; u < 2; ++u) {
+                const int m = m0 + r32 + u;
+                x_off[u] = m < p.M ? (static_cast<unsigned>(m) * static_cast<unsigned>(ld) + 8u * c4) * 4u : OOB;
+            }
+            return;
+        }
         if (p.fastseg) {
             const unsigned sel = (1u << ky) | (16u << kx);
             const int tap_pix = ky * p.w_in + kx;
@@ -786,6 +840,9 @@
         kg = kb0 * 64;
         tap = kg / Ctot;
         cc = kg - tap * Ctot;
+        if constexpr (A32) {
+            if constexpr (AFF) x_sidx = (min(m0 + r32, p.M - 1) / p.rows_per_img) * (Ctot >> 1) + 8 * c4;
+        }
         set_segment();
 #ifdef PF_GEMM_BDIRECT
         kw = kb0 * 64;
@@ -814,10 +871,16 @@
     auto lds_dma = [&](const __amdgpu_buffer_rsrc_t& r, unsigned short* dst, unsigned voff, int soff) __attribute__((always_inline)) {
         __builtin_amdgcn_raw_ptr_buffer_load_lds(r, (__attribute__((address_space(3))) void*)dst, 16, voff, soff, 0, 0);
     };
-    auto dma_piece = [&](const __amdgpu_buffer_rsrc_t& rs_a, int slot, int k) __attribute__((always_inline)) {
+    auto dma_piece = [&](const __amdgpu_buffer_rsrc_t& rs_a, int slot, int k, XR& q) __attribute__((always_inline)) {
         unsigned short* As = smem + slot * STAGE;
         unsigned short* Bs = As + BM * 64;
         if (k < APASS) {
+            if constexpr (A32) {
+                const int u = k >> 1, hf = k & 1;
+                q.x[u][hf] = __builtin_bit_cast(f32x4, __builtin_amdgcn_raw_buffer_load_b128(rs_a, x_off[u] + 16u * hf, st_soff_a, 0));
+                if (k == 0) q.cc = cc;
+                return;
+            }
             unsigned short* dst = As + (k * RPP + wave * 8) * 64;
             lds_dma(rs_a, dst, a_off[k], st_soff_a);
 #ifdef PF_GEMM_BDIRECT
@@ -830,11 +893,39 @@
             if (lane < 32) lds_dma(rs_w, Bs + (BFULL * RPP + wave * 4) * 64, w_off[BFULL], st_soff_w);
         }
     };
-    auto dma_stage = [&](int slot) __attribute__((always_inline)) {
+    auto dma_stage = [&](int slot, XR& q) __attribute__((always_inline)) {
         const __amdgpu_buffer_rsrc_t rs_a = stage_begin();
 #pragma unroll
-        for (int k = 0; k < NPIECE; ++k) dma_piece(rs_a, slot, k);
+        for (int k = 0; k < NPIECE; ++k) dma_piece(rs_a, slot, k, q);
         stage_end();
+    };
+    auto a32_affine = [&](XR& q) __attribute__((always_inline)) {
+        if constexpr (A32 && AFF) {
+            const int so = x_sidx + (q.cc >> 1);
+#pragma unroll
+            for (int hf = 0; hf < 2; ++hf) {
+                q.s[hf] = *reinterpret_cast<const f32x4*>(p.a_scale + so + 4 * hf);
+                q.h[hf] = *reinterpret_cast<const f32x4*>(p.a_shift + so + 4 * hf);
+            }
+        }
+    };
+    auto a32_write = [&](int slot, const XR& q) __attribute__((always_inline)) {
+        unsigned short* As = smem + slot * STAGE;
+#pragma unroll
+        for (int u = 0; u < 2; ++u) {
+            float f[8];
+#pragma unroll
+            for (int j = 0; j < 8; ++j) f[j] = q.x[u][j >> 2][j & 3];
+            if constexpr (AFF) {
+#pragma unroll
+                for (int j = 0; j < 8; ++j) f[j] = affine_f(f[j], q.s[j >> 2][j & 3], q.h[j >> 2][j & 3]);
+            }
+            u16x8 hi, lo;
+            split8<T>(f, hi, lo);
+            const int row = r32 + u;
+            *reinterpret_cast<u16x8*>(As + lds_off(row, c4)) = hi;
+            *reinterpret_cast<u16x8*>(As + lds_off(row, c4 + 4)) = lo;
+        }
     };
 
     f32x4 acc[MREP][NREP];
@@ -890,8 +981,22 @@
     };
 
     auto issue_prologue = [&]() __attribute__((always_inline)) {
-        dma_stage(0);
-        if (n_it > 1) dma_stage(1);
+        if constexpr (A32 && STAGES == 3) {
+            XR q0;
+            dma_stage(0, q0);
+            a32_affine(q0);
+            if (n_it > 1) { dma_stage(1, xq); a32_affine(xq); }
+            a32_write(0, q0);
+            if (n_it > 1) a32_write(1, xq);
+        } else if constexpr (A32) {
+            dma_stage(0, xq);
+            a32_affine(xq);
+            a32_write(0, xq);
+            if (n_it > 1) { dma_stage(1, xq); a32_affine(xq); }
+        } else {
+            dma_stage(0, xq);
+            if (n_it > 1) dma_stage(1, xq);
+        }
     };
     const std::true_type YES;
     const std::false_type NO;
@@ -914,6 +1019,13 @@
 #else
             if (idx == FLEAD - 1) {
                 __builtin_amdgcn_sched_barrier(0);
+                if constexpr (A32) {
+                    constexpr bool PEND = STAGES == 3 ? WAIT != 0 : MORE;
+                    if constexpr (PEND) {
+                        a32_write(STAGES == 3 ? nx2 : nx1, xq);
+                        __builtin_amdgcn_sched_barrier(0);
+                    }
+                }
 #ifndef PF_ABL_NOLDS
                 load_frags(cur, 1, fa1, fb1, 0);
 #endif
@@ -923,6 +1035,8 @@
         }
         if constexpr (S3) __builtin_amdgcn_sched_barrier(0);
         if constexpr (MORE) {
+            if constexpr (A32 && WAIT != 0) asm volatile("s_waitcnt vmcnt(%0) lgkmcnt(0)" :: "n"(WAIT) : "memory");
+            else
 #ifdef PF_GEMM_BDIRECT
             if constexpr (true) asm volatile("s_waitcnt vmcnt(0) lgkmcnt(0)" ::: "memory");
 #else
@@ -950,11 +1064,12 @@
                     const int k = idx - LEAD;
                     if (k >= 0 && (k & 1) == 0 && (k >> 1) < NPIECE) {
                         __builtin_amdgcn_sched_barrier(0);
-                        dma_piece(rs_a, cur, k >> 1);
+                        dma_piece(rs_a, cur, k >> 1, xq);
                         __builtin_amdgcn_sched_barrier(0);
                     }
                 }
             }
+            if constexpr (DMA) { __builtin_amdgcn_sched_barrier(0); a32_affine(xq); }
             if (MORE) { __builtin_amdgcn_sched_barrier(0); load_frags_a(nx1, 0, fa0); __builtin_amdgcn_sched_barrier(0); }
 #pragma unroll
             for (int j = 0; j < NREP; ++j) {
@@ -992,7 +1107,7 @@
 #ifdef PF_ABL_NODMA_B
                     if ((k >> 1) < APASS)
 #endif
-                    dma_piece(rs_a, cur, k >> 1);
+                    dma_piece(rs_a, cur, k >> 1, xq);
 #endif
                     __builtin_amdgcn_sched_barrier(0);
                 }
@@ -1032,6 +1147,8 @@
 #pragma unroll
             for (int j = 0; j < NREP; ++j) acc[i][j] = f32x4{0.f, 0.f, 0.f, 0.f};
         if (first && n_it > 1) {
+            if constexpr (A32) asm volatile("s_waitcnt vmcnt(%0)" :: "n"(NPIECE - APASS) : "memory");
+            else
 #ifdef PF_GEMM_BDIRECT
             if constexpr (true) asm volatile("s_waitcnt vmcnt(0)" ::: "memory");
 #else
@@ -1046,16 +1163,17 @@
         } else {
             asm volatile("s_waitcnt vmcnt(0)" ::: "memory");
         }
+        if constexpr (A32) asm volatile("s_waitcnt lgkmcnt(0)" ::: "memory");
         __builtin_amdgcn_s_barrier();
         asm volatile("" ::: "memory");
         if (first) stamp(p, 1);
         first = false;
         PF_TL(p, tl_tile == 1, 13);
-        if constexpr (STAGES == 3) { if (n_it > 2) dma_stage(2); }
+        if constexpr (STAGES == 3) { if (n_it > 2) { dma_stage(2, xq); a32_affine(xq); } }
         load_frags(0, 0, fa0, fb0, 0);
         cur = 0; nx1 = 1; nx2 = 2 % STAGES;
         PF_TL(p, tl_tile == 1, 14);
-        const std::integral_constant<int, NPIECE> W1;
+        const std::integral_constant<int, A32 ? NPIECE - APASS : NPIECE> W1;
         const std::integral_constant<int, 0> W0;
         if constexpr (STAGES == 3) {
             for (int it = 0; it + 3 < n_it; ++it) step(YES, YES, W1);
@@ -1155,14 +1273,14 @@
 }
 
 
-template <typename T, int MREP, int NREP, bool STATS, bool S3, int STAGES>
+template <typename T, int MREP, int NREP, bool STATS, bool S3, int STAGES, bool A32 = false>
 static pf_status launch_ring(const GemmParams& p, int batch, hipStream_t st) {
     constexpr int BM = 32 * MREP, BN = 32 * NREP;
     const size_t smem = static_cast<size_t>(STAGES) * (BM + BN) * 64 * sizeof(unsigned short);
     static std::atomic<unsigned long long> lds_set{0};
-    const pf_status s = allow_dynamic_lds(reinterpret_cast<const void*>(k_conv_gemm<T, MREP, NREP, STATS, S3, STAGES>), smem, lds_set, "pf_conv_gemm");
+    const pf_status s = allow_dynamic_lds(reinterpret_cast<const void*>(k_conv_gemm<T, MREP, NREP, STATS, S3, STAGES, A32>), smem, lds_set, "pf_conv_gemm");
     if (s != PF_OK) return s;
-    hipLaunchKernelGGL((k_conv_gemm<T, MREP, NREP, STATS, S3, STAGES>), dim3(p.mtiles * p.ntiles, p.splits, batch), dim3(256), smem, st, p);
+    hipLaunchKernelGGL((k_conv_gemm<T, MREP, NREP, STATS, S3, STAGES, A32>), dim3(p.mtiles * p.ntiles, p.splits, batch), dim3(256), smem, st, p);
     PF_CHECK_LAUNCH("pf_conv_gemm");
     return PF_OK;
 }
@@ -1178,6 +1296,9 @@
     if constexpr (!STATS && !S3) {
         if (g.ring_slots == 4) return launch_ring<T, MREP, NREP, false, false, 4>(p, batch, st);
     }
+    if constexpr (S3) {
+        if (p.a32) return launch_ring<T, MREP, NREP, STATS, true, 2, true>(p, batch, st);
+    }
     return launch_ring<T, MREP, NREP, STATS, S3, 2>(p, batch, st);
 }
 
@@ -1187,7 +1308,7 @@
     return gp.gn_partial ? launch_s<T, MREP, NREP, true>(g, gp, batch, st) : launch_s<T, MREP, NREP, false>(g, gp, batch, st);
 }
 
-template <typename T, int NREP, int NW, bool STATS = false, bool S3 = false, int BM = 256>
+template <typename T, int NREP, int NW, bool STATS = false, bool S3 = false, int BM = 256, bool A32 = false, bool AFF = false>
 static pf_status launch8w_s(const GemmParams& gp, int batch, hipStream_t st) {
     constexpr int BN = 32 * NREP, STAGES = BM == 128 ? 2 : 3;
     GemmParams p = gp;
@@ -1203,7 +1324,7 @@
     p.prof = (ps.buf && static_cast<long>(p.mtiles) * p.ntiles * p.splits * batch <= ps.blocks) ? ps.buf : nullptr;
     const size_t smem = static_cast<size_t>(STAGES) * (BM + BN) * 64 * sizeof(unsigned short);
     static std::atomic<unsigned long long> lds_set{0};
-    const pf_status s = allow_dynamic_lds(reinterpret_cast<const void*>(k_conv_gemm8<T, NREP, NW, STATS, S3, BM>), smem, lds_set, "pf_conv_gemm (8-wave)");
+    const pf_status s = allow_dynamic_lds(reinterpret_cast<const void*>(k_conv_gemm8<T, NREP, NW, STATS, S3, BM, A32, AFF>), smem, lds_set, "pf_conv_gemm (8-wave)");
     if (s != PF_OK) return s;
     const int cap1 = gemm_tuning().big_persist;
     const int cap = BM == 128 ? 2 * cap1 : cap1;
@@ -1213,7 +1334,7 @@
         if (gx >= 8) gx = gx / 8 * 8;
         grid = std::min(grid, gx);
     }
-    hipLaunchKernelGGL((k_conv_gemm8<T, NREP, NW, STATS, S3, BM>), dim3(grid, p.splits, batch), dim3(64 * NW), smem, st, p);
+    hipLaunchKernelGGL((k_conv_gemm8<T, NREP, NW, STATS, S3, BM, A32, AFF>), dim3(grid, p.splits, batch), dim3(64 * NW), smem, st, p);
     PF_CHECK_LAUNCH("pf_conv_gemm (8-wave)");
     return PF_OK;
 }
@@ -1221,6 +1342,11 @@
 template <typename T, int NREP, int NW, int BM = 256>
 static pf_status launch8w(const GemmParams& gp, int batch, hipStream_t st) {
     if constexpr (NW == 8 || BM == 128) {
+        if (gp.s3 && gp.a32 && gp.a_scale) {
+            if constexpr (NREP == 5 && BM == 256) { set_error("pf_conv_gemm: a_scale on the 256 x 160 tile"); return PF_ERR_ARG; }
+            else return launch8w_s<T, NREP, NW, false, true, BM, true, true>(gp, batch, st);
+        }
+        if (gp.s3 && gp.a32) return launch8w_s<T, NREP, NW, false, true, BM, true>(gp, batch, st);
         if (gp.s3) return gp.gn_partial ? launch8w_s<T, NREP, NW, true, true, BM>(gp, batch, st) : launch8w_s<T, NREP, NW, false, true, BM>(gp, batch, st);
         if (gp.gn_partial) return launch8w_s<T, NREP, NW, true, false, BM>(gp, batch, st);
     }
@@ -1265,6 +1391,18 @@
     PF_REQUIRE(d->out_dtype == d->dtype || d->out_dtype == PF_F32, "pf_conv_gemm: out_dtype must equal dtype or be PF_F32");
     PF_REQUIRE(!d->residual || d->res_dtype == d->dtype || d->res_dtype == PF_F32, "pf_conv_gemm: res_dtype must equal dtype or be PF_F32");
     const int c1 = d->a1 ? d->c1 : 0;
+    const bool a32 = d->a_src_dtype == PF_F32;
+    PF_REQUIRE(d->a_src_dtype == 0 || a32, "pf_conv_gemm: a_src_dtype must be 0 (a0 / a1 hold dtype elements) or PF_F32");
+    PF_REQUIRE(a32 || (!d->a_scale && !d->a_shift), "pf_conv_gemm: a_scale / a_shift belong to fp32 sources (a_src_dtype = PF_F32)");
+    if (a32) {
+        PF_REQUIRE(d->split3 && d->ksize == 1 && d->stride == 1 && d->pad == 0 && d->upsample == 0 && d->wrap_pad == 0 && d->crop == 0 && !d->subpixel &&
+                   d->batch == 1, "pf_conv_gemm: fp32 sources serve the split-precision 1x1 walk only (split3, ksize 1, stride 1, no padding, batch 1)");
+        PF_REQUIRE(d->c0 > 0 && d->c0 % 32 == 0 && c1 % 32 == 0, "pf_conv_gemm: fp32 channel counts (%d,%d) must be multiples of 32", d->c0, c1);
+        PF_REQUIRE(d->a0_ld >= d->c0 && d->a0_ld % 4 == 0 && (!d->a1 || (d->a1_ld >= c1 && d->a1_ld % 4 == 0)),
+                   "pf_conv_gemm: leading dimensions of fp32 sources must be >= their channels and multiples of 4");
+        PF_REQUIRE((d->a_scale != nullptr) == (d->a_shift != nullptr), "pf_conv_gemm: a_scale and a_shift come together");
+        PF_REQUIRE((!d->a_scale || aligned16(d->a_scale)) && (!d->a_shift || aligned16(d->a_shift)), "pf_conv_gemm: a_scale / a_shift must be 16-byte aligned");
+    } else
     PF_REQUIRE(d->c0 > 0 && d->c0 % 64 == 0 && c1 % 64 == 0, "pf_conv_gemm: channel counts (%d,%d) must be multiples of 64", d->c0, c1);
     PF_REQUIRE(d->ksize == 1 || d->ksize == 3, "pf_conv_gemm: ksize must be 1 or 3");
     PF_REQUIRE(d->stride == 1 || d->stride == 2, "pf_conv_gemm: stride must be 1 or 2");
@@ -1273,8 +1411,8 @@
     PF_REQUIRE(d->n_img > 0 && d->h_in > 0 && d->w_in > 0 && d->h_out > 0 && d->w_out > 0, "pf_conv_gemm: bad spatial sizes");
     PF_REQUIRE(d->n_out > 0 && (d->n_out % 4 == 0 || (!d->bias && !d->rowvec && !d->residual && d->out_ld >= (d->n_out + 3) / 4 * 4)),
                "pf_conv_gemm: n_out=%d must be a multiple of 4 (or no epilogue operands and a padded out_ld)", d->n_out);
-    PF_REQUIRE(d->a0_ld >= d->c0 && d->a0_ld % 8 == 0, "pf_conv_gemm: a0_ld must be >= c0 and a multiple of 8");
-    PF_REQUIRE(!d->a1 || (d->a1_ld >= c1 && d->a1_ld % 8 == 0), "pf_conv_gemm: a1_ld must be >= c1 and a multiple of 8");
+    PF_REQUIRE(a32 || (d->a0_ld >= d->c0 && d->a0_ld % 8 == 0), "pf_conv_gemm: a0_ld must be >= c0 and a multiple of 8");
+    PF_REQUIRE(a32 || !d->a1 || (d->a1_ld >= c1 && d->a1_ld % 8 == 0), "pf_conv_gemm: a1_ld must be >= c1 and a multiple of 8");
     PF_REQUIRE(d->epilogue == PF_EPILOGUE_GEGLU || (d->out_ld >= d->n_out && d->out_ld % 4 == 0), "pf_conv_gemm: out_ld must be >= n_out and a multiple of 4");
     PF_REQUIRE(!d->residual || (d->res_ld >= d->n_out && d->res_ld % 4 == 0), "pf_conv_gemm: res_ld must be >= n_out and a multiple of 4");
     PF_REQUIRE(!d->rowvec || (d->rowvec_ld >= d->n_out && d->rowvec_ld % 4 == 0), "pf_conv_gemm: rowvec_ld must be >= n_out and a multiple of 4");
@@ -1287,7 +1425,7 @@
     if (d->epilogue == PF_EPILOGUE_SPLIT)
         PF_REQUIRE(d->n_out % 32 == 0 && d->out_dtype == d->dtype && d->out_ld >= 2 * d->n_out && !d->rowvec,
                    "pf_conv_gemm: SPLIT epilogue needs n_out %% 32 == 0 (hi / lo interleave per 32 columns), a 16-bit output with out_ld >= 2 n_out, no row vector");
-    if (d->split3)
+    if (d->split3 && !a32)
         PF_REQUIRE(!d->a1 && d->c0 % 64 == 0, "pf_conv_gemm: a split-precision walk (split3) takes ONE source of 2 x channels = c0 (hi / lo interleaved per 32)");
     if (d->epilogue == PF_EPILOGUE_GEGLU)
         PF_REQUIRE(d->n_out % 4 == 0 && d->out_dtype == d->dtype && !d->residual && d->out_ld >= d->n_out / 2 && d->out_ld % 2 == 0,
@@ -1310,6 +1448,9 @@
     GemmParams p;
     params_from_desc(d, p);
     const pf_conv_plan g = plan_conv_gemm(p, batch, d->workspace != nullptr, d->gn_partial != nullptr);
+    PF_REQUIRE(!(a32 && d->a_scale && g.kernel == 1 && g.block_rows == 256 && g.nrep == 5),
+               "pf_conv_gemm: a_scale / a_shift are not available on the 256 x 160 tile of the 8-wave kernel (this problem's plan): use the pair form");
+    PF_REQUIRE(!(a32 && d->a_scale) || (d->h_out * d->w_out) % 2 == 0, "pf_conv_gemm: a_scale needs an even number of rows per image");
     if (d->gn_partial) {
         PF_REQUIRE(g.gn_rows > 0, "pf_conv_gemm: gn_partial given but this problem cannot emit GroupNorm moments (ask pf_conv_gemm_gn_rows first)");
         PF_REQUIRE(aligned16(d->gn_partial), "pf_conv_gemm: gn_partial must be 16-byte aligned");
@@ -1320,7 +1461,8 @@
     }
     {
         const long npix = static_cast<long>(d->n_img) * d->h_in * d->w_in;
-        const long a0b = ((npix - 1) * p.a0_ld + p.c0) * 2, a1b = p.a1 ? ((npix - 1) * p.a1_ld + p.c1) * 2 : 0;
+        const long a0b = a32 ? ((npix - 1) * p.a0_ld + p.c0 / 2) * 4 : ((npix - 1) * p.a0_ld + p.c0) * 2;
+        const long a1b = !p.a1 ? 0 : a32 ? ((npix - 1) * p.a1_ld + p.c1 / 2) * 4 : ((npix - 1) * p.a1_ld + p.c1) * 2;
         const long wb = static_cast<long>(p.N) * p.K * 2;
         PF_REQUIRE(a0b < (1L << 31) && a1b < (1L << 31) && wb < (1L << 31),
                    "pf_conv_gemm: each operand must be smaller than 2 GiB (32-bit buffer offsets)");
diff --git a/panfusion_amd/csrc/pf_gemm_params.h b/panfusion_amd/csrc/pf_gemm_params.h
--- a/panfusion_amd/csrc/pf_gemm_params.h
+++ b/panfusion_amd/csrc/pf_gemm_params.h
@@ -33,6 +33,8 @@
     float* gn_partial;
     int gn_rows;
     int fastseg;
+    int a32;
+    const float* a_scale; const float* a_shift;
     int subpix;
 };
 
diff --git a/panfusion_amd/csrc/pf_gemm_plan.hip b/panfusion_amd/csrc/pf_gemm_plan.hip
--- a/panfusion_amd/csrc/pf_gemm_plan.hip
+++ b/panfusion_amd/csrc/pf_gemm_plan.hip
@@ -33,6 +33,9 @@
     p.gn_partial = nullptr; p.gn_rows = 0;
     p.m_begin = 0; p.splits = 1; p.kb_per_split = 0; p.partial = nullptr; p.tickets = nullptr;
     p.a0_bytes = p.a1_bytes = p.w_bytes = 0; p.adv_img = p.adv_y = p.adv_x = 0;
+    p.a32 = d->a_src_dtype == PF_F32;
+    p.a_scale = p.a32 ? d->a_scale : nullptr; p.a_shift = p.a32 ? d->a_shift : nullptr;
+    if (p.a32) { p.c0 = 2 * d->c0; p.c1 = 2 * c1; p.K = 2 * Ctot; }
     p.subpix = 0;
     p.fastseg = (d->upsample == 0 || d->subpixel) && d->wrap_pad == 0 && GemmTuning::conv_fastseg() ? 1 : 0;
     if (d->subpixel) {
@@ -189,6 +192,7 @@
     } else {
         g = plan_tiles(p.M, p.N, p.K, batch, allow_split, p.s3 != 0);
         g.gn_rows = want_moments ? gn_rows16(p, g, batch) : 0;
+        if (p.a32 && g.kernel == 1) g.gn_rows = 0;
         if (g.kernel == 1) {
             if (takes_128_row_blocks(g, p.M, p.N, p.K, batch)) { g.block_rows = 128; g.waves = 4; g.ring_slots = 2; }
             else { g.waves = t.big_waves == 4 && !p.s3 ? 4 : 8; g.ring_slots = 3; }
diff --git a/panfusion_amd/engine.py b/panfusion_amd/engine.py
--- a/panfusion_amd/engine.py
+++ b/panfusion_amd/engine.py
@@ -14,6 +14,8 @@
 
 
 RAW_PAIR_FUSED = os.environ.get("PF_RAW_PAIR", "1") != "0"
+A32 = os.environ.get("PF_A32", "1") != "0"
+TAPING = False
 VIRTUAL_PAD = os.environ.get("PF_VIRTUAL_PAD", "1") != "0"
 EXACT_UP0 = os.environ.get("PF_EXACT_UP0", "1") != "0"
 SUBPIXEL_UP = os.environ.get("PF_SUBPIXEL_UP", "1") != "0"
@@ -67,6 +69,24 @@
     n_img = scale.shape[0] if scale is not None else 1
     hw = x0.numel() // (c * n_img)
     return ops.scale_shift_act(x0, x1, n_img, hw, scale, shift, act, out_dtype=dtype, split=True)
+
+
+def exact_gemm_f32(x0, w3, n_out, dtype, *, x1=None, scale=None, shift=None, save=None, **kw):
+    direct = getattr(ops, "conv_gemm_a32", None)
+    if direct is not None and A32 and save is None and not TAPING and ops.a32_ok(x0, x1):
+        n_img = scale.shape[0] if scale is not None else 1
+        rows = x0.numel() // x0.shape[-1]
+        w_in = kw.pop("w_in", rows)
+        a32 = dict(x1=x1, scale=scale, shift=shift, n_img=n_img, w_in=rows // n_img, **kw)
+        if ops.conv_gemm_a32_serves(x0, w3, n_out, dtype, **a32):
+            return direct(x0, w3, n_out, dtype, **a32)
+        kw["w_in"] = w_in
+    return exact_gemm(split_operand(x0, x1, scale, shift, 0, dtype=dtype), w3, n_out, **kw)
+
+
+def _a32_shortcut(r, x, skip, save):
+    return (r.ws3 is not None and A32 and save is None and not TAPING and getattr(ops, "conv_gemm_a32", None) is not None
+            and ops.a32_ok(x, skip))
 
 
 def exact_gemm(a_split, w3, n_out, **kw):
@@ -373,7 +393,8 @@
     if save is not None:
         save.sc1, save.sh1 = sc, sh
     pair = None
-    if r.ws3 is not None and x.dtype == torch.float32 and RAW_PAIR_FUSED:
+    direct = _a32_shortcut(r, x, skip, save)
+    if r.ws3 is not None and x.dtype == torch.float32 and RAW_PAIR_FUSED and not direct:
         y, pair = ops.scale_shift_act(x, skip, n, hw, sc, sh, 1, out_dtype=r.dtype, raw_pair=True)
     else:
         y = ops.scale_shift_act(x, skip, n, hw, sc, sh, 1, out_dtype=r.dtype)
@@ -387,9 +408,12 @@
         save.h1, save.sc2, save.sh2 = h1, sc, sh
     y2 = ops.scale_shift_act(h1, None, n, h * wp, sc, sh, 1, out_dtype=r.dtype)
     if r.ws3 is not None:
-        if pair is None:
-            pair = split_operand(x, skip, dtype=r.dtype)
-        short = exact_gemm(pair, r.ws3, r.cout, w_in=n * hw, bias=r.bs, out_dtype=r.stream)
+        if direct:
+            short = exact_gemm_f32(x, r.ws3, r.cout, r.dtype, x1=skip, w_in=n * hw, bias=r.bs, out_dtype=r.stream)
+        else:
+            if pair is None:
+                pair = split_operand(x, skip, dtype=r.dtype)
+            short = exact_gemm(pair, r.ws3, r.cout, w_in=n * hw, bias=r.bs, out_dtype=r.stream)
     elif r.ws is not None:
         short = ops.conv_gemm(x, r.ws, r.cout, a1=skip, n_img=n, h_in=h, w_in=w, ksize=1, bias=r.bs)
     else:
@@ -453,8 +477,7 @@
     hw = h * w
     sc, sh = ops.groupnorm_scale_shift(x, None, n, hw, t.norm.groups, t.norm.eps, t.norm.g, t.norm.b)
     if t.w_in3 is not None:
-        tok = exact_gemm(split_operand(x, None, sc, sh, 0, dtype=t.dtype), t.w_in3, Cc, w_in=n * hw, bias=t.b_in,
-                         out_dtype=t.stream)
+        tok = exact_gemm_f32(x, t.w_in3, Cc, t.dtype, scale=sc, shift=sh, w_in=n * hw, bias=t.b_in, out_dtype=t.stream)
     else:
         y = ops.scale_shift_act(x, None, n, hw, sc, sh, 0)
         tok = ops.linear(y.view(n * hw, Cc), t.w_in, bias=t.b_in)
diff --git a/panfusion_amd/ops.py b/panfusion_amd/ops.py
--- a/panfusion_amd/ops.py
+++ b/panfusion_amd/ops.py
@@ -487,7 +487,9 @@
               bias=None, rowvec=None, residual=None, out=None, out_dtype=None, batch=1,
               a_bstride=0, w_bstride=0, out_bstride=0, res_bstride=0, a0_ld=None, a1_ld=None, c0=None, c1=None,
               out_ld=None, res_ld=None, geglu=False, algo_k=None, split_out=False, pad_hi=0, gn_stats=False,
-              wrap_pad=0, crop=0, split3=False, plan_only=False, subpixel=False):
+              wrap_pad=0, crop=0, split3=False, plan_only=False, subpixel=False, a32_dtype=None, a_scale=None, a_shift=None,
+              want_plan=False):
+    op_dtype = a32_dtype or a0.dtype
     c0 = c0 if c0 is not None else a0.shape[-1]
     c1 = (c1 if c1 is not None else a1.shape[-1]) if a1 is not None else 0
     if w_in is None:
@@ -499,26 +501,27 @@
     if out is not None:
         out_dtype = out.dtype
     if split_out:
-        out_dtype = a0.dtype
-    out_dtype = out_dtype or (residual.dtype if residual is not None else a0.dtype)
+        out_dtype = op_dtype
+    out_dtype = out_dtype or (residual.dtype if residual is not None else op_dtype)
     n_store = n_out // 2 if geglu else (2 * n_out if split_out else n_out)
-    if out is None:
+    if out is None and not want_plan:
         out = torch.empty((batch, M, n_store) if batch > 1 else (M, n_store), device=a0.device, dtype=out_dtype)
     a0_ld = a0_ld if a0_ld is not None else _ld(a0)
     a1_ld = (a1_ld if a1_ld is not None else _ld(a1)) if a1 is not None else 0
     rowvec_ld = _ld(rowvec) if rowvec is not None else 0
     res_ld = (res_ld if res_ld is not None else _ld(residual)) if residual is not None else 0
-    res_dtype = dt(residual) if residual is not None else dt(a0)
-    out_ld = out_ld if out_ld is not None else _ld(out)
+    res_dtype = dt(residual) if residual is not None else dt(op_dtype)
+    out_ld = out_ld if out_ld is not None else (_ld(out) if out is not None else n_store)
     epilogue = 1 if geglu else (2 if split_out else 0)
     pkey = (c0, c1, a0_ld, a1_ld, n_img, h_in, w_in, h_out, w_out, ksize, stride, pad, upsample, n_out, batch, epilogue, wrap_pad,
-            crop, dt(a0), dt(out_dtype), residual is not None, res_dtype, res_ld, rowvec is not None, rowvec_ld, bias is not None,
-            out_ld, a_bstride, w_bstride, out_bstride, res_bstride, bool(split3), bool(subpixel))
+            crop, dt(op_dtype), dt(out_dtype), residual is not None, res_dtype, res_ld, rowvec is not None, rowvec_ld, bias is not None,
+            out_ld, a_bstride, w_bstride, out_bstride, res_bstride, bool(split3), bool(subpixel), PF_F32 if a32_dtype else 0, a_scale is not None)
     plans = _PLANS.plans
     plan = plans.get(pkey)
     if plan is None:
         d = _conv_desc(pkey)
         d.a0, d.a1, d.w, d.bias, d.rowvec, d.residual, d.out = _p(a0), _p(a1), _p(w), _p(bias), _p(rowvec), _p(residual), _p(out)
+        d.a_scale, d.a_shift = _p(a_scale), _p(a_shift)
         if len(plans) >= _PLANS.LIMIT:
             plans.pop(next(iter(plans)))
         plan = plans[pkey] = [d, _conv_plan(d, 0), None]
@@ -526,7 +529,12 @@
     if plan_only:
         return plan[1].kernel
     d.a0, d.a1, d.w, d.bias, d.rowvec, d.residual, d.out = _p(a0), _p(a1), _p(w), _p(bias), _p(rowvec), _p(residual), _p(out)
+    d.a_scale, d.a_shift = _p(a_scale), _p(a_shift)
     d.gn_partial, d.gn_rows, d.tickets, d.n_tickets = None, 0, None, 0
+    if want_plan:
+        if gn_stats and GN_FROM_EPILOGUE and batch == 1 and plan[2] is None:
+            plan[2] = _conv_plan(d, 1)
+        return plan[2] if gn_stats and GN_FROM_EPILOGUE and batch == 1 and plan[2].gn_rows > 0 else plan[1]
     g, gn = plan[1], None
     if gn_stats and GN_FROM_EPILOGUE and batch == 1:
         if plan[2] is None:
@@ -545,7 +553,7 @@
     else:
         _traced("k_conv_gemm", 2.0 * M * n_out * (algo_k or ksize * ksize * (c0 + c1)) * batch,
                 lambda: check(_lib.lib().pf_conv_gemm(C.byref(d), _stream()), "pf_conv_gemm"),
-                "M%d N%d K%d k%d s%d u%d b%d%s" % (M, n_out, ksize * ksize * (c0 + c1), ksize, stride, upsample, batch, " g32" if plan[1].kernel == 2 else " subpixel" if subpixel else ""))
+                "M%d N%d K%d k%d s%d u%d b%d%s" % (M, n_out, ksize * ksize * (c0 + c1) * (2 if a32_dtype else 1), ksize, stride, upsample, batch, " g32" if plan[1].kernel == 2 else " subpixel" if subpixel else ""))
     if gn is not None:
         out._pf_gn = gn
     elif hasattr(out, "_pf_gn"):
@@ -553,11 +561,35 @@
     return out
 
 
+def conv_gemm_a32(x0, w3, n_out, dtype, *, x1=None, scale=None, shift=None, n_img=1, w_in=None, **kw):
+    C0, C1 = x0.shape[-1], (x1.shape[-1] if x1 is not None else 0)
+    if w_in is None:
+        w_in = x0.numel() // (C0 * n_img)
+    return conv_gemm(x0, w3, n_out, a1=x1, n_img=n_img, h_in=1, w_in=w_in, c0=C0, c1=C1 if x1 is not None else None,
+                     algo_k=C0 + C1, split3=True, a32_dtype=dtype, a_scale=scale, a_shift=shift, **kw)
+
+
+def conv_gemm_a32_serves(x0, w3, n_out, dtype, **kw):
+    if kw.get("scale") is None:
+        return True
+    g = conv_gemm_a32(x0, w3, n_out, dtype, want_plan=True, **kw)
+    return not (g.kernel == 1 and g.block_rows == 256 and g.nrep == 5)
+
+
+def a32_ok(x0, x1=None):
+    for t in (x0, x1):
+        if t is None:
+            continue
+        if t.dtype != torch.float32 or t.shape[-1] % 32 or t.stride(-1) != 1 or _ld(t) % 4 or t.data_ptr() % 16 or not t.is_contiguous():
+            return False
+    return True
+
+
 def _conv_desc(pkey):
     d = ConvDesc()
     (d.c0, d.c1, d.a0_ld, d.a1_ld, d.n_img, d.h_in, d.w_in, d.h_out, d.w_out, d.ksize, d.stride, d.pad, d.upsample, d.n_out, d.batch,
      d.epilogue, d.wrap_pad, d.crop, d.dtype, d.out_dtype, _, d.res_dtype, d.res_ld, _, d.rowvec_ld, _, d.out_ld,
-     d.a_bstride, d.w_bstride, d.out_bstride, d.res_bstride, d.split3, d.subpixel) = pkey
+     d.a_bstride, d.w_bstride, d.out_bstride, d.res_bstride, d.split3, d.subpixel, d.a_src_dtype, _) = pkey
     return d
 
 
@@ -575,7 +607,7 @@
     h_out = ((h_in << upsample) + 2 * pad - ksize) // stride + 1
     w_out = (((w_in + 2 * wrap_pad) << upsample) + 2 * pad - ksize) // stride + 1 - 2 * crop
     d = _conv_desc((c0, c1, c0, c1, n_img, h_in, w_in, h_out, w_out, ksize, stride, pad, upsample, n_out, batch, 0, wrap_pad, crop,
-                    dt(a0), dt(a0), False, dt(a0), 0, False, 0, False, n_out, 0, 0, 0, 0, False, bool(subpixel)))
+                    dt(a0), dt(a0), False, dt(a0), 0, False, 0, False, n_out, 0, 0, 0, 0, False, bool(subpixel), 0, False))
     d.a1 = _p(a1)
     return max(_conv_plan(d, 0).workspace_bytes, _conv_plan(d, 1).workspace_bytes)
 
diff --git a/panfusion_amd/train_engine.py b/panfusion_amd/train_engine.py
--- a/panfusion_amd/train_engine.py
+++ b/panfusion_amd/train_engine.py
@@ -556,7 +556,11 @@
         if KEEP:
             self.h, rec = transformer_forward_keep(t, x, self.text)
         else:
-            super().attention(t)
+            engine.TAPING = True
+            try:
+                super().attention(t)
+            finally:
+                engine.TAPING = False
         self.tape.append(("attention", self, t, x, rec))
 
     def push(self):
```
